# qq456cvb/CanonicalVoting

Hardware: AMD Instinct MI355X
Metric: scenes/sec (80k-pt synthetic scans) (higher is better)
Workload: dtype f32

## Files before the change

### canonicalvoting_amd/_lib.py

```python
import ctypes
import os
import threading

_HERE = os.path.dirname(os.path.abspath(__file__))
LIB_PATH = os.path.join(_HERE, "_C", "libcvhip.so")

c_float_p = ctypes.POINTER(ctypes.c_float)
c_int_p = ctypes.POINTER(ctypes.c_int)
c_i32_p = ctypes.POINTER(ctypes.c_int32)
c_i64_p = ctypes.POINTER(ctypes.c_int64)
vp = ctypes.c_void_p
ABI_VERSION = 4


class CvError(RuntimeError):
    pass


class DecodeParams(ctypes.Structure):
    _fields_ = [("thresh_high", ctypes.c_float), ("thresh_low", ctypes.c_float),
                ("valid_ratio", ctypes.c_float), ("elimination", ctypes.c_int),
                ("prob_thresh", ctypes.c_float), ("elim_hi_plus1", ctypes.c_int),
                ("max_iters", ctypes.c_int), ("err_thresh", ctypes.c_double)]


class ConvDesc(ctypes.Structure):
    _fields_ = [("in_", vp), ("n_in", ctypes.c_longlong), ("in_ld", ctypes.c_int), ("cin", ctypes.c_int),
                ("weight", vp), ("K", ctypes.c_int), ("cout", ctypes.c_int), ("nbr", vp),
                ("n_out", ctypes.c_longlong), ("scale", vp), ("shift", vp), ("residual", vp),
                ("res_ld", ctypes.c_int), ("relu", ctypes.c_int), ("out", vp), ("out_ld", ctypes.c_int),
                ("flavour", ctypes.c_int), ("ws", vp), ("ws_bytes", ctypes.c_size_t), ("row_perm", vp),
                ("j_begin", ctypes.c_int), ("j_end", ctypes.c_int), ("acc_in", vp), ("acc_ld", ctypes.c_int),
                ("perm_groups", ctypes.c_int), ("plan_ent", vp), ("plan_cnt", vp),
                ("weight_packed", vp), ("weight_x6", vp), ("in2", vp), ("in2_ld", ctypes.c_int), ("cin2", ctypes.c_int),
                ("weight2_x6", vp), ("perm_has_map", ctypes.c_int), ("weight_pieces", ctypes.c_int),
                ("acc_scale", ctypes.c_float), ("range_flag", vp), ("in_hl", ctypes.c_int), ("out_hl", ctypes.c_int),
                ("res_hl", ctypes.c_int), ("split_tickets", vp), ("acc_scale_dev", vp)]


class SceneMaps(ctypes.Structure):
    _fields_ = [("stem", ctypes.c_longlong), ("out", ctypes.c_longlong), ("down", ctypes.c_longlong * 4),
                ("k3", ctypes.c_longlong * 5), ("up", ctypes.c_longlong * 4), ("mask_perm", ctypes.c_longlong * 5),
                ("up_perm", ctypes.c_longlong * 4), ("scratch", ctypes.c_longlong), ("bitmap", ctypes.c_longlong)]


class ScenePlanLayout(ctypes.Structure):
    _fields_ = [("cap", ctypes.c_longlong), ("perm", ctypes.c_longlong), ("inv", ctypes.c_longlong),
                ("coords", ctypes.c_longlong * 5), ("vals", ctypes.c_longlong * 5), ("counts", ctypes.c_longlong),
                ("arena", ctypes.c_longlong), ("int_words", ctypes.c_longlong), ("key_words", ctypes.c_longlong),
                ("sort_ws_bytes", ctypes.c_size_t), ("levels_ws_bytes", ctypes.c_size_t)]


NET_MAP_SLOTS, NET_PERM_SLOTS = 15, 9


class NetBuf(ctypes.Structure):
    _fields_ = [("level", ctypes.c_int), ("channels", ctypes.c_int), ("rows_level", ctypes.c_int), ("hl", ctypes.c_int)]


class NetOp(ctypes.Structure):
    _fields_ = [("in_buf", ctypes.c_int), ("in_col", ctypes.c_int), ("cin", ctypes.c_int),
                ("out_buf", ctypes.c_int), ("out_col", ctypes.c_int), ("cout", ctypes.c_int),
                ("res_buf", ctypes.c_int), ("res_col", ctypes.c_int), ("map", ctypes.c_int), ("K", ctypes.c_int),
                ("perm", ctypes.c_int), ("perm_groups", ctypes.c_int), ("relu", ctypes.c_int),
                ("weight", vp), ("scale", vp), ("shift", vp), ("weight_x6", vp), ("in2_buf", ctypes.c_int),
                ("in2_col", ctypes.c_int), ("cin2", ctypes.c_int), ("weight2_x6", vp), ("weight_pieces", ctypes.c_int), ("acc_scale", ctypes.c_float)]


class SceneDesc(ctypes.Structure):
    _fields_ = [("d_coords4", vp), ("n", ctypes.c_longlong), ("d_feats", vp), ("feats_ld", ctypes.c_int), ("d_points", vp),
                ("res", ctypes.c_float), ("num_rots", ctypes.c_int), ("ops", vp), ("n_ops", ctypes.c_int), ("bufs", vp),
                ("n_bufs", ctypes.c_int), ("stem_k", ctypes.c_int), ("mask_groups", ctypes.c_int),
                ("masked_min_rows", ctypes.c_longlong), ("max_channels", ctypes.c_int),
                ("use_range_flag", ctypes.c_int),
                ("d_out_feats", vp), ("out_ld", ctypes.c_int), ("out_channels", ctypes.c_int), ("nclasses", ctypes.c_int),
                ("log_scale", ctypes.c_int), ("d_xyz_in", vp), ("d_scale_in", vp), ("d_prob_in", vp), ("d_class_in", vp),
                ("vote_algo", ctypes.c_int), ("decode", DecodeParams), ("max_candidates", ctypes.c_int),
                ("nms_threshold", ctypes.c_double), ("d_ws", vp), ("ws_bytes", ctypes.c_size_t), ("d_grids", vp),
                ("grid_capacity_floats", ctypes.c_size_t), ("h_pinned", vp), ("pinned_bytes", ctypes.c_size_t),
                ("h_cand_idx", vp), ("h_verdict", vp), ("h_boxes", vp), ("h_scores", vp), ("h_classes", vp), ("h_pick", vp),
                ("adaptive_split", ctypes.c_int), ("events", vp * 5),
                ("conv_split_target", ctypes.c_int), ("vote_part_records", ctypes.c_int)]


MAX_CATEGORIES = 16


class SceneSeparateDesc(ctypes.Structure):
    _fields_ = [("d_coords4", vp), ("n", ctypes.c_longlong), ("d_feats", vp), ("feats_ld", ctypes.c_int), ("d_points", vp),
                ("res", ctypes.c_float), ("num_rots", ctypes.c_int), ("num_models", ctypes.c_int),
                ("ops", vp), ("n_ops", vp), ("bufs", vp), ("n_bufs", vp),
                ("stem_k", ctypes.c_int), ("mask_groups", ctypes.c_int), ("masked_min_rows", ctypes.c_longlong),
                ("max_channels", ctypes.c_int), ("use_range_flag", ctypes.c_int),
                ("d_out_feats", vp), ("out_ld", ctypes.c_int), ("out_channels", ctypes.c_int), ("log_scale", ctypes.c_int),
                ("d_xyz_in", vp), ("d_scale_in", vp), ("d_prob_in", vp), ("vote_algo", ctypes.c_int), ("decode", DecodeParams),
                ("max_candidates", ctypes.c_int), ("nms_threshold", ctypes.c_double), ("d_ws", vp), ("ws_bytes", ctypes.c_size_t),
                ("h_pinned", vp), ("pinned_bytes", ctypes.c_size_t), ("h_cand_idx", vp), ("h_verdict", vp), ("h_boxes", vp),
                ("h_scores", vp), ("h_det_cat", vp), ("h_det_box", vp), ("events", vp * 5),
                ("conv_split_target", ctypes.c_int), ("vote_part_records", ctypes.c_int)]


class SceneSeparateResult(ctypes.Structure):
    _fields_ = [("n_cand", ctypes.c_int * MAX_CATEGORIES), ("n_boxes", ctypes.c_int * MAX_CATEGORIES),
                ("truncated", ctypes.c_int * MAX_CATEGORIES), ("n_det", ctypes.c_int), ("range_flag", ctypes.c_int),
                ("duplicates", ctypes.c_int), ("out_of_window", ctypes.c_int), ("dims", ctypes.c_int * 3),
                ("corner", ctypes.c_float * 3), ("level_rows", ctypes.c_longlong * 5), ("needed_ws_bytes", ctypes.c_size_t),
                ("d_grid_obj", vp), ("d_grid_rot", vp), ("d_grid_scale", vp), ("d_xyz", vp), ("d_scale", vp), ("d_prob", vp),
                ("host_us", ctypes.c_float * 4)]


class PackJob(ctypes.Structure):
    _fields_ = [("w", vp), ("wp", vp), ("K", ctypes.c_int), ("cin", ctypes.c_int), ("cout", ctypes.c_int), ("trans", ctypes.c_int),
                ("scale_log2", ctypes.c_int), ("reserved", ctypes.c_int)]


class SceneResult(ctypes.Structure):
    _fields_ = [("n_cand", ctypes.c_int), ("n_boxes", ctypes.c_int), ("n_det", ctypes.c_int), ("truncated", ctypes.c_int),
                ("range_flag", ctypes.c_int), ("duplicates", ctypes.c_int), ("out_of_window", ctypes.c_int),
                ("scenes_in_flight", ctypes.c_int), ("dims", ctypes.c_int * 3), ("corner", ctypes.c_float * 3), ("level_rows", ctypes.c_longlong * 5),
                ("needed_ws_bytes", ctypes.c_size_t), ("needed_grid_floats", ctypes.c_size_t),
                ("d_grid_obj", vp), ("d_grid_rot", vp), ("d_grid_scale", vp), ("d_xyz", vp), ("d_scale", vp),
                ("d_prob", vp), ("d_class", vp), ("host_us", ctypes.c_float * 4)]


SIGNATURES = {
    "cv_abi_version": (ctypes.c_int, []),
    "cv_last_error": (ctypes.c_char_p, []),
    "cv_hv_minmax_workspace_bytes": (ctypes.c_size_t, []),
    "cv_hv_minmax_f32": (ctypes.c_int, [vp, ctypes.c_int64, c_float_p, c_float_p, vp, ctypes.c_size_t, vp]),
    "cv_hv_minmax_async_f32": (ctypes.c_int, [vp, ctypes.c_int64, vp, vp, ctypes.c_size_t, vp]),
    "cv_hv_grid_dims_f32": (ctypes.c_int, [c_float_p, c_float_p, ctypes.c_float, c_int_p]),
    "cv_hv_forward_workspace_bytes": (ctypes.c_size_t, [ctypes.c_int64, ctypes.c_int, c_int_p, ctypes.c_int]),
    "cv_hv_forward_f32": (ctypes.c_int, [vp, vp, vp, vp, ctypes.c_int64, ctypes.c_float, ctypes.c_int,
                                         c_float_p, c_int_p, vp, vp, vp, vp, ctypes.c_size_t,
                                         ctypes.c_int, vp]),
    "cv_hv_forward_cat_workspace_bytes": (ctypes.c_size_t, [ctypes.c_int64, ctypes.c_int, c_int_p, ctypes.c_int, ctypes.c_int]),
    "cv_hv_forward_cat_f32": (ctypes.c_int, [vp, vp, vp, vp, ctypes.c_int64, ctypes.c_float, ctypes.c_int, c_float_p, c_int_p,
                                             ctypes.c_int, vp, vp, vp, vp, ctypes.c_size_t, ctypes.c_int, vp]),
    "cv_hv_set_kernel_events": (ctypes.c_int, [vp, vp]),
    "cv_hv_backward_f32": (ctypes.c_int, [vp, vp, vp, vp, vp, ctypes.c_int64, ctypes.c_float,
                                          ctypes.c_int, c_float_p, c_int_p, vp, vp, vp, vp]),
    "cv_hv_count_votes_f32": (ctypes.c_int, [vp, vp, vp, ctypes.c_int64, ctypes.c_float, ctypes.c_int,
                                             c_float_p, c_int_p, c_i64_p, vp, ctypes.c_size_t, vp]),
    "cv_decode_workspace_bytes": (ctypes.c_size_t, [c_int_p, ctypes.c_int64, ctypes.c_int]),
    "cv_decode_f32": (ctypes.c_int, [vp, vp, vp, c_int_p, c_float_p, ctypes.c_float, vp, vp, vp, vp,
                                     ctypes.c_int64, ctypes.POINTER(DecodeParams), ctypes.c_int, vp,
                                     ctypes.c_size_t, c_int_p, c_i64_p, c_i32_p, c_int_p, c_float_p,
                                     c_float_p, c_i32_p, c_int_p, vp]),
    "cv_decode_cat_workspace_bytes": (ctypes.c_size_t, [c_int_p, ctypes.c_int64, ctypes.c_int, ctypes.c_int]),
    "cv_decode_cat_f32": (ctypes.c_int, [vp, vp, vp, c_int_p, c_float_p, ctypes.c_float, vp, vp, vp, vp, ctypes.c_int64,
                                         ctypes.c_int, ctypes.POINTER(DecodeParams), ctypes.c_int, vp, ctypes.c_size_t, c_int_p,
                                         c_i64_p, c_i32_p, c_int_p, c_float_p, c_float_p, c_i32_p, c_int_p, vp]),
    "cv_detect_scene_separate_f32": (ctypes.c_int, [ctypes.POINTER(SceneSeparateDesc), ctypes.POINTER(SceneSeparateResult), vp]),
    "cv_sp_table_capacity": (ctypes.c_longlong, [ctypes.c_longlong]),
    "cv_sp_levels_workspace_bytes": (ctypes.c_size_t, [ctypes.c_longlong]),
    "cv_sp_build_levels": (ctypes.c_int, [ctypes.POINTER(vp), ctypes.POINTER(vp), ctypes.POINTER(vp),
                                          ctypes.c_longlong, ctypes.c_longlong, ctypes.c_int, vp,
                                          c_i32_p, vp, ctypes.c_size_t, vp]),
    "cv_sp_quantize_workspace_bytes": (ctypes.c_size_t, [ctypes.c_longlong]),
    "cv_sp_quantize_f32": (ctypes.c_int, [vp, ctypes.c_longlong, ctypes.c_longlong, ctypes.c_float, ctypes.c_int, c_i64_p,
                                          ctypes.c_int, vp, vp, vp, vp, c_i32_p, vp, ctypes.c_size_t, vp]),
    "cv_sp_quantize_f64": (ctypes.c_int, [vp, ctypes.c_longlong, ctypes.c_longlong, ctypes.c_double, ctypes.c_int, c_i64_p,
                                          ctypes.c_int, vp, vp, vp, vp, c_i32_p, vp, ctypes.c_size_t, vp]),
    "cv_sp_morton_keys": (ctypes.c_int, [vp, ctypes.c_longlong, vp, vp]),
    "cv_sp_sort_workspace_bytes": (ctypes.c_size_t, [ctypes.c_longlong]),
    "cv_sp_sort_rows": (ctypes.c_int, [vp, ctypes.c_longlong, vp, vp, vp, vp, ctypes.c_size_t, vp]),
    "cv_sp_pack_weights_stem_h2_f32": (ctypes.c_int, [vp, ctypes.c_int, ctypes.c_int, vp, ctypes.c_int, vp, vp]),
    "cv_sp_to_hl_f32": (ctypes.c_int, [vp, ctypes.c_longlong, ctypes.c_int, ctypes.c_int, vp, ctypes.c_int, vp, vp]),
    "cv_sp_from_hl_f32": (ctypes.c_int, [vp, ctypes.c_longlong, ctypes.c_int, ctypes.c_int, vp, ctypes.c_int, vp]),
    "cv_sp_kernel_map": (ctypes.c_int, [vp, ctypes.c_longlong, vp, vp, ctypes.c_longlong, ctypes.c_int,
                                        ctypes.c_int, vp, vp]),
    "cv_sp_up_map": (ctypes.c_int, [vp, ctypes.c_longlong, ctypes.c_longlong, vp, vp]),
    "cv_sp_conv_workspace_bytes": (ctypes.c_size_t, [ctypes.c_longlong, ctypes.c_int, ctypes.c_int]),
    "cv_sp_conv_f32": (ctypes.c_int, [ctypes.POINTER(ConvDesc), vp]),
    "cv_sp_set_split_target": (ctypes.c_int, [ctypes.c_int]),
    "cv_hv_set_part_records": (ctypes.c_int, [ctypes.c_int]),
    "cv_hv_set_part_records_thread": (ctypes.c_int, [ctypes.c_int]),
    "cv_sp_pack_weights_h2_batch_f32": (ctypes.c_int, [ctypes.POINTER(PackJob), ctypes.c_int, vp, vp]),
    "cv_sp_copy_unless_flag": (ctypes.c_int, [ctypes.POINTER(vp), ctypes.POINTER(vp), ctypes.POINTER(ctypes.c_longlong), ctypes.c_int, vp, vp]),
    "cv_sp_pack_weights_t_f32": (ctypes.c_int, [vp, ctypes.c_int, ctypes.c_int, ctypes.c_int, ctypes.c_int, ctypes.c_int, vp, vp]),
    "cv_sp_set_split_target_thread": (ctypes.c_int, [ctypes.c_int]),
    "cv_sp_set_ablation": (ctypes.c_int, [ctypes.c_int]),
    "cv_sp_set_option": (ctypes.c_int, [ctypes.c_char_p, ctypes.c_longlong, ctypes.POINTER(ctypes.c_longlong)]),
    "cv_sp_get_option": (ctypes.c_int, [ctypes.c_char_p, ctypes.POINTER(ctypes.c_longlong)]),
    "cv_sp_pack_weights_x6_f32": (ctypes.c_int, [vp, ctypes.c_int, ctypes.c_int, ctypes.c_int, vp, vp, vp]),
    "cv_sp_pack_weights_h2_f32": (ctypes.c_int, [vp, ctypes.c_int, ctypes.c_int, ctypes.c_int, vp, ctypes.c_int, vp, vp]),
    "cv_sp_pack_weights_bf16_f32": (ctypes.c_int, [vp, ctypes.c_int, ctypes.c_int, ctypes.c_int, vp, vp, vp]),
    "cv_sp_scene_maps_words": (ctypes.c_size_t, [c_i64_p, ctypes.c_longlong, ctypes.c_int, ctypes.c_int,
                                                 ctypes.c_longlong, ctypes.POINTER(SceneMaps)]),
    "cv_sp_scene_maps": (ctypes.c_int, [ctypes.POINTER(vp), ctypes.POINTER(vp), ctypes.POINTER(vp), ctypes.c_longlong,
                                        c_i64_p, vp, ctypes.c_longlong, ctypes.c_int,
                                        ctypes.c_int, ctypes.c_longlong, vp, ctypes.c_size_t, vp]),
    "cv_sp_scene_plan_words": (ctypes.c_size_t, [ctypes.c_longlong, ctypes.c_int, ctypes.c_int, ctypes.c_longlong]),
    "cv_sp_scene_plan": (ctypes.c_int, [vp, ctypes.c_longlong, vp, vp, ctypes.POINTER(vp), ctypes.POINTER(vp),
                                        ctypes.POINTER(vp), ctypes.c_longlong, vp, c_i32_p, ctypes.c_int, ctypes.c_int,
                                        ctypes.c_longlong, vp, ctypes.c_size_t, ctypes.POINTER(SceneMaps), vp,
                                        ctypes.c_size_t, vp, ctypes.c_size_t, vp]),
    "cv_sp_scene_plan_layout": (ctypes.c_int, [ctypes.c_longlong, ctypes.c_int, ctypes.c_int, ctypes.c_longlong,
                                               ctypes.POINTER(ScenePlanLayout)]),
    "cv_sp_scene_plan_slots": (ctypes.c_int, [ctypes.POINTER(ScenePlanLayout), ctypes.POINTER(SceneMaps), c_i64_p,
                                              ctypes.c_longlong, vp, ctypes.POINTER(vp), ctypes.POINTER(vp)]),
    "cv_sp_scene_conv_workspace_bytes": (ctypes.c_size_t, [c_i64_p, c_int_p, ctypes.c_int, ctypes.c_int]),
    "cv_net_arena_bytes": (ctypes.c_size_t, [ctypes.POINTER(NetBuf), ctypes.c_int, c_i64_p, ctypes.c_int]),
    "cv_net_run_f32": (ctypes.c_int, [ctypes.POINTER(NetOp), ctypes.c_int, ctypes.POINTER(NetBuf), ctypes.c_int,
                                      c_i64_p, ctypes.c_int, vp, ctypes.c_size_t, ctypes.POINTER(vp), c_int_p,
                                      ctypes.POINTER(vp), ctypes.c_int, ctypes.POINTER(vp), ctypes.c_int,
                                      vp, ctypes.c_size_t, vp, vp]),
    "cv_sp_mask_keys": (ctypes.c_int, [vp, ctypes.c_longlong, ctypes.c_int, ctypes.c_int, ctypes.c_int, vp, vp]),
    "cv_sp_mask_perms": (ctypes.c_int, [vp, ctypes.c_longlong, ctypes.c_int, ctypes.c_int, vp, vp, ctypes.c_size_t,
                                        ctypes.c_int, vp]),
    "cv_sp_transpose_map": (ctypes.c_int, [vp, ctypes.c_longlong, ctypes.c_int, ctypes.c_longlong, vp, vp]),
    "cv_sp_wgrad_workspace_bytes": (ctypes.c_size_t, [ctypes.c_longlong, ctypes.c_int, ctypes.c_int, ctypes.c_int]),
    "cv_sp_conv_wgrad_f32": (ctypes.c_int, [vp, ctypes.c_int, ctypes.c_int, vp, ctypes.c_int, ctypes.c_int, vp,
                                            ctypes.c_int, ctypes.c_longlong, vp, vp, ctypes.c_size_t, vp]),
    "cv_sp_conv_wgrad_px_f32": (ctypes.c_int, [vp, ctypes.c_int, ctypes.c_int, vp, ctypes.c_int, ctypes.c_int, vp,
                                               ctypes.c_int, ctypes.c_longlong, vp, vp, ctypes.c_size_t, ctypes.c_int,
                                               vp]),
    "cv_sp_col_sum_f32": (ctypes.c_int, [vp, ctypes.c_longlong, ctypes.c_int, ctypes.c_int, vp, vp]),
    "cv_sp_col_sum_workspace_bytes": (ctypes.c_size_t, [ctypes.c_longlong, ctypes.c_int]),
    "cv_sp_col_sum_det_f32": (ctypes.c_int, [vp, ctypes.c_longlong, ctypes.c_int, ctypes.c_int, vp, vp, ctypes.c_size_t, vp]),
    "cv_sp_bn_workspace_bytes": (ctypes.c_size_t, [ctypes.c_int]),
    "cv_sp_bn_stats_f32": (ctypes.c_int, [vp, ctypes.c_longlong, ctypes.c_int, ctypes.c_int, vp, vp, ctypes.c_float,
                                          ctypes.c_float, vp, vp, vp, vp, vp, vp, vp, ctypes.c_size_t, vp]),
    "cv_sp_bn_backward_f32": (ctypes.c_int, [vp, vp, vp, ctypes.c_longlong, ctypes.c_int, ctypes.c_int, vp, vp,
                                             ctypes.c_float, vp, vp, vp, vp, vp, vp, ctypes.c_size_t, vp]),
    "cv_sp_bn_backward_hl_f32": (ctypes.c_int, [vp, vp, vp, ctypes.c_longlong, ctypes.c_int, ctypes.c_int, vp, vp,
                                                ctypes.c_float, vp, vp, vp, vp, vp, vp, ctypes.c_size_t, vp, vp, vp, vp, vp]),
    "cv_sp_affine_f32": (ctypes.c_int, [vp, ctypes.c_longlong, ctypes.c_int, ctypes.c_int, vp, vp, vp, ctypes.c_int,
                                        ctypes.c_int, vp, ctypes.c_int, vp]),
    "cv_sp_affine_hl_f32": (ctypes.c_int, [vp, ctypes.c_longlong, ctypes.c_int, ctypes.c_int, vp, vp, vp, ctypes.c_int,
                                           ctypes.c_int, vp, ctypes.c_int, vp, ctypes.c_int, vp, vp, vp]),
    "cv_sp_bn_fold_f32": (ctypes.c_int, [vp, vp, vp, vp, vp, ctypes.c_float, ctypes.c_int, vp, vp, vp]),
    "cv_head_joint_f32": (ctypes.c_int, [vp, ctypes.c_longlong, ctypes.c_int, ctypes.c_int, ctypes.c_int,
                                         vp, vp, vp, vp, vp]),
    "cv_head_separate_f32": (ctypes.c_int, [vp, ctypes.c_longlong, ctypes.c_int, ctypes.c_int, vp, vp, vp, vp]),
    "cv_detect_scene_f32": (ctypes.c_int, [ctypes.POINTER(SceneDesc), ctypes.POINTER(SceneResult), vp]),
    "cv_iou_obb": (ctypes.c_double, [c_float_p, c_float_p]),
    "cv_nms_obb": (ctypes.c_int, [c_float_p, c_float_p, ctypes.c_int, ctypes.c_double, c_i32_p]),
}

_lib = None


def lib():
    global _lib
    if _lib is None:
        if not os.path.exists(LIB_PATH):
            raise CvError(
                "canonicalvoting_amd: HIP library %s not found. Build it with "
                "`python -m canonicalvoting_amd.csrc.build` (hipcc, gfx950). There is no CPU "
                "fallback for this op." % LIB_PATH)
        import torch
        if torch.cuda.is_available():
            torch.cuda.init()
        L = ctypes.CDLL(LIB_PATH)
        for name, (res, args) in SIGNATURES.items():
            fn = getattr(L, name)
            fn.restype = res
            fn.argtypes = args
        _lib = L
    return _lib


_scratch_lock = threading.Lock()
_scratch_bufs = {}


def scratch(dev, name, nbytes):
    import torch
    key = (dev.index if dev.index is not None else torch.cuda.current_device(),
           torch.cuda.current_stream(dev).cuda_stream, name)
    nbytes = max(int(nbytes), 256)
    with _scratch_lock:
        buf = _scratch_bufs.get(key)
    if buf is None or buf.numel() < nbytes:
        buf = torch.empty(nbytes + nbytes // 8, dtype=torch.uint8, device=dev)
        with _scratch_lock:
            _scratch_bufs[key] = buf
    return buf


def release_scratch(dev=None, stream=None):
    h = getattr(stream, "cuda_stream", stream)
    d = getattr(dev, "index", dev)
    with _scratch_lock:
        for key in [k for k in _scratch_bufs if (d is None or k[0] == d) and (h is None or k[1] == h)]:
            del _scratch_bufs[key]


def scratch_bytes():
    with _scratch_lock:
        return sum(b.numel() for b in _scratch_bufs.values())


def check(rc, what):
    if rc != 0:
        msg = lib().cv_last_error()
        raise CvError("%s failed (%d): %s" % (what, rc, msg.decode() if msg else ""))
```

### canonicalvoting_amd/csrc/net_exec.cpp

```cpp
#include <algorithm>
#include <cstdlib>
#include <mutex>
#include <unordered_map>
#include <vector>

#include "cv_common.h"

namespace {

struct Slot { char* ptr; int ld; long long rows; };

}

extern "C" {

static void scene_maps_layout(const long long* rows, long long n_orig, int stem_k, int mask_groups,
                              long long masked_min_rows, cv_scene_maps* o, size_t* total) {
    size_t off = 0;
    auto take = [&](size_t words) { const size_t at = off; off += cv_align_up(words, 64); return (long long)at; };
    const size_t K5 = (size_t)stem_k * stem_k * stem_k;
    const size_t mp_w = mask_groups > 1 ? (size_t)mask_groups * (1 + (27 + mask_groups - 1) / mask_groups) + (mask_groups + 3) / 4 : 0;
    o->stem = take((size_t)rows[0] * K5);
    o->k3[0] = take((size_t)rows[0] * 28);
    o->mask_perm[0] = (mask_groups > 1 && rows[0] >= masked_min_rows) ? take(mp_w * rows[0]) : -1;
// ... 103 lines not shown
}

namespace {
struct PlanSide { hipEvent_t ev; int32_t* h_pinned; int device; };
std::mutex g_plan_mu;
std::unordered_map<int, std::vector<PlanSide>> g_plan_free;
int plan_side_acquire(PlanSide* out) {
    int dev = 0;
    CV_HIP_CHECK(hipGetDevice(&dev));
    {
        std::lock_guard<std::mutex> lk(g_plan_mu);
        auto& pool = g_plan_free[dev];
        if (!pool.empty()) {
            *out = pool.back();
            pool.pop_back();
            return CV_OK;
        }
    }
    PlanSide p{};
    p.device = dev;
    CV_HIP_CHECK(hipEventCreateWithFlags(&p.ev, hipEventDisableTiming));
    CV_HIP_CHECK(hipHostMalloc(reinterpret_cast<void**>(&p.h_pinned), 64, hipHostMallocDefault));
    *out = p;
    return CV_OK;
}
struct PlanSideLease {
    PlanSide ps{};
    bool held = false;
    ~PlanSideLease() {
        if (!held) return;
        (void)hipEventSynchronize(ps.ev);
        std::lock_guard<std::mutex> lk(g_plan_mu);
        g_plan_free[ps.device].push_back(ps);
    }
};
}

size_t cv_sp_scene_plan_words(long long n, int stem_k, int mask_groups, long long masked_min_rows) {
    if (n <= 0 || stem_k < 1) return 0;
    const long long rows[5] = {n, n, n, n, n};
    cv_scene_maps o;
    size_t total = 0;
    scene_maps_layout(rows, n, stem_k, mask_groups, masked_min_rows, &o, &total);
    return total;
}

int cv_sp_scene_plan_layout(long long n, int stem_k, int mask_groups, long long masked_min_rows, cv_scene_plan_layout* out) {
    CV_REQUIRE(out && n > 0, CV_EINVAL, "bad scene plan layout arguments");
    auto up64 = [](long long v) { return (v + 63) / 64 * 64; };
    cv_scene_plan_layout& l = *out;
    l.cap = cv_sp_table_capacity(n);
    l.perm = 0, l.inv = up64(n);
    for (int i = 0; i < 5; ++i) l.coords[i] = l.inv + up64(n) + i * up64(4 * n);
    for (int i = 0; i < 5; ++i) l.vals[i] = l.coords[4] + up64(4 * n) + i * up64(l.cap);
    l.counts = l.vals[4] + up64(l.cap), l.arena = l.counts + 64;
    l.int_words = l.arena + (long long)cv_sp_scene_plan_words(n, stem_k, mask_groups, masked_min_rows);
    l.key_words = 5 * l.cap;
    l.sort_ws_bytes = cv_sp_sort_workspace_bytes(n), l.levels_ws_bytes = cv_sp_levels_workspace_bytes(n);
    return CV_OK;
}

int cv_sp_scene_plan_slots(const cv_scene_plan_layout* layout, const cv_scene_maps* offsets, const long long* level_rows,
                           long long min_rows, const int32_t* d_ibuf, const int32_t** maps, const int32_t** perms) {
    CV_REQUIRE(layout && offsets && level_rows && maps && perms, CV_EINVAL, "null pointer argument");
    const cv_scene_maps& off = *offsets;
    const int32_t* ap = d_ibuf + layout->arena;
    maps[0] = ap + off.stem;
    for (int i = 0; i < 4; ++i) maps[1 + i] = ap + off.down[i];
    for (int i = 0; i < 5; ++i) maps[5 + i] = ap + off.k3[i];
    for (int i = 0; i < 4; ++i) maps[10 + i] = ap + off.up[i];
    maps[14] = d_ibuf + layout->inv;
    for (int i = 0; i < 5; ++i) perms[i] = (off.mask_perm[i] >= 0 && level_rows[i] >= min_rows) ? ap + off.mask_perm[i] : nullptr;
    for (int i = 0; i < 4; ++i) perms[5 + i] = ap + off.up_perm[i];
    return CV_OK;
}

size_t cv_sp_scene_conv_workspace_bytes(const long long* level_rows, const int* masked, int mask_groups, int max_channels) {
    if (!level_rows || !masked) return 0;
    size_t bytes = 0;
    for (int i = 0; i < 5; ++i) {
        if (masked[i]) bytes = std::max(bytes, (size_t)4 * mask_groups * (size_t)level_rows[i] * max_channels + 256);
        bytes = std::max(bytes, cv_sp_conv_workspace_bytes(std::min<long long>(level_rows[i], 128 * 384 - 1), max_channels, 27));
    }
    return bytes;
}

int cv_sp_scene_plan(const int32_t* d_input, long long n, int32_t* d_perm, int32_t* d_inv, int32_t* const* d_coords,
                     unsigned long long* const* d_keys, int32_t* const* d_vals, long long cap, int32_t* d_counts,
                     int32_t* h_counts, int stem_k, int mask_groups, long long masked_min_rows, int32_t* d_arena,
                     size_t arena_words, cv_scene_maps* offsets, void* d_sort_ws, size_t sort_ws_bytes, void* d_levels_ws,
                     size_t levels_ws_bytes, void* stream) {
    return cv_sp_scene_plan_ex(d_input, n, d_perm, d_inv, d_coords, d_keys, d_vals, cap, d_counts, h_counts, stem_k, mask_groups,
                               masked_min_rows, d_arena, arena_words, offsets, d_sort_ws, sort_ws_bytes, d_levels_ws,
                               levels_ws_bytes, false, stream);
}

}

int cv_sp_scene_plan_ex(const int32_t* d_input, long long n, int32_t* d_perm, int32_t* d_inv, int32_t* const* d_coords,
                        unsigned long long* const* d_keys, int32_t* const* d_vals, long long cap, int32_t* d_counts,
                        int32_t* h_counts, int stem_k, int mask_groups, long long masked_min_rows,
                        int32_t* d_arena, size_t arena_words, cv_scene_maps* offsets, void* d_sort_ws, size_t sort_ws_bytes,
                        void* d_levels_ws, size_t levels_ws_bytes, bool single_batch, void* stream, bool bounds_prefilled) {
    CV_REQUIRE(d_input && d_perm && d_inv && d_coords && d_keys && d_vals && d_counts && h_counts && d_arena && offsets &&
                   d_sort_ws && d_levels_ws, CV_EINVAL, "null pointer argument");
    CV_REQUIRE(arena_words >= cv_sp_scene_plan_words(n, stem_k, mask_groups, masked_min_rows), CV_ENOMEM,
               "scene map arena too small (cv_sp_scene_plan_words)");
    hipStream_t st = static_cast<hipStream_t>(stream);
    int rc = cv_sp_sort_rows_ex(d_input, n, d_coords[0], d_perm, d_inv, d_sort_ws, sort_ws_bytes, single_batch, stream, bounds_prefilled);
    if (rc != CV_OK) return rc;
    long long rows[5] = {n, 1, 1, 1, 1};
    cv_scene_maps o;
    size_t total = 0;
    scene_maps_layout(rows, n, stem_k, mask_groups, masked_min_rows, &o, &total);
    static const bool bitmap_on = !(getenv("CV_MAP_BITMAP") && atoi(getenv("CV_MAP_BITMAP")) == 0);
    const long long n_zero = o.bitmap + (bitmap_on ? CV_BITMAP_WORDS : 0) - o.scratch;
    rc = cv_sp_build_levels_zero(d_coords, d_keys, d_vals, n, cap, 5, d_counts, nullptr, d_levels_ws, levels_ws_bytes,
                                 d_arena + o.scratch, n_zero, bitmap_on ? static_cast<int32_t*>(d_sort_ws) + 7 : nullptr, stream,
                                 bitmap_on ? reinterpret_cast<uint32_t*>(d_arena + o.bitmap) : nullptr);
    if (rc != CV_OK) return rc;
    PlanSideLease lease;
    rc = plan_side_acquire(&lease.ps);
    if (rc != CV_OK) return rc;
    lease.held = true;
    const PlanSide& ps = lease.ps;
    CV_HIP_CHECK(hipMemcpyAsync(ps.h_pinned, d_counts, sizeof(int32_t) * 8, hipMemcpyDeviceToHost, st));
    CV_HIP_CHECK(hipEventRecord(ps.ev, st));
    rc = scene_maps_level0(d_coords, d_keys, d_vals, cap, n, d_perm, stem_k, mask_groups, o, d_arena,
                           bitmap_on ? static_cast<const int32_t*>(d_sort_ws) : nullptr, stream, true, bitmap_on);
    if (rc != CV_OK) return rc;
    CV_HIP_CHECK(hipEventSynchronize(ps.ev));
    for (int i = 0; i < 8; ++i) h_counts[i] = ps.h_pinned[i];
    if (h_counts[5] != 0 || h_counts[6] != 0) return CV_OK;
    for (int i = 0; i < 5; ++i) rows[i] = h_counts[i];
    CV_REQUIRE(rows[0] == n, CV_EINVAL, "level 0 lost rows (%lld of %lld)", rows[0], n);
    scene_maps_layout(rows, n, stem_k, mask_groups, masked_min_rows, &o, &total);
    CV_REQUIRE(arena_words >= total, CV_ENOMEM, "scene map arena too small");
    *offsets = o;
    return scene_maps_coarse(d_coords, d_keys, d_vals, cap, rows, mask_groups, o, d_arena, stream, true);
}

extern "C" {

size_t cv_net_arena_bytes(const cv_net_buf* bufs, int n_bufs, const long long* level_rows, int n_levels) {
    if (!bufs || !level_rows || n_bufs <= 0) return 0;
    size_t total = 256;
    for (int i = 0; i < n_bufs; ++i) {
        if (bufs[i].level < 0 || bufs[i].level >= n_levels) continue;
        total += cv_align_up(sizeof(float) * (size_t)level_rows[bufs[i].level] * (size_t)bufs[i].channels, 256);
    }
    return total;
}

int cv_net_run_f32(const cv_net_op* ops, int n_ops, const cv_net_buf* bufs, int n_bufs, const long long* level_rows,
                   int n_levels, void* d_arena, size_t arena_bytes, const void* const* ext_ptr, const int* ext_ld,
                   const int32_t* const* maps, int n_maps, const int32_t* const* perms, int n_perms,
                   void* d_ws, size_t ws_bytes, int32_t* range_flag, void* stream) {
    CV_REQUIRE(ops && bufs && level_rows && d_arena && n_ops > 0 && n_bufs > 0 && n_levels > 0, CV_EINVAL,
               "bad network program arguments");
    CV_REQUIRE(arena_bytes >= cv_net_arena_bytes(bufs, n_bufs, level_rows, n_levels), CV_ENOMEM, "arena too small");
    std::vector<Slot> slot((size_t)n_bufs);
    {
        CvCarver cv(d_arena);
        int ext = 0;
        for (int i = 0; i < n_bufs; ++i) {
            const int lv = bufs[i].level;
            if (lv < 0 || lv >= n_levels) {
                CV_REQUIRE(ext_ptr && ext_ld && ext_ptr[ext], CV_EINVAL, "external buffer %d has no pointer", ext);
                slot[i] = {static_cast<char*>(const_cast<void*>(ext_ptr[ext])), ext_ld[ext], bufs[i].rows_level >= 0 &&
                           bufs[i].rows_level < n_levels ? level_rows[bufs[i].rows_level] : 0};
                ++ext;
            } else {
                slot[i] = {reinterpret_cast<char*>(cv.take<float>((size_t)level_rows[lv] * bufs[i].channels)),
                           bufs[i].channels, level_rows[lv]};
            }
        }
    }
    for (int k = 0; k < n_ops; ++k) {
        const cv_net_op& o = ops[k];
        CV_REQUIRE(o.in_buf >= 0 && o.in_buf < n_bufs && o.out_buf >= 0 && o.out_buf < n_bufs &&
                       o.res_buf < n_bufs && o.map < n_maps && o.perm < n_perms, CV_EINVAL, "op %d: bad slot", k);
        const Slot& in = slot[o.in_buf];
        const Slot& out = slot[o.out_buf];
        cv_conv_desc d = {};
        d.in_hl = bufs[o.in_buf].hl;
        d.out_hl = bufs[o.out_buf].hl;
        d.res_hl = o.res_buf >= 0 ? bufs[o.res_buf].hl : 0;
        CV_REQUIRE(o.in2_buf < 0 || bufs[o.in2_buf].hl == d.in_hl, CV_EINVAL, "op %d: both sources must share a format", k);
        d.in = reinterpret_cast<const float*>(in.ptr) + o.in_col;
        d.n_in = in.rows;
        d.in_ld = in.ld;
        d.cin = o.cin;
        d.weight = o.weight;
        d.weight_x6 = o.weight_x6;
        d.weight_pieces = o.weight_pieces;
        d.acc_scale = o.acc_scale;
        d.range_flag = (o.weight_pieces == 2 || d.out_hl) ? range_flag : nullptr;
        if (o.in2_buf >= 0) {
            CV_REQUIRE(o.in2_buf < n_bufs, CV_EINVAL, "op %d: bad second-source slot", k);
            d.in2 = reinterpret_cast<const float*>(slot[o.in2_buf].ptr) + o.in2_col;
            d.in2_ld = slot[o.in2_buf].ld;
            d.cin2 = o.cin2;
            d.weight2_x6 = o.weight2_x6;
        }
        d.K = o.K;
        d.cout = o.cout;
        d.nbr = o.map >= 0 ? maps[o.map] : nullptr;
        d.n_out = out.rows;
        d.scale = o.scale;
        d.shift = o.shift;
        if (o.res_buf >= 0) {
            d.residual = reinterpret_cast<const float*>(slot[o.res_buf].ptr) + o.res_col;
            d.res_ld = slot[o.res_buf].ld;
        }
        d.relu = o.relu;
        d.out = reinterpret_cast<float*>(out.ptr) + o.out_col;
        d.out_ld = out.ld;
        d.ws = d_ws;
        d.ws_bytes = ws_bytes;
        const int32_t* perm = o.perm >= 0 ? perms[o.perm] : nullptr;
        if (perm) {
            d.row_perm = perm;
            d.perm_groups = o.perm_groups;
            d.perm_has_map = o.perm_groups > 1;
        }
        const int rc = cv_sp_conv_f32(&d, stream);
        if (rc != CV_OK) return rc;
    }
    return CV_OK;
}

}
```

### canonicalvoting_amd/csrc/scene_exec.cpp

```cpp
#include <algorithm>
#include <atomic>
#include <chrono>
#include <cstdlib>
#include <cstring>
#include <vector>

#include "cv_common.h"

namespace {

struct Carver {
    char* base; size_t off = 0, cap;
    Carver(void* p, size_t c) : base(static_cast<char*>(p)), cap(c) {}
    template <typename T> T* take(size_t count) {
        off = cv_align_up(off, 256);
        T* r = (base && off + count * sizeof(T) <= cap) ? reinterpret_cast<T*>(base + off) : nullptr;
        off += count * sizeof(T);
        return r;
    }
};

std::atomic<int> g_scenes_inside{0};
struct SceneCount {
    int before;
    bool set_target, set_records;
    int prev_target = 0, prev_records = 0;
    SceneCount(bool adaptive, int split_target, int part_records)
        : before(g_scenes_inside.fetch_add(1, std::memory_order_relaxed)), set_target(adaptive || split_target > 0),
          set_records(part_records > 0) {
        if (set_target) prev_target = cv_sp_set_split_target_thread(split_target > 0 ? split_target : before + 1 >= 4 ? 256 : 768);
        if (set_records) prev_records = cv_hv_set_part_records_thread(part_records);
    }
    ~SceneCount() {
        if (set_target) cv_sp_set_split_target_thread(prev_target);
        if (set_records) cv_hv_set_part_records_thread(prev_records);
        g_scenes_inside.fetch_sub(1, std::memory_order_relaxed);
    }
};

struct StageClock {
    void* const* events; hipStream_t st; float* host_us;
    std::chrono::steady_clock::time_point t_prev = std::chrono::steady_clock::now();
    hipError_t mark(int i) const { return events[i] ? hipEventRecord(static_cast<hipEvent_t>(events[i]), st) : hipSuccess; }
    void lap(int i) {
        const auto t = std::chrono::steady_clock::now();
        host_us[i] += std::chrono::duration<float, std::micro>(t - t_prev).count();
        t_prev = t;
    }
};

struct SceneFront {
    const int32_t* d_coords4; long long n; const float* d_points; float res;
    int stem_k, mask_groups; long long masked_min_rows; int max_channels;
    float* h_minmax;
    cv_scene_plan_layout lay;
    void* mm_ws; int32_t* ibuf; unsigned long long* kbuf; char* sort_ws; char* lev_ws;
    cv_scene_maps off;
    long long rows[5];
    float mn[3]; int dims[3]; size_t cells;
    const int32_t* maps[CV_NET_MAP_SLOTS]; const int32_t* perms[CV_NET_PERM_SLOTS];
    size_t conv_ws_b;

    template <class D> explicit SceneFront(const D* d)
        : d_coords4(d->d_coords4), n(d->n), d_points(d->d_points), res(d->res), stem_k(d->stem_k), mask_groups(d->mask_groups),
          masked_min_rows(d->masked_min_rows), max_channels(d->max_channels), h_minmax(static_cast<float*>(d->h_pinned)) {}

    bool carve(Carver& cv) {
        mm_ws = cv.take<char>(cv_hv_minmax_workspace_bytes());
        cv_sp_scene_plan_layout(n, stem_k, mask_groups, masked_min_rows, &lay);
        ibuf = cv.take<int32_t>((size_t)lay.int_words);
        kbuf = cv.take<unsigned long long>((size_t)lay.key_words);
        sort_ws = cv.take<char>(lay.sort_ws_bytes);
        lev_ws = cv.take<char>(lay.levels_ws_bytes);
        return mm_ws && ibuf && kbuf && sort_ws && lev_ws;
    }

    template <class R> int run(int32_t* d_zero_word, R* r, StageClock& clock, void* stream) {
        int rc = cv_hv_minmax_async_ex(d_points, n, h_minmax, mm_ws, cv_hv_minmax_workspace_bytes(), d_zero_word,
                                       reinterpret_cast<int32_t*>(sort_ws), stream);
        if (rc != CV_OK) return rc;
        int32_t *c_coords[5], *c_vals[5];
        unsigned long long* c_keys[5];
        for (int i = 0; i < 5; ++i) {
            c_coords[i] = ibuf + lay.coords[i];
            c_keys[i] = kbuf + (size_t)lay.cap * i;
            c_vals[i] = ibuf + lay.vals[i];
        }
        int32_t counts_h[8] = {0};
        rc = cv_sp_scene_plan_ex(d_coords4, n, ibuf + lay.perm, ibuf + lay.inv, c_coords, c_keys, c_vals, lay.cap, ibuf + lay.counts,
                                 counts_h, stem_k, mask_groups, masked_min_rows, ibuf + lay.arena, (size_t)(lay.int_words - lay.arena),
                                 &off, sort_ws, lay.sort_ws_bytes, lev_ws, lay.levels_ws_bytes,
                                  true, stream,  true);
        if (rc != CV_OK) return rc;
        r->duplicates = counts_h[5];
        r->out_of_window = counts_h[6];
        CV_REQUIRE(counts_h[5] == 0 && counts_h[6] == 0, CV_EINVAL,
                   "duplicate coordinates (%d) or coordinates outside the 16-bit key window (%d)", counts_h[5], counts_h[6]);
        clock.lap(0);
        for (int i = 0; i < 5; ++i) { rows[i] = counts_h[i]; r->level_rows[i] = counts_h[i]; }
        float mx[3];
        for (int k = 0; k < 3; ++k) { mn[k] = h_minmax[k]; mx[k] = h_minmax[3 + k]; r->corner[k] = mn[k]; }
        rc = cv_hv_grid_dims_f32(mn, mx, res, dims);
        if (rc != CV_OK) return rc;
        for (int k = 0; k < 3; ++k) r->dims[k] = dims[k];
        cells = (size_t)dims[0] * dims[1] * dims[2];
        int masked[5];
        for (int i = 0; i < 5; ++i) masked[i] = off.mask_perm[i] >= 0;
        conv_ws_b = cv_sp_scene_conv_workspace_bytes(rows, masked, mask_groups, max_channels);
        return cv_sp_scene_plan_slots(&lay, &off, rows, masked_min_rows, ibuf, maps, perms);
    }
};

template <class R> int fixed_part_too_small(R* r, size_t fixed_end) {
    r->needed_ws_bytes = fixed_end * 2 + ((size_t)256 << 20);
    cv_set_error("scene workspace too small (needs at least %zu bytes)", r->needed_ws_bytes);
    return CV_ENOMEM;
}

}

extern "C" {

int cv_detect_scene_f32(const cv_scene_desc* d, cv_scene_result* r, void* stream) {
    CV_REQUIRE(d && r, CV_EINVAL, "null scene descriptor / result");
    CV_REQUIRE(d->d_coords4 && d->d_feats && d->d_points && d->n > 0 && d->ops && d->bufs && d->n_ops > 0 && d->n_bufs > 0,
               CV_EINVAL, "bad scene descriptor");
    CV_REQUIRE(d->d_out_feats && d->out_ld >= d->out_channels && d->out_channels > 0, CV_EINVAL, "bad network output buffer");
    CV_REQUIRE(d->h_pinned && d->pinned_bytes >= 256 && d->d_ws, CV_EINVAL, "pinned scratch (>= 256 bytes) and a device workspace are required");
    CV_REQUIRE(d->h_boxes && d->h_scores && d->h_classes && d->h_cand_idx && d->h_verdict && d->h_pick && d->max_candidates > 0,
               CV_EINVAL, "null result arrays");
    hipStream_t st = static_cast<hipStream_t>(stream);
    const long long n = d->n;
    std::memset(r, 0, sizeof(*r));
    CV_REQUIRE(d->conv_split_target >= 0 && d->vote_part_records >= 0, CV_EINVAL, "negative launch sizing");
    SceneCount in_flight(d->adaptive_split != 0, d->conv_split_target, d->vote_part_records);
    r->scenes_in_flight = in_flight.before + 1;
    Carver cv(d->d_ws, d->ws_bytes);
    StageClock clock{d->events, st, r->host_us};
    CV_HIP_CHECK(clock.mark(0));

    SceneFront f(d);
    int32_t* h_flag = reinterpret_cast<int32_t*>(static_cast<char*>(d->h_pinned) + 64);
    const bool plan_fits = f.carve(cv);
    float* xyz = cv.take<float>((size_t)n * 3);
    float* scale = cv.take<float>((size_t)n * 3);
    float* prob = cv.take<float>((size_t)n);
    int32_t* cls = cv.take<int32_t>((size_t)n);
    int32_t* d_flag = cv.take<int32_t>(64);
    if (!plan_fits || !xyz || !scale || !prob || !cls || !d_flag) return fixed_part_too_small(r, cv.off);
    int rc = f.run(d_flag, r, clock, stream);
    if (rc != CV_OK) return rc;
    const size_t cells = f.cells;

    const size_t arena_b = cv_net_arena_bytes(d->bufs, d->n_bufs, f.rows, 5);
    const size_t vote_ws_b = cv_hv_forward_workspace_bytes(n, d->num_rots, f.dims, d->vote_algo);
    const size_t dec_ws_b = cv_decode_workspace_bytes(f.dims, n, d->max_candidates);
    char* arena = cv.take<char>(arena_b);
    char* conv_ws = cv.take<char>(f.conv_ws_b);
    char* vote_ws = cv.take<char>(std::max<size_t>(vote_ws_b, 256));
    char* dec_ws = cv.take<char>(dec_ws_b);
    float* grids = d->d_grids ? d->d_grids : cv.take<float>(6 * cells);
    r->needed_ws_bytes = cv.off + 4096;
    r->needed_grid_floats = 6 * cells;
    CV_REQUIRE(arena && conv_ws && vote_ws && dec_ws && grids, CV_ENOMEM, "scene workspace too small (needs %zu bytes)", r->needed_ws_bytes);
    CV_REQUIRE(!d->d_grids || d->grid_capacity_floats >= 6 * cells, CV_ENOMEM, "grid buffer too small (needs %zu floats)", 6 * cells);
    float* g_obj = grids;
    float* g_rot = grids + cells;
    float* g_scale = grids + 3 * cells;
    r->d_grid_obj = g_obj; r->d_grid_rot = g_rot; r->d_grid_scale = g_scale;

    const void* ext_ptr[2] = {d->d_feats, d->d_out_feats};
    const int ext_ld[2] = {d->feats_ld, d->out_ld};
    rc = cv_net_run_f32(d->ops, d->n_ops, d->bufs, d->n_bufs, f.rows, 5, arena, arena_b, ext_ptr, ext_ld, f.maps, CV_NET_MAP_SLOTS,
                        f.perms, CV_NET_PERM_SLOTS, conv_ws, f.conv_ws_b, d->use_range_flag ? d_flag : nullptr, stream);
    if (rc != CV_OK) return rc;
    clock.lap(1);
    CV_HIP_CHECK(clock.mark(1));
    rc = cv_head_joint_f32(d->d_out_feats, n, d->out_ld, d->nclasses, d->log_scale, xyz, scale, prob, cls, stream);
    if (rc != CV_OK) return rc;
    if (d->use_range_flag) CV_HIP_CHECK(hipMemcpyAsync(h_flag, d_flag, sizeof(int32_t), hipMemcpyDeviceToHost, st));
    r->d_xyz = xyz; r->d_scale = scale; r->d_prob = prob; r->d_class = cls;
    CV_HIP_CHECK(clock.mark(2));

    const float* v_xyz = d->d_xyz_in ? d->d_xyz_in : xyz;
    const float* v_scale = d->d_scale_in ? d->d_scale_in : scale;
    const float* v_prob = d->d_prob_in ? d->d_prob_in : prob;
    const int32_t* v_cls = d->d_class_in ? d->d_class_in : cls;
    rc = cv_hv_forward_f32(d->d_points, v_xyz, v_scale, v_prob, n, d->res, d->num_rots, f.mn, f.dims, g_obj, g_rot, g_scale, vote_ws,
                           std::max<size_t>(vote_ws_b, 256), d->vote_algo, stream);
    if (rc != CV_OK) return rc;
    CV_HIP_CHECK(clock.mark(3));
    clock.lap(2);
    cv_decode_params prm = d->decode;
    prm.max_iters = d->max_candidates;
    int n_cand = 0, n_boxes = 0, truncated = 0;
    rc = cv_decode_f32_ev(g_obj, g_rot, g_scale, f.dims, f.mn, d->res, d->d_points, v_xyz, v_prob, v_cls, n, &prm, 0, dec_ws, dec_ws_b, &n_cand,
                          d->h_cand_idx, d->h_verdict, &n_boxes, d->h_boxes, d->h_scores, d->h_classes, &truncated, stream, d->events[4]);
    if (rc != CV_OK) return rc;
    r->n_cand = n_cand;
    r->n_boxes = n_boxes;
    r->truncated = truncated;
    r->range_flag = d->use_range_flag ? *h_flag : 0;

    int n_det = 0;
    std::vector<float> bc, sc;
    std::vector<int32_t> idx, pick;
    for (int c = 0; c < d->nclasses; ++c) {
        bc.clear(); sc.clear(); idx.clear();
        for (int i = 0; i < n_boxes; ++i)
            if (d->h_classes[i] == c) {
                bc.insert(bc.end(), d->h_boxes + (size_t)i * 24, d->h_boxes + (size_t)i * 24 + 24);
                sc.push_back(d->h_scores[i]);
                idx.push_back(i);
            }
        if (idx.empty()) continue;
        pick.assign(idx.size(), 0);
        const int k = cv_nms_obb(bc.data(), sc.data(), (int)idx.size(), d->nms_threshold, pick.data());
        if (k < 0) return k;
        for (int j = 0; j < k; ++j) d->h_pick[n_det++] = idx[(size_t)pick[j]];
    }
    r->n_det = n_det;
    clock.lap(3);
    return CV_OK;
}

int cv_detect_scene_separate_f32(const cv_scene_separate_desc* d, cv_scene_separate_result* r, void* stream) {
    CV_REQUIRE(d && r, CV_EINVAL, "null scene descriptor / result");
    std::memset(r, 0, sizeof(*r));
    const int K = d->num_models;
    CV_REQUIRE(K >= 1 && K <= CV_MAX_CATEGORIES, CV_EINVAL, "num_models out of range (%d, 1..%d)", K, CV_MAX_CATEGORIES);
    CV_REQUIRE(d->d_coords4 && d->d_feats && d->d_points && d->n > 0 && d->ops && d->n_ops && d->bufs && d->n_bufs && d->d_out_feats,
               CV_EINVAL, "bad scene descriptor");
    for (int k = 0; k < K; ++k)
        CV_REQUIRE(d->ops[k] && d->bufs[k] && d->n_ops[k] > 0 && d->n_bufs[k] > 0 && d->d_out_feats[k], CV_EINVAL,
                   "bad program or output buffer of model %d", k);
    CV_REQUIRE(d->out_ld >= d->out_channels && d->out_channels >= 8, CV_EINVAL, "bad network output buffer");
    CV_REQUIRE(d->h_pinned && d->pinned_bytes >= 64 + 64 * (size_t)K && d->d_ws, CV_EINVAL,
               "pinned scratch (>= 64 + 64 K bytes) and a device workspace are required");
    CV_REQUIRE(d->h_boxes && d->h_scores && d->h_cand_idx && d->h_verdict && d->h_det_cat && d->h_det_box && d->max_candidates > 0,
               CV_EINVAL, "null result arrays");
    CV_REQUIRE(!!d->d_xyz_in == !!d->d_scale_in && !!d->d_xyz_in == !!d->d_prob_in, CV_EINVAL, "predictions: all three or none");
    CV_REQUIRE(d->conv_split_target >= 0 && d->vote_part_records >= 0, CV_EINVAL, "negative launch sizing");
    hipStream_t st = static_cast<hipStream_t>(stream);
    const long long n = d->n;
    SceneCount in_flight(false, d->conv_split_target, d->vote_part_records);
    Carver cv(d->d_ws, d->ws_bytes);
    StageClock clock{d->events, st, r->host_us};
    CV_HIP_CHECK(clock.mark(0));

    SceneFront f(d);
    int32_t* h_flags = reinterpret_cast<int32_t*>(static_cast<char*>(d->h_pinned) + 64);
    const bool plan_fits = f.carve(cv);
    float* xyz = cv.take<float>((size_t)K * n * 3);
    float* scale = cv.take<float>((size_t)K * n * 3);
    float* prob = cv.take<float>((size_t)K * n);
    int32_t* d_flags = cv.take<int32_t>(16 * (size_t)K);
    if (!plan_fits || !xyz || !scale || !prob || !d_flags) return fixed_part_too_small(r, cv.off);
    if (d->use_range_flag) CV_HIP_CHECK(hipMemsetAsync(d_flags, 0, sizeof(int32_t) * 16 * K, st));
    int rc = f.run(nullptr, r, clock, stream);
    if (rc != CV_OK) return rc;
    const size_t cells = f.cells;

    size_t arena_b = 0;
    for (int k = 0; k < K; ++k) arena_b = std::max(arena_b, cv_net_arena_bytes(d->bufs[k], d->n_bufs[k], f.rows, 5));
    const size_t vote_ws_b = cv_hv_forward_cat_workspace_bytes(n, d->num_rots, f.dims, d->vote_algo, K);
    const size_t dec_ws_b = cv_decode_cat_workspace_bytes(f.dims, n, d->max_candidates, K);
    char* arena = cv.take<char>(arena_b);
    char* conv_ws = cv.take<char>(f.conv_ws_b);
    char* vote_ws = cv.take<char>(std::max<size_t>(vote_ws_b, 256));
    char* dec_ws = cv.take<char>(dec_ws_b);
    float* grids = cv.take<float>(6 * cells * (size_t)K);
    r->needed_ws_bytes = cv.off + 4096;
    CV_REQUIRE(arena && conv_ws && vote_ws && dec_ws && grids, CV_ENOMEM, "scene workspace too small (needs %zu bytes)", r->needed_ws_bytes);
    float* g_obj = grids;
    float* g_rot = grids + cells * K;
    float* g_scale = grids + 3 * cells * K;
    r->d_grid_obj = g_obj; r->d_grid_rot = g_rot; r->d_grid_scale = g_scale;

    for (int k = 0; k < K; ++k) {
        const void* ext_ptr[2] = {d->d_feats, d->d_out_feats[k]};
        const int ext_ld[2] = {d->feats_ld, d->out_ld};
        rc = cv_net_run_f32(d->ops[k], d->n_ops[k], d->bufs[k], d->n_bufs[k], f.rows, 5, arena, arena_b, ext_ptr, ext_ld, f.maps,
                            CV_NET_MAP_SLOTS, f.perms, CV_NET_PERM_SLOTS, conv_ws, f.conv_ws_b,
                            d->use_range_flag ? d_flags + 16 * k : nullptr, stream);
        if (rc != CV_OK) return rc;
    }
    clock.lap(1);
    CV_HIP_CHECK(clock.mark(1));
    for (int k = 0; k < K; ++k) {
        rc = cv_head_separate_f32(d->d_out_feats[k], n, d->out_ld, d->log_scale, xyz + (size_t)k * n * 3, scale + (size_t)k * n * 3,
                                  prob + (size_t)k * n, stream);
        if (rc != CV_OK) return rc;
    }
    if (d->use_range_flag) CV_HIP_CHECK(hipMemcpyAsync(h_flags, d_flags, sizeof(int32_t) * 16 * K, hipMemcpyDeviceToHost, st));
    r->d_xyz = xyz; r->d_scale = scale; r->d_prob = prob;
    CV_HIP_CHECK(clock.mark(2));

    const float* v_xyz = d->d_xyz_in ? d->d_xyz_in : xyz;
    const float* v_scale = d->d_xyz_in ? d->d_scale_in : scale;
    const float* v_prob = d->d_xyz_in ? d->d_prob_in : prob;
    rc = cv_hv_forward_cat_f32(d->d_points, v_xyz, v_scale, v_prob, n, d->res, d->num_rots, f.mn, f.dims, K, g_obj, g_rot, g_scale, vote_ws,
                               std::max<size_t>(vote_ws_b, 256), d->vote_algo, stream);
    if (rc != CV_OK) return rc;
    CV_HIP_CHECK(clock.mark(3));
    clock.lap(2);
    cv_decode_params prm = d->decode;
    prm.max_iters = d->max_candidates;
    const int M = d->max_candidates;
    std::vector<int32_t> classes((size_t)K * M);
    rc = cv_decode_cat_f32_ev(g_obj, g_rot, g_scale, f.dims, f.mn, d->res, d->d_points, v_xyz, v_prob, nullptr, n, K, &prm, 0, dec_ws,
                              dec_ws_b, r->n_cand, d->h_cand_idx, d->h_verdict, r->n_boxes, d->h_boxes, d->h_scores, classes.data(),
                              r->truncated, stream, d->events[4]);
    if (rc != CV_OK) return rc;
    if (d->use_range_flag)
        for (int k = 0; k < K; ++k) r->range_flag |= h_flags[16 * k] ? (1 << k) : 0;

    int n_det = 0;
    std::vector<int32_t> pick((size_t)M);
    for (int k = 0; k < K; ++k) {
        const int nb = r->n_boxes[k];
        if (nb == 0) continue;
        const int kept = cv_nms_obb(d->h_boxes + (size_t)k * M * 24, d->h_scores + (size_t)k * M, nb, d->nms_threshold, pick.data());
        if (kept < 0) return kept;
        for (int j = 0; j < kept; ++j) { d->h_det_cat[n_det] = k; d->h_det_box[n_det] = pick[(size_t)j]; ++n_det; }
    }
    r->n_det = n_det;
    clock.lap(3);
    return CV_OK;
}

}
```

### canonicalvoting_amd/csrc/sparse_conv.hip

```cpp
#include "cv_common.h"

#include <atomic>
#include <cstring>
#include <type_traits>
#include <utility>

#include "sparse_conv_common.h"

using namespace cvsc;

namespace {

template <int NB, bool VEC>
__global__ __launch_bounds__(THREADS) void conv_rows(ConvArgs a) {
    __shared__ float A_s[KC][A_LD];
    __shared__ float B_s[KC][NB * 32];
    __shared__ int nbr_s[TM];
    __shared__ int rows_s[TM];
    __shared__ __attribute__((aligned(16))) float ep_s[4][32][EP_LD];
    const int tid = threadIdx.x, lane = tid & 63, wave = tid >> 6;
    const int n0 = blockIdx.y * (NB * 32);

    if (tid < TM) {
        const long long tile_id = a.row_perm ? (long long)gridDim.x - 1 - blockIdx.x : blockIdx.x;
// ... 1254 lines not shown

__global__ __launch_bounds__(256) void col_sum_partial(const float* __restrict__ x, long long n, int c, int ld,
                                                       float* __restrict__ ws) {
    __shared__ float s[8][32];
    const int col = blockIdx.x * 32 + (threadIdx.x & 31), ry = threadIdx.x >> 5;
    const long long r_lo = n * blockIdx.y / gridDim.y, r_hi = n * (blockIdx.y + 1) / gridDim.y;
    float acc = 0.f;
    if (col < c)
        for (long long r = r_lo + ry; r < r_hi; r += 8) acc += x[r * ld + col];
    s[ry][threadIdx.x & 31] = acc;
    __syncthreads();
    if (ry == 0 && col < c) {
        float t = 0.f;
        for (int k = 0; k < 8; ++k) t += s[k][threadIdx.x & 31];
        ws[(long long)blockIdx.y * c + col] = t;
    }
}
__global__ __launch_bounds__(256) void col_sum_chunks(const float* __restrict__ ws, int chunks, int c,
                                                      float* __restrict__ out) {
    const int col = blockIdx.x * 256 + threadIdx.x;
    if (col >= c) return;
    float s0 = 0.f, s1 = 0.f, s2 = 0.f, s3 = 0.f;
    int k = 0;
    for (; k + 3 < chunks; k += 4) {
        s0 += ws[(long long)k * c + col];
        s1 += ws[(long long)(k + 1) * c + col];
        s2 += ws[(long long)(k + 2) * c + col];
        s3 += ws[(long long)(k + 3) * c + col];
    }
    for (; k < chunks; ++k) s0 += ws[(long long)k * c + col];
    out[col] = (s0 + s1) + (s2 + s3);
}

__global__ __launch_bounds__(256) void conv_finish(ConvArgs a) {
    __shared__ float4 red[4][64];
    const int q = threadIdx.x >> 6, l = threadIdx.x & 63;
    const long long total4 = a.n_out * (long long)a.cout / 4;
    const long long total = a.n_out * (long long)a.cout;
    for (long long base = blockIdx.x * 64ll; base < total4; base += (long long)gridDim.x * 64) {
        const long long e4 = base + l;
        float4 s = make_float4(0.f, 0.f, 0.f, 0.f);
        if (e4 < total4) {
            const float4* p = reinterpret_cast<const float4*>(a.partial) + e4;
#pragma unroll 4
            for (int k = q; k < a.splits; k += 4) {
                const float4 v = partial_load4(p + (long long)k * (total / 4));
                s.x += v.x; s.y += v.y; s.z += v.z; s.w += v.w;
            }
        }
        red[q][l] = s;
        __syncthreads();
        if (q == 0 && e4 < total4) {
            float v[4] = {red[0][l].x + red[1][l].x + red[2][l].x + red[3][l].x,
                          red[0][l].y + red[1][l].y + red[2][l].y + red[3][l].y,
                          red[0][l].z + red[1][l].z + red[2][l].z + red[3][l].z,
                          red[0][l].w + red[1][l].w + red[2][l].w + red[3][l].w};
            const long long e = e4 * 4;
            const long long row = e / a.cout;
            const int col = (int)(e - row * a.cout);
            if (a.wide) {
                float4 x = make_float4(v[0], v[1], v[2], v[3]);
                if (a.acc_in) {
                    const float4 p = *reinterpret_cast<const float4*>(a.acc_in + row * a.acc_ld + col);
                    x.x += p.x; x.y += p.y; x.z += p.z; x.w += p.w;
                }
                const float4 sc = a.scale ? *reinterpret_cast<const float4*>(a.scale + col) : make_float4(1.f, 1.f, 1.f, 1.f);
                const float4 sh = a.shift ? *reinterpret_cast<const float4*>(a.shift + col) : make_float4(0.f, 0.f, 0.f, 0.f);
                x.x = x.x * sc.x + sh.x; x.y = x.y * sc.y + sh.y; x.z = x.z * sc.z + sh.z; x.w = x.w * sc.w + sh.w;
                if (a.res) {
                    const float4 p = a.res_hl ? hl_load4(a.res + row * a.res_ld, col)
                                              : *reinterpret_cast<const float4*>(a.res + row * a.res_ld + col);
                    x.x += p.x; x.y += p.y; x.z += p.z; x.w += p.w;
                }
                if (a.relu) { x.x = fmaxf(x.x, 0.f); x.y = fmaxf(x.y, 0.f); x.z = fmaxf(x.z, 0.f); x.w = fmaxf(x.w, 0.f); }
                if (a.out_hl) {
                    if (a.range_flag && hl_out_of_range(x)) *a.range_flag = 1;
                    hl_store4(a.out + row * a.out_ld, col, x);
                } else {
                    *reinterpret_cast<float4*>(a.out + row * a.out_ld + col) = x;
                }
            } else
#pragma unroll
            for (int i = 0; i < 4; ++i) {
                float x = v[i];
                if (a.acc_in) x += a.acc_in[row * a.acc_ld + col + i];
                x = x * (a.scale ? a.scale[col + i] : 1.f) + (a.shift ? a.shift[col + i] : 0.f);
                if (a.res) x += a.res[row * a.res_ld + col + i];
                if (a.relu) x = fmaxf(x, 0.f);
                a.out[row * a.out_ld + col + i] = x;
            }
        }
        __syncthreads();
    }
}

constexpr int FINISH_SMALL_MAX = 16;
__global__ __launch_bounds__(256) void conv_finish_small(ConvArgs a) {
    const long long total4 = a.n_out * (long long)a.cout / 4;
    const int cq = a.cout >> 2;
    for (long long e4 = blockIdx.x * 256ll + threadIdx.x; e4 < total4; e4 += (long long)gridDim.x * 256) {
        const float4* p = reinterpret_cast<const float4*>(a.partial) + e4;
        const long long row = e4 / cq;
        float4 pv[FINISH_SMALL_MAX];
#pragma unroll
        for (int k = 0; k < FINISH_SMALL_MAX; ++k)
            pv[k] = (k < a.splits && (!a.gvalid || a.gvalid[(long long)k * a.n_out + row]))
                        ? partial_load4(p + (long long)k * total4) : make_float4(0.f, 0.f, 0.f, 0.f);
        const int col = (int)(e4 - row * cq) * 4;
        float4 sq[4];
#pragma unroll
        for (int q = 0; q < 4; ++q) sq[q] = make_float4(0.f, 0.f, 0.f, 0.f);
#pragma unroll
        for (int k = 0; k < FINISH_SMALL_MAX; ++k)
            if (k < a.splits) { sq[k & 3].x += pv[k].x; sq[k & 3].y += pv[k].y; sq[k & 3].z += pv[k].z; sq[k & 3].w += pv[k].w; }
        float4 x = make_float4(sq[0].x + sq[1].x + sq[2].x + sq[3].x, sq[0].y + sq[1].y + sq[2].y + sq[3].y,
                               sq[0].z + sq[1].z + sq[2].z + sq[3].z, sq[0].w + sq[1].w + sq[2].w + sq[3].w);
        if (a.acc_in) {
            const float4 q = *reinterpret_cast<const float4*>(a.acc_in + row * a.acc_ld + col);
            x.x += q.x; x.y += q.y; x.z += q.z; x.w += q.w;
        }
        const float4 sc = a.scale ? *reinterpret_cast<const float4*>(a.scale + col) : make_float4(1.f, 1.f, 1.f, 1.f);
        const float4 sh = a.shift ? *reinterpret_cast<const float4*>(a.shift + col) : make_float4(0.f, 0.f, 0.f, 0.f);
        x.x = x.x * sc.x + sh.x; x.y = x.y * sc.y + sh.y; x.z = x.z * sc.z + sh.z; x.w = x.w * sc.w + sh.w;
        if (a.res) {
            const float4 q = a.res_hl ? hl_load4(a.res + row * a.res_ld, col)
                                      : *reinterpret_cast<const float4*>(a.res + row * a.res_ld + col);
            x.x += q.x; x.y += q.y; x.z += q.z; x.w += q.w;
        }
        if (a.relu) { x.x = fmaxf(x.x, 0.f); x.y = fmaxf(x.y, 0.f); x.z = fmaxf(x.z, 0.f); x.w = fmaxf(x.w, 0.f); }
        if (a.out_hl) {
            if (a.range_flag && hl_out_of_range(x)) *a.range_flag = 1;
            hl_store4(a.out + row * a.out_ld, col, x);
        } else {
            *reinterpret_cast<float4*>(a.out + row * a.out_ld + col) = x;
        }
    }
}

__global__ __launch_bounds__(256) void conv_finish_scalar(ConvArgs a) {
    const long long total = a.n_out * (long long)a.cout;
    for (long long t = blockIdx.x * 256ll + threadIdx.x; t < total; t += (long long)gridDim.x * 256) {
        const long long row = t / a.cout;
        const int col = (int)(t - row * a.cout);
        float v = 0.f;
        for (int sidx = 0; sidx < a.splits; ++sidx) v += a.partial[sidx * total + t];
        if (a.acc_in) v += a.acc_in[row * a.acc_ld + col];
        v = v * (a.scale ? a.scale[col] : 1.f) + (a.shift ? a.shift[col] : 0.f);
        if (a.res) v += a.res[row * a.res_ld + col];
        if (a.relu) v = fmaxf(v, 0.f);
        a.out[row * a.out_ld + col] = v;
    }
}

}
namespace cvsc {
std::atomic<int> g_ablation{0};
int launch_finish(const ConvArgs& a, hipStream_t st) {
    if (g_ablation.load(std::memory_order_relaxed) & 1) return CV_OK;
    const long long total = a.n_out * (long long)a.cout;
    if (a.wide && a.splits <= FINISH_SMALL_MAX)
        conv_finish_small<<<(unsigned)std::min<long long>((total / 4 + 255) / 256, 16384), 256, 0, st>>>(a);
    else if (a.cout % 4 == 0)
        conv_finish<<<(unsigned)std::min<long long>((total / 4 + 63) / 64, 8192), 256, 0, st>>>(a);
    else
        conv_finish_scalar<<<(unsigned)std::min<long long>((total + 255) / 256, 4096), 256, 0, st>>>(a);
    CV_LAUNCH_CHECK();
    return CV_OK;
}
}
namespace {

__global__ __launch_bounds__(256) void mask_keys(const int* __restrict__ nbr, long long n, int K, int j_begin,
                                                 int j_end, long long* __restrict__ keys) {
    const long long i = blockIdx.x * 256ll + threadIdx.x;
    if (i >= n) return;
    unsigned long long m = 0;
    for (int j = j_begin; j < j_end; ++j)
        if (nbr[i * K + j] >= 0) m |= 1ull << (j - j_begin);
    keys[i] = (long long)m;
}

constexpr int MP_BINS = 1024;
constexpr int MP_THREADS = 1024;

__device__ __forceinline__ int group_mask(const int* __restrict__ nbr, long long row, long long n, int K, int jb, int je) {
    int m = 0;
    for (int j = jb; j < je; ++j)
        if (nbr[row * K + j] >= 0) m |= 1 << (j - jb);
    if (je - jb <= 7) m |= __popc(m) << 7;
    (void)n;
    return m;
}

__device__ __forceinline__ int group_mask_of_word(int word, int jb, int je) {
    int m = (int)(((unsigned)word >> jb) & ((1u << (je - jb)) - 1u));
    if (je - jb <= 7) m |= __popc(m) << 7;
    return m;
}

__global__ __launch_bounds__(MP_THREADS) void mp_hist(const int* __restrict__ nbr, long long n, int K, int groups,
                                                      int* __restrict__ hist ) {
    __shared__ int lh[MP_BINS];
    const int g = blockIdx.y;
    const int jb = K * g / groups, je = K * (g + 1) / groups;
    for (int i = threadIdx.x; i < MP_BINS; i += MP_THREADS) lh[i] = 0;
    __syncthreads();
    const long long row = blockIdx.x * (long long)MP_THREADS + threadIdx.x;
    if (row < n) atomicAdd(&lh[group_mask(nbr, row, n, K, jb, je)], 1);
    __syncthreads();
    for (int i = threadIdx.x; i < MP_BINS; i += MP_THREADS)
        if (lh[i]) atomicAdd(&hist[g * MP_BINS + i], lh[i]);
}

__global__ __launch_bounds__(MP_BINS) void mp_scan(int* __restrict__ hist) {
    __shared__ int s[MP_BINS];
    int* h = hist + blockIdx.x * MP_BINS;
    const int v = h[threadIdx.x];
    s[threadIdx.x] = v;
    __syncthreads();
    for (int off = 1; off < MP_BINS; off <<= 1) {
        const int t = threadIdx.x >= off ? s[threadIdx.x - off] : 0;
        __syncthreads();
        s[threadIdx.x] += t;
        __syncthreads();
    }
    h[threadIdx.x] = s[threadIdx.x] - v;
}

__global__ __launch_bounds__(MP_THREADS) void mp_scatter(const int* __restrict__ nbr, long long n, int K, int groups,
                                                         int* __restrict__ cursor, int* __restrict__ perm,
                                                         int* __restrict__ nbrp, int W) {
    unsigned char* gv = nbrp ? reinterpret_cast<unsigned char*>(nbrp + (long long)groups * n * W) : nullptr;
    __shared__ int lh[MP_BINS];
    const int g = blockIdx.y;
    const int jb = K * g / groups, je = K * (g + 1) / groups;
    for (int i = threadIdx.x; i < MP_BINS; i += MP_THREADS) lh[i] = 0;
    __syncthreads();
    const long long row = blockIdx.x * (long long)MP_THREADS + threadIdx.x;
    int key = 0, rank = 0;
    if (row < n) {
        key = group_mask(nbr, row, n, K, jb, je);
        rank = atomicAdd(&lh[key], 1);
    }
    __syncthreads();
    for (int i = threadIdx.x; i < MP_BINS; i += MP_THREADS)
        if (lh[i]) lh[i] = atomicAdd(&cursor[g * MP_BINS + i], lh[i]);
    __syncthreads();
    if (row < n) {
        const long long pos = (long long)g * n + lh[key] + rank;
        perm[pos] = (int)row;
        if (nbrp) {
            for (int j = jb; j < je; ++j) nbrp[pos * W + (j - jb)] = nbr[row * K + j];
            gv[(long long)g * n + row] = key != 0;
        }
    }
}

struct PermJobsDev {
    CvPermJob j[CV_MAX_PERM_JOBS];
    int group_begin[CV_MAX_PERM_JOBS + 1];
    int n;
};

__device__ __forceinline__ int perm_job_of(const PermJobsDev& jobs, int gy) {
    int ji = 0;
    while (ji + 1 < jobs.n && gy >= jobs.group_begin[ji + 1]) ++ji;
    return ji;
}

__global__ __launch_bounds__(MP_THREADS) void mp_hist_batch(const PermJobsDev jobs, int* __restrict__ hist) {
    __shared__ int lh[MP_BINS];
    const int ji = perm_job_of(jobs, blockIdx.y);
    const CvPermJob& jb = jobs.j[ji];
    const long long row = blockIdx.x * (long long)MP_THREADS + threadIdx.x;
    if (blockIdx.x * (long long)MP_THREADS >= jb.n) return;
    const int g = blockIdx.y - jobs.group_begin[ji];
    const int jlo = jb.K * g / jb.groups, jhi = jb.K * (g + 1) / jb.groups;
    for (int i = threadIdx.x; i < MP_BINS; i += MP_THREADS) lh[i] = 0;
    __syncthreads();
    if (row < jb.n)
        atomicAdd(&lh[jb.mask_words ? group_mask_of_word(jb.mask_words[row], jlo, jhi) : group_mask(jb.nbr, row, jb.n, jb.K, jlo, jhi)], 1);
    __syncthreads();
    for (int i = threadIdx.x; i < MP_BINS; i += MP_THREADS)
        if (lh[i]) atomicAdd(&hist[blockIdx.y * MP_BINS + i], lh[i]);
}

__global__ __launch_bounds__(MP_THREADS) void mp_scatter_batch(const PermJobsDev jobs, const int* __restrict__ hist,
                                                               int* __restrict__ cursor) {
    static_assert(MP_THREADS == MP_BINS, "one bin per thread in the scan");
    __shared__ int lh[MP_BINS];
    __shared__ int pre[MP_BINS];
    __shared__ int wtot[MP_THREADS / 64];
    const int ji = perm_job_of(jobs, blockIdx.y);
    const CvPermJob& jb = jobs.j[ji];
    if (blockIdx.x * (long long)MP_THREADS >= jb.n) return;
    const int g = blockIdx.y - jobs.group_begin[ji];
    const int K = jb.K, jlo = K * g / jb.groups, jhi = K * (g + 1) / jb.groups, W = (K + jb.groups - 1) / jb.groups;
    int* nbrp = jb.with_map ? jb.perm + (long long)jb.groups * jb.n : nullptr;
    for (int i = threadIdx.x; i < MP_BINS; i += MP_THREADS) lh[i] = 0;
    {
        const int lane = threadIdx.x & 63, wave = threadIdx.x >> 6;
        const int v = hist[blockIdx.y * MP_BINS + threadIdx.x];
        int incl = v;
#pragma unroll
        for (int off = 1; off < 64; off <<= 1) {
            const int t = __shfl_up(incl, off);
            if (lane >= off) incl += t;
        }
        if (lane == 63) wtot[wave] = incl;
        __syncthreads();
        int base = 0;
#pragma unroll
// ... 227 lines not shown
            const long long o = r * ld + k;
            take(*reinterpret_cast<const float4*>(x + o), MODE == 1 ? *reinterpret_cast<const float4*>(dy + o) : z4,
                 (MODE == 1 && (y || ybits)) ? relu_open4(y, ybits, r, k, ld, c) : z4, y != nullptr || ybits != nullptr);
        }
    }
#pragma unroll
    for (int i = 0; i < 8; ++i) red[threadIdx.x][i] = a[i];
    __syncthreads();
    if (threadIdx.x < cq) {
        double t[8] = {0, 0, 0, 0, 0, 0, 0, 0};
        for (int q = 0; q < rl; ++q)
#pragma unroll
            for (int i = 0; i < 8; ++i) t[i] += red[q * cq + threadIdx.x][i];
#pragma unroll
        for (int i = 0; i < 4; ++i) {
            partial[((long long)blockIdx.x * c + threadIdx.x * 4 + i) * 2 + 0] = t[i];
            partial[((long long)blockIdx.x * c + threadIdx.x * 4 + i) * 2 + 1] = t[4 + i];
        }
    }
}

template <int MODE>
__global__ __launch_bounds__(256) void bn_col_finish(const double* __restrict__ partial, int chunks, long long n, int c,
                                                     float* out0, float* out1, float* running_mean, float* running_var,
                                                     float momentum, const float* gamma, const float* beta, float eps,
                                                     float* scale, float* shift) {
    const int sub = threadIdx.x & 15;
    const int k = blockIdx.x * 16 + (threadIdx.x >> 4);
    double t0 = 0.0, t1 = 0.0;
    if (k < c)
        for (int q = sub; q < chunks; q += 16) {
            t0 += partial[((long long)q * c + k) * 2];
            t1 += partial[((long long)q * c + k) * 2 + 1];
        }
#pragma unroll
    for (int off = 8; off >= 1; off >>= 1) {
        t0 += __shfl_xor(t0, off);
        t1 += __shfl_xor(t1, off);
    }
    if (k >= c || sub != 0) return;
    if (MODE == 0) {
        const double mu = t0 / (double)n;
        double v = t1 / (double)n - mu * mu;
        if (v < 0.0) v = 0.0;
        out0[k] = (float)mu;
        out1[k] = (float)v;
        if (running_mean) {
            const double unb = n > 1 ? v * (double)n / (double)(n - 1) : v;
            running_mean[k] = (1.f - momentum) * running_mean[k] + momentum * (float)mu;
            running_var[k] = (1.f - momentum) * running_var[k] + momentum * (float)unb;
        }
        const float sc = gamma[k] / sqrtf((float)v + eps);
        scale[k] = sc;
        shift[k] = beta[k] - (float)mu * sc;
    } else {
        out0[k] = (float)t0;
        out1[k] = (float)t1;
    }
}

constexpr int BN_SLOT_BLOCKS = 4096;
__global__ __launch_bounds__(256) void bn_backward_apply(const float* __restrict__ x, const float* __restrict__ dy,
                                                         const float* __restrict__ y, long long n, int c, int ld,
                                                         const float* __restrict__ mean, const float* __restrict__ var,
                                                         float eps, const float* __restrict__ gamma,
                                                         const float* __restrict__ sum_dy,
                                                         const float* __restrict__ sum_dy_xhat, float* __restrict__ dx,
                                                         float* __restrict__ dres) {
    const float inv_n = 1.0f / (float)n;
    for (long long t = blockIdx.x * 256ll + threadIdx.x; t < n * c; t += (long long)gridDim.x * 256) {
        const long long r = t / c;
        const int k = (int)(t - r * c);
        const float istd = 1.0f / sqrtf(var[k] + eps);
        const float xh = (x[r * ld + k] - mean[k]) * istd;
        float g = dy[r * ld + k];
        if (y && !(y[r * ld + k] > 0.f)) g = 0.f;
        dx[r * ld + k] = gamma[k] * istd * (g - sum_dy[k] * inv_n - xh * sum_dy_xhat[k] * inv_n);
        if (dres) dres[r * ld + k] = g;
    }
}

__global__ __launch_bounds__(256) void bn_backward_apply4(const float* __restrict__ x, const float* __restrict__ dy,
                                                          const float* __restrict__ y, long long n, int c, int ld,
                                                          const float* __restrict__ mean, const float* __restrict__ var,
                                                          float eps, const float* __restrict__ gamma,
                                                          const float* __restrict__ sum_dy,
                                                          const float* __restrict__ sum_dy_xhat, float* __restrict__ dx,
                                                          float* __restrict__ dres, float* __restrict__ dx_hl = nullptr,
                                                          unsigned* __restrict__ slot = nullptr,
                                                          int* __restrict__ range_flag = nullptr,
                                                          const unsigned* __restrict__ ybits = nullptr) {
    const float inv_n = 1.0f / (float)n;
    const int cq = c >> 2;
    __shared__ unsigned wred[4];
    float hs = 1.f, dmax = 0.f;
    if (dx_hl) {
        unsigned mb = 0u;
        for (int i = threadIdx.x; i < BN_SLOT_BLOCKS; i += 256) mb = max(mb, slot[BN_SLOT_BLOCKS + i]);
#pragma unroll
        for (int off = 32; off > 0; off >>= 1) mb = max(mb, (unsigned)__shfl_xor((int)mb, off));
        if ((threadIdx.x & 63) == 0) wred[threadIdx.x >> 6] = mb;
        __syncthreads();
        mb = max(max(wred[0], wred[1]), max(wred[2], wred[3]));
        __syncthreads();
        const unsigned E = (mb >> 23) & 255u;
        hs = (E >= 10u && E <= 250u) ? __uint_as_float((263u - E) << 23) : 1.f;
        if (blockIdx.x == 0 && threadIdx.x == 0) reinterpret_cast<float*>(slot)[2 * BN_SLOT_BLOCKS] = 1.f / hs;
    }
    for (long long t = blockIdx.x * 256ll + threadIdx.x; t < n * cq; t += (long long)gridDim.x * 256) {
        const long long r = t / cq;
        const int k = (int)(t - r * cq) * 4;
        const long long o = r * ld + k;
        const float4 xv = *reinterpret_cast<const float4*>(x + o);
        float4 g = *reinterpret_cast<const float4*>(dy + o);
        if (y || ybits) {
            const float4 yv = relu_open4(y, ybits, r, k, ld, c);
            if (!(yv.x > 0.f)) g.x = 0.f;
            if (!(yv.y > 0.f)) g.y = 0.f;
            if (!(yv.z > 0.f)) g.z = 0.f;
            if (!(yv.w > 0.f)) g.w = 0.f;
        }
        const float xs[4] = {xv.x, xv.y, xv.z, xv.w}, gs[4] = {g.x, g.y, g.z, g.w};
        float d[4];
#pragma unroll
        for (int i = 0; i < 4; ++i) {
            const float istd = 1.0f / sqrtf(var[k + i] + eps);
            const float xh = (xs[i] - mean[k + i]) * istd;
            d[i] = gamma[k + i] * istd * (gs[i] - sum_dy[k + i] * inv_n - xh * sum_dy_xhat[k + i] * inv_n);
        }
        *reinterpret_cast<float4*>(dx + o) = make_float4(d[0], d[1], d[2], d[3]);
        if (dres) *reinterpret_cast<float4*>(dres + o) = g;
        if (dx_hl) {
            dmax = fmaxf(fmaxf(dmax, fmaxf(fabsf(d[0]), fabsf(d[1]))), fmaxf(fabsf(d[2]), fabsf(d[3])));
            const float4 v = make_float4(d[0] * hs, d[1] * hs, d[2] * hs, d[3] * hs);
            if (range_flag && hl_out_of_range(v)) *range_flag = 1;
            hl_store4(dx_hl + r * ld, k, v);
        }
    }
    if (dx_hl) {
#pragma unroll
        for (int off = 32; off > 0; off >>= 1) dmax = fmaxf(dmax, __shfl_xor(dmax, off));
        if ((threadIdx.x & 63) == 0) wred[threadIdx.x >> 6] = __float_as_uint(dmax);
        __syncthreads();
        if (threadIdx.x == 0) slot[blockIdx.x] = max(max(wred[0], wred[1]), max(wred[2], wred[3]));
    }
}

__global__ __launch_bounds__(256) void head_joint(const float* __restrict__ f, long long n, int ld,
                                                  int ncls, int log_scale, float* __restrict__ xyz,
                                                  float* __restrict__ scale, float* __restrict__ prob,
                                                  int* __restrict__ cls) {
    const long long i = blockIdx.x * 256ll + threadIdx.x;
    if (i >= n) return;
    const float* row = f + i * ld;
    const float* logit = row + 6 * ncls;
    float mx = logit[0];
    int am = 0;
    for (int k = 1; k <= ncls; ++k)
        if (logit[k] > mx) { mx = logit[k]; am = k; }
    float mo = logit[0];
    int ao = 0;
    for (int k = 1; k < ncls; ++k)
        if (logit[k] > mo) { mo = logit[k]; ao = k; }
    float den = 0.f;
    for (int k = 0; k <= ncls; ++k) den += expf(logit[k] - mx);
    const int h = am == ncls ? 0 : am;
    for (int d = 0; d < 3; ++d) {
        xyz[i * 3 + d] = row[h * 3 + d];
        const float s = row[3 * ncls + h * 3 + d];
        scale[i * 3 + d] = log_scale ? expf(s) : s;
    }
    prob[i] = expf(mo - mx) / den;
    cls[i] = ao;
}

__global__ __launch_bounds__(256) void head_separate(const float* __restrict__ f, long long n, int ld,
                                                     int log_scale, float* __restrict__ xyz,
                                                     float* __restrict__ scale, float* __restrict__ prob) {
    const long long i = blockIdx.x * 256ll + threadIdx.x;
    if (i >= n) return;
    const float* row = f + i * ld;
    for (int d = 0; d < 3; ++d) {
        xyz[i * 3 + d] = row[d];
        scale[i * 3 + d] = log_scale ? expf(row[3 + d]) : row[3 + d];
    }
    const float mx = fmaxf(row[6], row[7]);
    const float e0 = expf(row[6] - mx), e1 = expf(row[7] - mx);
    prob[i] = e1 / (e0 + e1);
}

std::atomic<long long> g_opt_zskip{getenv("CV_ZSKIP") ? atoll(getenv("CV_ZSKIP")) : 0};
std::atomic<long long> g_opt_hd_mask{getenv("CV_HD") ? atoll(getenv("CV_HD")) : 4};
std::atomic<long long> g_opt_hd_min_rows{getenv("CV_HD_MIN_ROWS") ? atoll(getenv("CV_HD_MIN_ROWS")) : 16384};
std::atomic<long long> g_opt_hd_shape{getenv("CV_HD_SHAPE") ? atoll(getenv("CV_HD_SHAPE")) : 2};

template <int NB>
int launch_rows(const ConvArgs& a, bool vec, hipStream_t st) {
    dim3 grid((unsigned)((a.n_out + TM - 1) / TM), (unsigned)((a.cout + NB * 32 - 1) / (NB * 32)),
              (unsigned)a.splits);
    int per_wg = 0;
    if (vec) {
        const int nj_wp = a.j_end - a.j_begin, nch_wp = a.cin / KC;
        for (int z = 0; z < a.splits; ++z) {
            long long lo, hi;
            if (a.perm_per_split) {
                lo = (long long)nj_wp * z / a.splits * nch_wp;
                hi = (long long)nj_wp * (z + 1) / a.splits * nch_wp;
            } else {
                lo = (long long)nj_wp * nch_wp * z / a.splits;
                hi = (long long)nj_wp * nch_wp * (z + 1) / a.splits;
            }
            if (hi > lo) per_wg = std::max(per_wg, (int)((hi - 1) / nch_wp - lo / nch_wp + 1));
        }
    }
    static const bool xcd_on = getenv("CV_XCD_TILES") && atoi(getenv("CV_XCD_TILES")) != 0;
    ConvArgs ax = a;
    dim3 gridx = grid;
    if (xcd_on && grid.x >= 64) {
        ax.xcd_tiles = 1;
        gridx.x = (grid.x + 7) / 8 * 8;
    }
    if (a.in_hl) {
        CV_REQUIRE(per_wg * (a.cin / KC) + (a.in2 ? a.cin2 / KC : 0) <= HL_MAX_UNITS, CV_EINVAL,
                   "hl-format convolution: more than %d units per workgroup (Cin too wide)", HL_MAX_UNITS);
        CV_REQUIRE(vec && a.wp6 && a.pieces == 2 && a.wide && per_wg <= WP_NPRE && NB <= 4, CV_EINVAL,
                   "hl-format input needs the fp16-pair weights, Cin %% 32 == 0, 16-byte aligned operands and at most %d "
                   "kernel offsets per workgroup", WP_NPRE);
        const int hd_mask = (int)g_opt_hd_mask.load(std::memory_order_relaxed);
        const long long hd_min_rows = g_opt_hd_min_rows.load(std::memory_order_relaxed);
        const int hd_shape = (int)g_opt_hd_shape.load(std::memory_order_relaxed);
        if constexpr (NB <= 3) {
            if (((hd_mask >> (NB - 1)) & 1) && a.n_out >= hd_min_rows && !ax.xcd_tiles) {
                ConvArgs ah = a;
                ah.tickets = nullptr;
                const int nw = hd_shape == 1 ? 4 : 8;
                dim3 g((unsigned)((a.n_out + nw * 32 - 1) / (nw * 32)), grid.y, grid.z);
                if (hd_shape == 1) conv_hd<NB, 4, 2><<<g, 256, 0, st>>>(ah);
                else if (hd_shape == 2) conv_hd<NB, 8, 2><<<g, 512, 0, st>>>(ah);
                else conv_hd<NB, 8, 3><<<g, 512, 0, st>>>(ah);
                CV_LAUNCH_CHECK();
                if (a.splits > 1) return launch_finish(a, st);
                return CV_OK;
            }
        }
        if (!(ax.splits > 1 && !ax.perm_per_split && !ax.xcd_tiles && (long long)gridx.x * gridx.y <= CV_SPLIT_TICKETS))
            ax.tickets = nullptr;
        conv_hl<NB><<<gridx, THREADS, 0, st>>>(ax);
        CV_LAUNCH_CHECK();
        if (a.splits > 1 && !ax.tickets) return launch_finish(a, st);
        return CV_OK;
    }
    if (vec && a.wp6 && per_wg <= WP_NPRE) {
        if (a.pieces == 2) conv_rows_wp<NB, 2><<<gridx, THREADS, 0, st>>>(ax);
        else if (a.pieces == 1) conv_rows_wp<NB, 1><<<gridx, THREADS, 0, st>>>(ax);
        else conv_rows_wp<NB, 3><<<gridx, THREADS, 0, st>>>(ax);
        CV_LAUNCH_CHECK();
        if (a.splits > 1) return launch_finish(a, st);
        return CV_OK;
    }
    if (vec && a.wp6 && per_wg <= WP_NPRE_BIG) {
        if (a.pieces == 2) conv_rows_wp<NB, 2, WP_NPRE_BIG><<<gridx, THREADS, 0, st>>>(ax);
        else if (a.pieces == 1) conv_rows_wp<NB, 1, WP_NPRE_BIG><<<gridx, THREADS, 0, st>>>(ax);
        else conv_rows_wp<NB, 3, WP_NPRE_BIG><<<gridx, THREADS, 0, st>>>(ax);
        CV_LAUNCH_CHECK();
        if (a.splits > 1) return launch_finish(a, st);
        return CV_OK;
    }
    CV_REQUIRE(a.pieces != 1 || !(vec && a.wp6), CV_EINVAL, "the bf16 compute mode takes at most %d kernel offsets per workgroup", WP_NPRE_BIG);
    if (vec) conv_rows<NB, true><<<grid, THREADS, 0, st>>>(a);
    else conv_rows<NB, false><<<grid, THREADS, 0, st>>>(a);
    CV_LAUNCH_CHECK();
    if (a.splits > 1) return launch_finish(a, st);
    return CV_OK;
}

}
namespace cvsc {
int nb_full(int cout) { return cout <= 32 ? 1 : cout <= 64 ? 2 : cout <= 96 ? 3 : 4; }
}
namespace {
int nb_for(int cout) {
    static const int nb_max = getenv("CV_NB_MAX") ? atoi(getenv("CV_NB_MAX")) : 0;
    if (nb_max > 0) return std::min(nb_max, nb_full(cout));
    if (cout <= 32) return 1;
    if (cout <= 64) return 2;
    if (cout <= 96) return 3;
    static const int nb_wide = getenv("CV_NB_WIDE") ? atoi(getenv("CV_NB_WIDE")) : 2;
    return std::max(1, std::min(nb_wide, 2));
}

std::atomic<long long> g_split_target{-1};
thread_local long long t_split_target = 0;
long long process_split_target() {
    long long v = g_split_target.load(std::memory_order_relaxed);
    if (v <= 0) {
        v = getenv("CV_SPLIT_TARGET") ? std::max(1ll, atoll(getenv("CV_SPLIT_TARGET"))) : 768;
        g_split_target.store(v, std::memory_order_relaxed);
    }
    return v;
}
long long split_target() { return t_split_target > 0 ? t_split_target : process_split_target(); }

int pick_splits(long long n_out, int cout, int K, int cin, bool vec) {
    const int nb = nb_for(cout);
    const long long tiles = ((n_out + TM - 1) / TM) * ((cout + nb * 32 - 1) / (nb * 32));
    const long long units = vec ? (long long)K * (cin / KC) : ((long long)K * cin + KC - 1) / KC;
    if (tiles >= 384 || units <= 1) return 1;
    const long long target = split_target();
    long long s = (target + tiles - 1) / tiles;
    s = std::min(s, units);
    static const long long traffic_mb = getenv("CV_SPLIT_TRAFFIC_MB") ? atoll(getenv("CV_SPLIT_TRAFFIC_MB")) : 24;
    const long long by_traffic = (traffic_mb << 20) / std::max<long long>(1, n_out * cout * 4);
    s = std::min(s, std::max<long long>(by_traffic, 2));
    s = std::min<long long>(s, 64);
    return (int)std::max<long long>(s, 1);
}

}

int cv_sp_set_option(const char* name, long long value, long long* previous) {
    CV_REQUIRE(name, CV_EINVAL, "null option name");
    std::atomic<long long>* o = !strcmp(name, "hd_mask") ? &g_opt_hd_mask : !strcmp(name, "hd_min_rows") ? &g_opt_hd_min_rows :
                                !strcmp(name, "hd_shape") ? &g_opt_hd_shape : !strcmp(name, "zskip") ? &g_opt_zskip : nullptr;
    CV_REQUIRE(o, CV_EINVAL, "unknown option '%s' (hd_mask, hd_min_rows, hd_shape, zskip)", name);
    const long long before = o->exchange(value, std::memory_order_relaxed);
    if (previous) *previous = before;
    return CV_OK;
}

int cv_sp_get_option(const char* name, long long* value) {
    CV_REQUIRE(name && value, CV_EINVAL, "null option name / value");
    const std::atomic<long long>* o = !strcmp(name, "hd_mask") ? &g_opt_hd_mask : !strcmp(name, "hd_min_rows") ? &g_opt_hd_min_rows :
                                      !strcmp(name, "hd_shape") ? &g_opt_hd_shape : !strcmp(name, "zskip") ? &g_opt_zskip : nullptr;
    CV_REQUIRE(o, CV_EINVAL, "unknown option '%s'", name);
    *value = o->load(std::memory_order_relaxed);
    return CV_OK;
}

int cv_sp_set_ablation(int bits) { return cvsc::g_ablation.exchange(bits, std::memory_order_relaxed); }

int cv_sp_set_split_target_thread(int workgroups) {
    const int before = (int)t_split_target;
    t_split_target = workgroups > 0 ? workgroups : 0;
    return before;
}

int cv_sp_set_split_target(int workgroups) {
    const int before = (int)process_split_target();
    g_split_target.store(workgroups > 0 ? workgroups : -1, std::memory_order_relaxed);
    return before;
}

int cv_sp_mask_perms_batch(const CvPermJob* jobs, int n_jobs, void* d_ws, size_t ws_bytes, void* stream, bool pre_zeroed) {
    CV_REQUIRE(jobs && d_ws && n_jobs > 0 && n_jobs <= CV_MAX_PERM_JOBS, CV_EINVAL, "bad mask perm batch");
    PermJobsDev d;
    d.n = n_jobs;
    int groups = 0;
    long long max_n = 0;
    for (int i = 0; i < n_jobs; ++i) {
        const CvPermJob& j = jobs[i];
        CV_REQUIRE(j.nbr && j.perm && j.n > 0 && j.K > 0 && j.groups >= 1 && j.groups <= j.K, CV_EINVAL,
                   "bad mask perm job %d", i);
        CV_REQUIRE((j.K + j.groups - 1) / j.groups <= 10, CV_EINVAL, "at most 10 kernel offsets per group");
        CV_REQUIRE(!j.mask_words || j.K <= 32, CV_EINVAL, "validity words hold at most 32 kernel offsets");
        d.j[i] = j;
        d.group_begin[i] = groups;
        groups += j.groups;
        max_n = std::max(max_n, j.n);
    }
    d.group_begin[n_jobs] = groups;
    CV_REQUIRE(ws_bytes >= sizeof(int) * (size_t)groups * MP_BINS * 2, CV_ENOMEM, "workspace too small");
    hipStream_t st = static_cast<hipStream_t>(stream);
    int* hist = static_cast<int*>(d_ws);
    int* cursor = hist + (size_t)groups * MP_BINS;
    if (!pre_zeroed) CV_HIP_CHECK(hipMemsetAsync(hist, 0, sizeof(int) * (size_t)groups * MP_BINS * 2, st));
    dim3 grid((unsigned)((max_n + MP_THREADS - 1) / MP_THREADS), (unsigned)groups);
    mp_hist_batch<<<grid, MP_THREADS, 0, st>>>(d, hist);
    CV_LAUNCH_CHECK();
    mp_scatter_batch<<<grid, MP_THREADS, 0, st>>>(d, hist, cursor);
    CV_LAUNCH_CHECK();
    return CV_OK;
}

extern "C" {

size_t cv_sp_conv_workspace_bytes(long long n_out, int cout, int K) {
    if (n_out <= 0 || cout <= 0 || K <= 0) return 0;
    const size_t one = sizeof(float) * (size_t)n_out * (size_t)cout;
    return 256 + std::min<size_t>(64 * one, std::max<size_t>((size_t)48 << 20, 3 * one));
}

int cv_sp_conv_f32(const cv_conv_desc* d, void* stream) {
    CV_REQUIRE(d, CV_EINVAL, "null descriptor");
    CV_REQUIRE(d->in && d->weight && d->out, CV_EINVAL, "null pointer argument");
    CV_REQUIRE(d->n_in > 0 && d->n_out > 0 && d->cin > 0 && d->cout > 0 && d->K > 0, CV_EINVAL, "bad conv sizes");
    CV_REQUIRE(d->nbr || (d->K == 1 && d->n_in == d->n_out), CV_EINVAL, "a kernel map is required unless K == 1");
    CV_REQUIRE(d->in_ld >= d->cin && d->out_ld >= d->cout && (!d->residual || d->res_ld >= d->cout) &&
                   (!d->acc_in || d->acc_ld >= d->cout), CV_EINVAL, "bad leading dimension");
    CV_REQUIRE(d->out != d->in, CV_EINVAL, "conv cannot run in place");
    const int jb = d->j_begin, je = d->j_end > 0 ? d->j_end : d->K;
    CV_REQUIRE(jb >= 0 && jb < je && je <= d->K, CV_EINVAL, "bad kernel offset range");
    hipStream_t st = static_cast<hipStream_t>(stream);
    ConvArgs a{d->in, d->n_in, d->in_ld, d->cin, d->weight, d->K, d->cout, d->nbr, d->n_out, d->scale,
               d->shift, d->residual, d->res_ld, d->relu, d->out, d->out_ld, 1, nullptr, d->row_perm, 0, jb, je,
               d->acc_in, d->acc_ld, d->plan_ent, d->plan_cnt,
               reinterpret_cast<const float4*>(d->weight_packed), 0, nullptr, 0, 0,
               static_cast<const unsigned short*>(d->weight_x6), d->in2, d->in2_ld, d->cin2,
               static_cast<const unsigned short*>(d->weight2_x6), d->weight_pieces == 2 ? 2 : d->weight_pieces == 1 ? 1 : 3,
               d->acc_scale != 0.f ? d->acc_scale : 1.f, d->range_flag, d->in_hl, d->out_hl, d->res_hl, 0, d->split_tickets};
    if (d->in_hl || d->out_hl || d->res_hl) {
        CV_REQUIRE(!d->in_hl || (d->weight_pieces == 2 && d->cin % 32 == 0 && d->in_ld % 32 == 0 &&
                                 (reinterpret_cast<uintptr_t>(d->in) & 127) == 0 &&
                                 (!d->in2 || (d->cin2 % 32 == 0 && d->in2_ld % 32 == 0 &&
                                              (reinterpret_cast<uintptr_t>(d->in2) & 127) == 0))),
                   CV_EINVAL, "hl-format input: fp16-pair weights, channels and leading dimensions %% 32 == 0, 128-byte aligned rows");
        CV_REQUIRE(!d->out_hl || (d->cout % 32 == 0 && d->out_ld % 32 == 0 && (reinterpret_cast<uintptr_t>(d->out) & 127) == 0),
                   CV_EINVAL, "hl-format output: Cout and leading dimension %% 32 == 0, 128-byte aligned rows");
        CV_REQUIRE(!d->res_hl || !d->residual || (d->res_ld % 32 == 0 && (reinterpret_cast<uintptr_t>(d->residual) & 127) == 0),
                   CV_EINVAL, "hl-format residual: leading dimension %% 32 == 0, 128-byte aligned rows");
        CV_REQUIRE(d->flavour == 0, CV_EINVAL, "the hl format runs with flavour 0 only");
        CV_REQUIRE(!d->in_hl || ((unsigned long long)d->n_in * (unsigned long long)d->in_ld * 4ull + (unsigned long long)d->cin * 4ull < (1ull << 32) &&
                                 (!d->in2 || (unsigned long long)d->n_out * (unsigned long long)d->in2_ld * 4ull + (unsigned long long)d->cin2 * 4ull < (1ull << 32))),
                   CV_EINVAL, "hl-format input larger than 4 GiB (rows x leading dimension x 4): split the batch");
    }
    CV_REQUIRE(d->weight_pieces >= 0 && d->weight_pieces <= 3, CV_EINVAL,
               "weight_pieces is 0/3 (bf16 triples), 2 (fp16 pairs) or 1 (single bf16 product)");
    CV_REQUIRE(d->weight_pieces != 1 || (d->weight_x6 && d->cin % KC == 0), CV_EINVAL,
               "weight_pieces = 1 needs weight_x6 from cv_sp_pack_weights_bf16_f32 and Cin %% 32 == 0");
    const bool stem_h2 = d->weight_pieces == 2 && d->weight_x6 && d->cout == 32 && (d->cin == 3 || d->cin == 6) && d->K <= 128;
    CV_REQUIRE(d->weight_pieces != 2 || stem_h2 || (d->weight_x6 && d->cin % KC == 0), CV_EINVAL,
               "weight_pieces = 2 needs weight_x6 from cv_sp_pack_weights_h2_f32 and Cin %% 32 == 0 (or the stem shape with "
               "cv_sp_pack_weights_stem_h2_f32)");

    if (!d->in_hl) a.tickets = nullptr;
    CV_REQUIRE(!d->plan_ent && !d->plan_cnt && !d->weight_packed && (d->flavour == 0 || d->flavour == 1), CV_EINVAL,
               "flavours 3 / 4 (the experimental wave / tile kernels of rounds 1-3) are gone: flavour is 0 or 1, plan_ent / plan_cnt / "
               "weight_packed must be NULL");
    a.wide = d->cout % 4 == 0 && d->out_ld % 4 == 0 && (!d->residual || d->res_ld % 4 == 0) &&
             (!d->acc_in || d->acc_ld % 4 == 0) &&
             ((reinterpret_cast<uintptr_t>(d->out) | reinterpret_cast<uintptr_t>(d->residual) |
               reinterpret_cast<uintptr_t>(d->acc_in) | reinterpret_cast<uintptr_t>(d->scale) |
               reinterpret_cast<uintptr_t>(d->shift) | reinterpret_cast<uintptr_t>(d->ws)) & 15) == 0;
    CV_REQUIRE(a.wide || (!d->out_hl && !d->res_hl), CV_EINVAL,
               "hl-format output / residual: Cout, leading dimensions %% 4 == 0 and 16-byte aligned out, residual, acc_in, "
               "scale, shift and ws");
    const bool vec = (d->cin % KC == 0) && (d->in_ld % 4 == 0) && (d->cout % 4 == 0) &&
                     ((reinterpret_cast<uintptr_t>(d->in) & 15) == 0) &&
                     ((reinterpret_cast<uintptr_t>(d->weight) & 15) == 0);
    CV_REQUIRE(!d->weight_x6 || vec || stem_h2, CV_EINVAL,
               "weight_x6 needs the vector path: Cin %% 32 == 0, Cout %% 4 == 0, in_ld %% 4 == 0, 16-byte aligned in / weight");
    if (d->in2) {
        CV_REQUIRE(vec && d->weight_x6 && d->weight2_x6 && d->cin2 > 0 && d->cin2 % KC == 0 && d->in2_ld >= d->cin2 &&
                       d->in2_ld % 4 == 0 && (reinterpret_cast<uintptr_t>(d->in2) & 15) == 0,
                   CV_EINVAL, "a second source needs the bf16x6 vector path (weight_x6, weight2_x6, Cin2 %% 32 == 0, "
                              "16-byte aligned rows)");
    }
    if (!vec && d->cout == 32 && (d->cin == 3 || d->cin == 6) && d->nbr && !d->row_perm && d->perm_groups <= 1 &&
        d->flavour == 0) {
        if (d->weight_x6 && d->weight_pieces == 2 && d->K <= 128 && a.wide && !d->acc_in && d->j_begin == 0 &&
            (d->j_end == 0 || d->j_end == d->K)) {
            const unsigned gm = (unsigned)((d->n_out + TM - 1) / TM);
            if (d->cin == 3) conv_stem_mfma<3><<<gm, THREADS, 0, st>>>(a);
            else conv_stem_mfma<6><<<gm, THREADS, 0, st>>>(a);
            CV_LAUNCH_CHECK();
            return CV_OK;
        }
    }
    a.acc_scale_dev = d->acc_scale_dev;
    if (d->perm_groups > 1) {
        const size_t need = sizeof(float) * (size_t)d->perm_groups * (size_t)d->n_out * (size_t)d->cout;
        CV_REQUIRE(d->row_perm && vec && d->ws && d->ws_bytes >= need, CV_EINVAL,
                   "perm_groups needs row_perm[groups][n_out], Cin %% 32 == 0 and a workspace of %zu bytes", need);
        a.splits = d->perm_groups;
        a.perm_per_split = 1;
        a.partial = static_cast<float*>(d->ws);
        if (d->perm_has_map && jb == 0 && je == d->K && d->nbr) {
            a.nbr_perm = d->row_perm + (long long)d->perm_groups * d->n_out;
            a.nbr_perm_w = (d->K + d->perm_groups - 1) / d->perm_groups;
            if (g_opt_zskip.load(std::memory_order_relaxed) && !d->in2 && a.wide && d->perm_groups <= FINISH_SMALL_MAX && d->in_hl)
                a.gvalid = reinterpret_cast<const unsigned char*>(a.nbr_perm + (long long)d->perm_groups * d->n_out * a.nbr_perm_w);
        }
    } else if (d->flavour == 0) {
        int sp = pick_splits(d->n_out, d->cout, je - jb, d->cin, vec);
        if (d->in_hl || (vec && a.wp6)) {
            const int nj = je - jb;
            const int per_wg = sp <= 1 ? nj : (nj + sp - 1) / sp + 1;
            if (per_wg > WP_NPRE) sp = std::max(sp, (nj + WP_NPRE - 2) / (WP_NPRE - 1));
        }
        const size_t need = sizeof(float) * (size_t)sp * (size_t)d->n_out * (size_t)d->cout;
        CV_REQUIRE(!d->in_hl || sp <= 1 || (d->ws && d->ws_bytes >= need), CV_ENOMEM,
                   "hl-format convolution needs a workspace of %zu bytes (cv_sp_conv_workspace_bytes)", need);
        if (sp > 1 && d->ws && d->ws_bytes >= need) {
            a.splits = sp;
            a.partial = static_cast<float*>(d->ws);
        }
    }
    switch (nb_for(d->cout)) {
        case 1: return launch_rows<1>(a, vec, st);
        case 2: return launch_rows<2>(a, vec, st);
        case 3: return launch_rows<3>(a, vec, st);
        default: return launch_rows<4>(a, vec, st);
    }
}

int cv_sp_mask_keys(const int32_t* d_nbr, long long n, int K, int j_begin, int j_end, long long* d_keys,
                    void* stream) {
    CV_REQUIRE(d_nbr && d_keys && n > 0 && K > 0 && j_begin >= 0 && j_begin < j_end && j_end <= K &&
                   j_end - j_begin <= 63, CV_EINVAL, "bad mask key arguments");
    hipStream_t st = static_cast<hipStream_t>(stream);
    mask_keys<<<(unsigned)((n + 255) / 256), 256, 0, st>>>(d_nbr, n, K, j_begin, j_end, d_keys);
    CV_LAUNCH_CHECK();
    return CV_OK;
}

int cv_sp_mask_perms(const int32_t* d_nbr, long long n, int K, int groups, int32_t* d_perm, void* d_ws,
                     size_t ws_bytes, int with_map, void* stream) {
    CV_REQUIRE(d_nbr && d_perm && d_ws && n > 0 && K > 0 && groups >= 1 && groups <= K, CV_EINVAL,
               "bad mask perm arguments");
    CV_REQUIRE((K + groups - 1) / groups <= 10, CV_EINVAL, "at most 10 kernel offsets per group");
    CV_REQUIRE(ws_bytes >= sizeof(int) * (size_t)groups * MP_BINS, CV_ENOMEM, "workspace too small");
    hipStream_t st = static_cast<hipStream_t>(stream);
    int* hist = static_cast<int*>(d_ws);
    CV_HIP_CHECK(hipMemsetAsync(hist, 0, sizeof(int) * (size_t)groups * MP_BINS, st));
    dim3 grid((unsigned)((n + MP_THREADS - 1) / MP_THREADS), (unsigned)groups);
    mp_hist<<<grid, MP_THREADS, 0, st>>>(d_nbr, n, K, groups, hist);
    CV_LAUNCH_CHECK();
    mp_scan<<<groups, MP_BINS, 0, st>>>(hist);
    CV_LAUNCH_CHECK();
    mp_scatter<<<grid, MP_THREADS, 0, st>>>(d_nbr, n, K, groups, hist, d_perm,
                                            with_map ? d_perm + (long long)groups * n : nullptr, (K + groups - 1) / groups);
    CV_LAUNCH_CHECK();
    return CV_OK;
}

int cv_sp_pack_weights_x6_f32(const float* d_w, int K, int cin, int cout, const float* d_col_scale, void* d_wp6,
                              void* stream) {
    CV_REQUIRE(d_w && d_wp6 && K > 0 && cin > 0 && cout > 0, CV_EINVAL, "bad pack_weights_x6 arguments");
    CV_REQUIRE(cin % 32 == 0, CV_EINVAL, "pack_weights_x6 needs Cin %% 32 == 0 (got %d)", cin);
    CV_REQUIRE((reinterpret_cast<uintptr_t>(d_wp6) & 15) == 0, CV_EINVAL, "d_wp6 must be 16-byte aligned");
    hipStream_t st = static_cast<hipStream_t>(stream);
    const long long total = (long long)K * cin * cout / 2;
    pack_weights_x6<<<(unsigned)std::min<long long>((total + 255) / 256, 8192), 256, 0, st>>>(
        d_w, K, cin, cout, d_col_scale, static_cast<unsigned short*>(d_wp6));
    CV_LAUNCH_CHECK();
    return CV_OK;
}
// ... 429 lines not shown
```

### canonicalvoting_amd/csrc/sparse_conv_common.h

```cpp
#pragma once
#include "cv_common.h"

#include <type_traits>
#include <utility>

namespace cvsc {

typedef float f32x16 __attribute__((ext_vector_type(16)));

constexpr int KC = 32;
constexpr int TM = 128;
constexpr int A_LD = TM + 2;
constexpr int THREADS = 256;

struct ConvArgs {
    const float* in; long long n_in; int in_ld; int cin;
    const float* w; int K; int cout;
    const int* nbr; long long n_out;
    const float* scale; const float* shift;
    const float* res; int res_ld;
    int relu;
    float* out; int out_ld;
    int splits;
    float* partial;
    const int* row_perm;
    int perm_per_split;
    int j_begin, j_end;
    const float* acc_in;
    int acc_ld;
    const int* plan_ent;
    const int* plan_cnt;
    const float4* wp;
    int wide;
    const int* nbr_perm;
    int nbr_perm_w;
    int reserved0;
    const unsigned short* wp6;
    const float* in2;
    int in2_ld, cin2;
    const unsigned short* wp6_2;
    int pieces;
    float acc_scale;
    int* range_flag;
    int in_hl, out_hl, res_hl;
    int xcd_tiles;
    int* tickets;
    const float* acc_scale_dev;
    const unsigned char* gvalid;
};

__device__ __forceinline__ void hl_split2(float x0, float x1, unsigned& h, unsigned& l);
__device__ __forceinline__ float4 hl_load4(const float* row, int col) {
    const unsigned char* p = reinterpret_cast<const unsigned char*>(row) + (col >> 5) * 128 + (col & 31) * 2;
    const uint2 h = *reinterpret_cast<const uint2*>(p), l = *reinterpret_cast<const uint2*>(p + 64);
    typedef _Float16 h2 __attribute__((ext_vector_type(2)));
    const h2 h0 = __builtin_bit_cast(h2, h.x), h1 = __builtin_bit_cast(h2, h.y), l0 = __builtin_bit_cast(h2, l.x),
             l1 = __builtin_bit_cast(h2, l.y);
    return make_float4((float)h0[0] + (float)l0[0], (float)h0[1] + (float)l0[1], (float)h1[0] + (float)l1[0],
                       (float)h1[1] + (float)l1[1]);
}
__device__ __forceinline__ void hl_store4(float* row, int col, float4 v) {
    unsigned h0, l0, h1, l1;
    hl_split2(v.x, v.y, h0, l0);
    hl_split2(v.z, v.w, h1, l1);
    unsigned char* p = reinterpret_cast<unsigned char*>(row) + (col >> 5) * 128 + (col & 31) * 2;
    *reinterpret_cast<uint2*>(p) = make_uint2(h0, h1);
    *reinterpret_cast<uint2*>(p + 64) = make_uint2(l0, l1);
}
__device__ __forceinline__ bool hl_out_of_range(float4 v) {
    return fmaxf(fmaxf(fabsf(v.x), fabsf(v.y)), fmaxf(fabsf(v.z), fabsf(v.w))) > 65000.f;
}

typedef float f32x4v __attribute__((ext_vector_type(4)));
__device__ __forceinline__ void partial_store4(float* p, float4 v) {
    f32x4v t; t[0] = v.x; t[1] = v.y; t[2] = v.z; t[3] = v.w;
    __builtin_nontemporal_store(t, reinterpret_cast<f32x4v*>(p));
}
__device__ __forceinline__ void partial_store4_wt(float* p, float4 v) {
    f32x4v t; t[0] = v.x; t[1] = v.y; t[2] = v.z; t[3] = v.w;
    asm volatile("global_store_dwordx4 %0, %1, off sc1\n\ts_nop 1" :: "v"(p), "v"(t) : "memory");
}
__device__ __forceinline__ float4 partial_load4(const float4* p) {
    const f32x4v t = __builtin_nontemporal_load(reinterpret_cast<const f32x4v*>(p));
    return make_float4(t[0], t[1], t[2], t[3]);
}

__device__ __forceinline__ void epilogue_store(const ConvArgs& a, const f32x16& acc, const int* rows,
                                               int col, int lane) {
    if (col >= a.cout) return;
    if (a.splits > 1) {
        float* p = a.partial + (long long)blockIdx.z * a.n_out * a.cout;
#pragma unroll
        for (int r = 0; r < 16; ++r) {
            const int row = rows[(r & 3) + 8 * (r >> 2) + 4 * (lane >> 5)];
            if (row >= 0) p[(long long)row * a.cout + col] = acc[r];
        }
        return;
    }
    const float sc = a.scale ? a.scale[col] : 1.f;
    const float sh = a.shift ? a.shift[col] : 0.f;
#pragma unroll
    for (int r = 0; r < 16; ++r) {
        const int row = rows[(r & 3) + 8 * (r >> 2) + 4 * (lane >> 5)];
        if (row < 0) continue;
        float v = acc[r];
        if (a.acc_in) v += a.acc_in[(long long)row * a.acc_ld + col];
        v = v * sc + sh;
        if (a.res) v += a.res[(long long)row * a.res_ld + col];
        if (a.relu) v = fmaxf(v, 0.f);
        a.out[(long long)row * a.out_ld + col] = v;
    }
}

__device__ __forceinline__ void epilogue_apply4(const ConvArgs& a, long long row, int col, float4 v) {
    if (a.acc_in) {
        const float4 p = *reinterpret_cast<const float4*>(a.acc_in + row * a.acc_ld + col);
        v.x += p.x; v.y += p.y; v.z += p.z; v.w += p.w;
    }
    const float4 sc = a.scale ? *reinterpret_cast<const float4*>(a.scale + col) : make_float4(1.f, 1.f, 1.f, 1.f);
    const float4 sh = a.shift ? *reinterpret_cast<const float4*>(a.shift + col) : make_float4(0.f, 0.f, 0.f, 0.f);
    v.x = v.x * sc.x + sh.x; v.y = v.y * sc.y + sh.y; v.z = v.z * sc.z + sh.z; v.w = v.w * sc.w + sh.w;
    if (a.res) {
        const float4 p = a.res_hl ? hl_load4(a.res + row * a.res_ld, col)
                                  : *reinterpret_cast<const float4*>(a.res + row * a.res_ld + col);
        v.x += p.x; v.y += p.y; v.z += p.z; v.w += p.w;
    }
    if (a.relu) { v.x = fmaxf(v.x, 0.f); v.y = fmaxf(v.y, 0.f); v.z = fmaxf(v.z, 0.f); v.w = fmaxf(v.w, 0.f); }
    if (a.out_hl) {
        if (a.range_flag && hl_out_of_range(v)) *a.range_flag = 1;
        hl_store4(a.out + row * a.out_ld, col, v);
    } else {
        *reinterpret_cast<float4*>(a.out + row * a.out_ld + col) = v;
    }
}

constexpr int EP_LD = 36;
__device__ __forceinline__ void epilogue_store_wide(const ConvArgs& a, const f32x16& acc, const int* rows, int colbase,
                                                    int lane, float (*T)[EP_LD]) {
    const int h = lane >> 5, c = lane & 31;
#pragma unroll
    for (int r = 0; r < 16; ++r) T[(r & 3) + 8 * (r >> 2) + 4 * h][c] = acc[r];
    __builtin_amdgcn_fence(__ATOMIC_RELEASE, "wavefront");
    __builtin_amdgcn_wave_barrier();
    __builtin_amdgcn_fence(__ATOMIC_ACQUIRE, "wavefront");
    const int col = colbase + (lane & 7) * 4;
    if (col < a.cout) {
#pragma unroll
        for (int it = 0; it < 4; ++it) {
            const int rl = (lane >> 3) + 8 * it;
            const int row = rows[rl];
            if (row < 0) continue;
            float4 v = *reinterpret_cast<const float4*>(&T[rl][(lane & 7) * 4]);
            if (a.splits > 1) {
                float* pp = a.partial + ((long long)blockIdx.z * a.n_out + row) * a.cout + col;
                if (a.tickets) partial_store4_wt(pp, v);
                else partial_store4(pp, v);
                continue;
            }
            epilogue_apply4(a, row, col, v);
        }
    }
    __builtin_amdgcn_wave_barrier();
}

typedef short bf16x8 __attribute__((ext_vector_type(8)));

typedef __bf16 bf16x2v __attribute__((ext_vector_type(2)));
typedef float f32x2v __attribute__((ext_vector_type(2)));
__device__ __forceinline__ unsigned cvt_pk_bf16(float lo, float hi) {
    const f32x2v v = {lo, hi};
    return __builtin_bit_cast(unsigned, __builtin_convertvector(v, bf16x2v));
}
__device__ __forceinline__ void split3(float x0, float x1, unsigned& h, unsigned& m, unsigned& l) {
    h = cvt_pk_bf16(x0, x1);
    const float r0 = x0 - __uint_as_float(h << 16), r1 = x1 - __uint_as_float(h & 0xffff0000u);
    m = cvt_pk_bf16(r0, r1);
    const float s0 = r0 - __uint_as_float(m << 16), s1 = r1 - __uint_as_float(m & 0xffff0000u);
    l = cvt_pk_bf16(s0, s1);
}

typedef _Float16 f16x2 __attribute__((ext_vector_type(2)));
typedef _Float16 f16x8 __attribute__((ext_vector_type(8)));
__device__ __forceinline__ void split2h(float x0, float x1, unsigned& h, unsigned& l) {
    const f16x2 hv = {(_Float16)x0, (_Float16)x1};
    h = __builtin_bit_cast(unsigned, hv);
    float r0, r1;
    asm("v_fma_mix_f32 %0, %1, -1.0, %2 op_sel_hi:[1,0,0]" : "=v"(r0) : "v"(h), "v"(x0));
    asm("v_fma_mix_f32 %0, %1, -1.0, %2 op_sel:[1,0,0] op_sel_hi:[1,0,0]" : "=v"(r1) : "v"(h), "v"(x1));
    const f16x2 lv = {(_Float16)r0, (_Float16)r1};
    l = __builtin_bit_cast(unsigned, lv);
}

__device__ __forceinline__ void hl_split2(float x0, float x1, unsigned& h, unsigned& l) { split2h(x0, x1, h, l); }


template <int... I, class F>
__device__ __forceinline__ void static_for_impl(std::integer_sequence<int, I...>, F&& f) {
    (f(std::integral_constant<int, I>{}), ...);
}
template <int N, class F>
__device__ __forceinline__ void static_for(F&& f) { static_for_impl(std::make_integer_sequence<int, N>{}, f); }

static __device__ __attribute__((aligned(128))) unsigned char g_zero_chunk[128];
// ... 50 lines not shown
```

### canonicalvoting_amd/me/__init__.py

```python
import ctypes
import math
import os
import threading

import numpy as np
import torch
import torch.nn as nn

from .. import _lib
from . import utils

__version__ = "0.5.3-cvhip"


def _ptr(t):
    return ctypes.c_void_p(t.data_ptr() if t is not None else 0)


def _stream(dev):
    return ctypes.c_void_p(torch._C._cuda_getCurrentRawStream(dev.index if dev.index is not None else torch.cuda.current_device()))


class _NoSwitch:
    def __enter__(self):
# ... 214 lines not shown
            keys = [kbuf[i * cap:(i + 1) * cap] for i in range(NL)]
            vals = [ibuf[o:o + cap] for o in lay.vals]
            cm_s = CoordinateManager._from_levels(coords_buf, keys, vals, ibuf[o_counts:o_counts + 8], c, cap)
            arena = ibuf[o_arena:]
            view = lambda o, r, k: arena[o:o + r * k].view(r, k)
            stem_map = view(off.stem, c[0], stem_k ** 3)
            out_map = ibuf[o_inv:o_inv + n].view(n, 1)
            for i in range(4):
                cm_s._maps[("k", 2, 1 << i, 2)] = view(off.down[i], c[i + 1], 8)
                cm_s._maps[("up", 16 >> i)] = view(off.up[i], c[3 - i], 8)
                cm_s._maps[("upperm", 16 >> i)] = arena[off.up_perm[i]:off.up_perm[i] + c[3 - i]]
            for i in range(5):
                cm_s._maps[("k", 3, 1 << i, 1)] = view(off.k3[i], c[i], 27)
                if off.mask_perm[i] >= 0:
                    mp = view(off.mask_perm[i], G, c[i])
                    mp._cv_has_map = True
                    mp._cv_from_plan = True
                    cm_s._maps[("mp", 3, 1 << i, G)] = mp
                    cm_s._maps[("k", 3, 1 << i, 1)]._cv_mask_perms = mp
            plan.views = (cm_s, stem_map, out_map)
        return plan.views

    def num_rows(self, ts):
        if ts == 1:
            return self._input.shape[0]
        if ts not in self._level:
            self.ensure_levels()
        return self.counts[self._level[ts]]

    def kernel_map(self, k, ts_in, stride=1):
        if ts_in * stride not in self._level:
            self.ensure_levels()
        self._verify()
        key = ("k", k, ts_in, stride)
        m = self._maps.get(key)
        if m is None:
            L = _lib.lib()
            li = self._level[ts_in]
            out = self.coords[ts_in * stride]
            m = torch.empty((out.shape[0], k ** 3), dtype=torch.int32, device=self.device)
            with torch.cuda.device(self.device):
                _lib.check(L.cv_sp_kernel_map(_ptr(out), out.shape[0], _ptr(self._keys[li]),
                                              _ptr(self._vals[li]), self.cap, k, ts_in, _ptr(m),
                                              _stream(self.device)), "cv_sp_kernel_map")
            self._maps[key] = m
        return m

    def up_map(self, ts_coarse):
        key = ("up", ts_coarse)
        m = self._maps.get(key)
        if m is None:
            L = _lib.lib()
            down = self.kernel_map(2, ts_coarse // 2, 2)
            n_fine = self.num_rows(ts_coarse // 2)
            m = torch.empty((n_fine, 8), dtype=torch.int32, device=self.device)
            with torch.cuda.device(self.device):
                _lib.check(L.cv_sp_up_map(_ptr(down), down.shape[0], n_fine, _ptr(m), _stream(self.device)),
                           "cv_sp_up_map")
            self._maps[key] = m
        return m


class SparseTensor:

    def __init__(self, features, coordinates=None, device=None, coordinate_manager=None, tensor_stride=1,
                 **_):
        if device is None:
            device = features.device if coordinates is None else (
                features.device if features.is_cuda else torch.device("cuda"))
        device = torch.device(device)
        if device.type != "cuda":
            raise RuntimeError("canonicalvoting_amd SparseTensor runs on the GPU only (no CPU engine); "
                               "pass device='cuda'")
        self.F = features.to(device=device, dtype=torch.float32)
        self.F_hl = None
        if coordinate_manager is None:
            if coordinates is None:
                raise ValueError("coordinates or coordinate_manager required")
            c = coordinates
            if c.is_floating_point():
                c = torch.floor(c)
            coordinate_manager = CoordinateManager(c.to(device=device, dtype=torch.int32).contiguous(),
                                                   num_levels=1, check=False, lazy=True)
        self.coordinate_manager = coordinate_manager
        self.tensor_stride = tensor_stride if isinstance(tensor_stride, int) else int(tensor_stride[0])
        if self.F.shape[0] != coordinate_manager.num_rows(self.tensor_stride):
            raise RuntimeError("features have %d rows, coordinate set has %d" % (
                self.F.shape[0], coordinate_manager.num_rows(self.tensor_stride)))

    @property
    def C(self):
        cm = self.coordinate_manager
        if self.tensor_stride not in cm.coords:
            cm.ensure_levels()
        return cm.coords[self.tensor_stride]

    @property
    def coordinates(self):
        return self.C

    @property
    def features(self):
        return self.F

    @property
    def device(self):
        return self.F.device

    @property
    def shape(self):
        return self.F.shape

    def __len__(self):
        return self.F.shape[0]

    @property
    def decomposed_coordinates_and_features(self):
        C, Fm = self.C, self.F
        nb = int(C[:, 0].max().item()) + 1
        cs, fs = [], []
        for b in range(nb):
            m = C[:, 0] == b
            cs.append(C[m][:, 1:])
            fs.append(Fm[m])
        return cs, fs

    def _like(self, F, tensor_stride=None, F_hl=None):
        t = SparseTensor(F, coordinate_manager=self.coordinate_manager,
                         tensor_stride=self.tensor_stride if tensor_stride is None else tensor_stride)
        t.F_hl = F_hl
        return t


def _workspace(dev, nbytes):
    return _lib.scratch(dev, "conv_ws", nbytes)


_range_flags = {}
_range_lock = threading.Lock()


def range_flag(dev):
    key = (dev, torch.cuda.current_stream(dev).cuda_stream)
    with _range_lock:
        f = _range_flags.get(key)
        if f is None:
            f = _range_flags[key] = torch.zeros(1, dtype=torch.int32).pin_memory()
    return f


def conv_forward(x_feats, weight, nbr, n_out, scale=None, shift=None, residual=None, relu=False,
                 out=None, flavour=0, row_perm=None, j_begin=0, j_end=0, acc_in=None, perm_groups=0,
                 cache_weights=True, pieces=None, in_hl=False, out_hl=False, res_hl=False, stem_mfma=False,
                 split_tickets=None, weight_t=False, acc_scale_dev=None):
    if pieces is None:
        pieces = 1 if COMPUTE_DTYPE == "bf16" else 3
    L = _lib.lib()
    dev = x_feats.device
    w = weight if weight.dim() == 3 else weight[None]
    if weight_t:
        K, cout, cin = w.shape
        x6_ok = CONV_X6 and flavour in (0, 1) and cin % 32 == 0 and cout % 4 == 0 and pieces in (1, 2, 3)
        if not x6_ok:
            w = w.permute(0, 2, 1)
            weight_t = False
    else:
        K, cin, cout = w.shape
    assert x_feats.shape[1] == cin and x_feats.stride(1) == 1
    w = w.contiguous()
    if out is None:
        out = torch.empty((n_out, cout), dtype=torch.float32, device=dev)
    if (AUTO_MASK_GROUPS > 1 and row_perm is None and perm_groups == 0 and flavour == 0 and nbr is not None
            and K == 27 and n_out >= AUTO_MASK_MIN_ROWS and cin % 32 == 0 and j_begin == 0 and j_end == 0
            and acc_in is None):
        row_perm = map_mask_perms(nbr, AUTO_MASK_GROUPS)
        perm_groups = row_perm.shape[0]
    wp6 = None
    acc_scale, flag = 0.0, None
    if CONV_X6 and flavour in (0, 1) and cin % 32 == 0 and cout % 4 == 0:
        if pieces == 2 and weight_t:
            pk = _bwd_ctx.get("packed")
            pre = pk.get((w.data_ptr(), 1)) if pk else None
            if pre is not None and pre[0].numel() == 2 * w.numel():
                wp6, k = pre
                TRAIN_COUNTERS["prepacked"] += 1
            else:
                hints = _bwd_ctx.get("pair_scales")
                k = hints.get(weight.data_ptr()) if hints is not None else None
                if k is None:
                    k = h2_scale_log2((w, None))
                wp6 = torch.empty(2 * w.numel(), dtype=torch.int16, device=dev)
                with _on(dev):
                    _lib.check(L.cv_sp_pack_weights_t_f32(_ptr(w), K, cout, cin, 2, int(k), _ptr(wp6), _stream(dev)),
                               "cv_sp_pack_weights_t_f32")
            acc_scale, flag = 2.0 ** -k, range_flag(dev)
        elif pieces == 2:
            key = id(weight)
            ver = (weight.data_ptr(), weight._version, tuple(weight.shape))
            hit = _packed_h2.get(key) if cache_weights else None
            pk = _bwd_ctx.get("packed") if not cache_weights else None
            pre = pk.get((w.data_ptr(), 0)) if pk else None
            if pre is not None and pre[0].numel() == 2 * w.numel():
                hit = (ver, pre[0], pre[1])
                TRAIN_COUNTERS["prepacked"] += 1
            elif hit is None or hit[0] != ver:
                hints = getattr(_train_state, "pair_scales", None)
                k = hints.get(weight.data_ptr()) if hints is not None else None
                if k is None:
                    k = h2_scale_log2((w, None))
                hit = (ver, packed_weights_h2(w, None, k), k)
                if cache_weights:
                    if len(_packed_h2) > 512:
                        _packed_h2.clear()
                    _packed_h2[key] = hit
            wp6, acc_scale, flag = hit[1], 2.0 ** -hit[2], range_flag(dev)
        elif weight_t:
            wp6 = torch.empty((3 if pieces == 3 else 1) * w.numel(), dtype=torch.int16, device=dev)
            with _on(dev):
                _lib.check(L.cv_sp_pack_weights_t_f32(_ptr(w), K, cout, cin, pieces, 0, _ptr(wp6), _stream(dev)),
                           "cv_sp_pack_weights_t_f32")
        elif pieces == 1:
            wp6 = packed_weights_bf16(w)
        else:
            wp6 = packed_weights_x6(weight, w, cache_weights)
    if stem_mfma and pieces == 2 and cin in (3, 6) and cout == 32 and K <= 128 and nbr is not None and flavour == 0:
        hints = getattr(_train_state, "pair_scales", None) if scale is None else None
        k = hints.get(weight.data_ptr()) if hints is not None else None
        if k is None:
            k = h2_scale_log2((w, scale))
        wp6, acc_scale, flag, scale = packed_weights_stem_h2(w, scale, k), 2.0 ** -k, range_flag(dev), None
    ws = None
    if perm_groups > 1:
        ws = _workspace(dev, 4 * perm_groups * n_out * cout + 256)
    elif flavour == 0 and n_out < 128 * 384:
        ws = _workspace(dev, int(L.cv_sp_conv_workspace_bytes(n_out, cout, K)))
    p = lambda t: t.data_ptr() if t is not None else None
    d = _lib.ConvDesc(p(x_feats), x_feats.shape[0], x_feats.stride(0), cin, p(w), K, cout, p(nbr), n_out,
                      p(scale), p(shift), p(residual), residual.stride(0) if residual is not None else 0,
                      1 if relu else 0, p(out), out.stride(0), flavour, p(ws),
                      ws.numel() if ws is not None else 0, p(row_perm), j_begin, j_end, p(acc_in),
                      acc_in.stride(0) if acc_in is not None else 0, perm_groups,
                      None, None, None, p(wp6), None, 0, 0, None,
                      1 if (perm_groups > 1 and getattr(row_perm, "_cv_has_map", False)) else 0,
                      2 if flag is not None else (1 if (pieces == 1 and wp6 is not None) else 0), acc_scale, p(flag),
                      1 if in_hl else 0, 1 if out_hl else 0, 1 if res_hl else 0, p(split_tickets), p(acc_scale_dev))
    with _on(dev):
        _lib.check(L.cv_sp_conv_f32(ctypes.byref(d), _stream(dev)), "cv_sp_conv_f32")
    return out


_policy_tls = threading.local()


def masked_min_rows():
    v = getattr(_policy_tls, "masked_min_rows", None)
    return CoordinateManager.MASKED_MIN_ROWS if v is None else v


def set_masked_min_rows_thread(rows):
    before = getattr(_policy_tls, "masked_min_rows", None)
    _policy_tls.masked_min_rows = None if rows is None else int(rows)
    return before


def set_split_target(workgroups):
    return int(_lib.lib().cv_sp_set_split_target(int(workgroups)))


def set_option(name, value):
    import ctypes
    prev = ctypes.c_longlong(0)
    _lib.check(_lib.lib().cv_sp_set_option(name.encode(), int(value), ctypes.byref(prev)), "cv_sp_set_option")
    return int(prev.value)


def option(name):
    v = ctypes.c_longlong(0)
    _lib.check(_lib.lib().cv_sp_get_option(name.encode(), ctypes.byref(v)), "cv_sp_get_option")
    return int(v.value)


def to_hl(x):
    y = torch.empty((x.shape[0], x.shape[1]), dtype=torch.float32, device=x.device)
    with _on(x.device):
        _lib.check(_lib.lib().cv_sp_to_hl_f32(x.data_ptr(), x.shape[0], x.shape[1], x.stride(0), y.data_ptr(), y.stride(0),
                                              range_flag(x.device).data_ptr(), _stream(x.device)), "cv_sp_to_hl_f32")
    return y


def from_hl(x):
    y = torch.empty((x.shape[0], x.shape[1]), dtype=torch.float32, device=x.device)
    with _on(x.device):
        _lib.check(_lib.lib().cv_sp_from_hl_f32(x.data_ptr(), x.shape[0], x.shape[1], x.stride(0), y.data_ptr(),
                                                y.stride(0), _stream(x.device)), "cv_sp_from_hl_f32")
    return y


AUTO_MASK_GROUPS = int(os.environ.get("CV_MASK_GROUPS", "4"))
AUTO_MASK_MIN_ROWS = int(os.environ.get("CV_AUTO_MASK_MIN_ROWS", "16384"))


def map_mask_perms(nbr, groups):
    hit = getattr(nbr, "_cv_mask_perms", None)
    if hit is not None and getattr(hit, "_cv_from_plan", False):
        return hit
    if hit is None or hit.shape[0] != groups:
        hit = nbr._cv_mask_perms = _perms_with_map(nbr, groups)
    return hit


def _perms_with_map(nbr, groups):
    L = _lib.lib()
    n, K = nbr.shape
    W = (K + groups - 1) // groups
    flat = torch.empty(groups * n * (1 + W) + (groups * n + 3) // 4, dtype=torch.int32, device=nbr.device)
    ws = torch.empty(groups * 4096, dtype=torch.uint8, device=nbr.device)
    with _on(nbr.device):
        _lib.check(L.cv_sp_mask_perms(_ptr(nbr), n, K, groups, _ptr(flat), _ptr(ws), ws.numel(), 1,
                                      _stream(nbr.device)), "cv_sp_mask_perms")
    m = flat[:groups * n].view(groups, n)
    m._cv_has_map = True
    m._cv_flat = flat
    return m


_packed = {}
_packed_x6 = {}
_packed_h2 = {}
CONV_X6 = os.environ.get("CV_CONV_X6", "1") != "0"


COMPUTE_DTYPE = "bf16" if os.environ.get("CV_COMPUTE_DTYPE", "fp32") == "bf16" else "fp32"


def set_compute_dtype(dtype):
    global COMPUTE_DTYPE
    assert dtype in ("fp32", "bf16"), dtype
    prev, COMPUTE_DTYPE = COMPUTE_DTYPE, dtype
    return prev


def packed_weights_bf16(w3, col_scale=None):
    L = _lib.lib()
    K, cin, cout = w3.shape
    wp = torch.empty(w3.numel(), dtype=torch.int16, device=w3.device)
    with _on(w3.device):
        _lib.check(L.cv_sp_pack_weights_bf16_f32(_ptr(w3), K, cin, cout, _ptr(col_scale), _ptr(wp),
                                                 _stream(w3.device)), "cv_sp_pack_weights_bf16_f32")
    return wp


def invalidate_weight_caches():
    _packed.clear()
    _packed_x6.clear()
    _packed_h2.clear()


def packed_weights_x6_scaled(w3, col_scale):
    L = _lib.lib()
    K, cin, cout = w3.shape
    wp = torch.empty(3 * w3.numel(), dtype=torch.int16, device=w3.device)
    with _on(w3.device):
        _lib.check(L.cv_sp_pack_weights_x6_f32(_ptr(w3), K, cin, cout, _ptr(col_scale), _ptr(wp), _stream(w3.device)),
                   "cv_sp_pack_weights_x6_f32")
    return wp


def h2_scale_log2(*scaled_weights):
    import math
    amax = 0.0
    for w3, col_scale in scaled_weights:
        a = w3.abs().amax(dim=(0, 1)) if col_scale is not None else w3.abs().max()
        amax = max(amax, float((a * col_scale.abs()).max()) if col_scale is not None else float(a))
    if not math.isfinite(amax) or amax <= 0.0:
        return 0
    return max(-60, min(60, 13 - math.ceil(math.log2(amax))))


def packed_weights_h2(w3, col_scale, scale_log2):
    L = _lib.lib()
    K, cin, cout = w3.shape
    wp = torch.empty(2 * w3.numel(), dtype=torch.int16, device=w3.device)
    with _on(w3.device):
        _lib.check(L.cv_sp_pack_weights_h2_f32(_ptr(w3), K, cin, cout, _ptr(col_scale), int(scale_log2), _ptr(wp),
                                               _stream(w3.device)), "cv_sp_pack_weights_h2_f32")
    return wp


def packed_weights_stem_h2(w3, col_scale, scale_log2):
    L = _lib.lib()
    K, cin, cout = w3.shape
    assert cout == 32
    wp = torch.empty(8 * cin * 1024, dtype=torch.int16, device=w3.device)
    with _on(w3.device):
        _lib.check(L.cv_sp_pack_weights_stem_h2_f32(_ptr(w3), K, cin, _ptr(col_scale), int(scale_log2), _ptr(wp),
                                                    _stream(w3.device)), "cv_sp_pack_weights_stem_h2_f32")
    return wp

# ... 657 lines not shown
```

### include/cv_hip.h

```cpp
#ifndef CV_HIP_H
#define CV_HIP_H

#include <stddef.h>
#include <stdint.h>

#ifdef __cplusplus
extern "C" {
#endif

#define CV_OK 0
#define CV_EINVAL (-22)
#define CV_ENOMEM (-12)
#define CV_EHIP (-5)
#define CV_ERANGE (-34)

#define CV_ABI_VERSION 4
int cv_abi_version(void);
const char* cv_last_error(void);


size_t cv_hv_minmax_workspace_bytes(void);
int cv_hv_minmax_f32(const float* d_points, int64_t n, float* h_min3, float* h_max3,
                     void* d_ws, size_t ws_bytes, void* stream);
int cv_hv_minmax_async_f32(const float* d_points, int64_t n, float* h_minmax6, void* d_ws, size_t ws_bytes,
                           void* stream);

int cv_hv_grid_dims_f32(const float h_min3[3], const float h_max3[3], float res, int dims_out[3]);

size_t cv_hv_forward_workspace_bytes(int64_t n, int num_rots, const int dims[3], int algo);

int cv_hv_forward_f32(const float* d_points, const float* d_xyz, const float* d_scale,
                      const float* d_obj, int64_t n, float res, int num_rots,
                      const float h_corner3[3], const int dims[3], float* d_grid_obj,
                      float* d_grid_rot, float* d_grid_scale, void* d_ws, size_t ws_bytes,
                      int algo, void* stream);

#define CV_MAX_CATEGORIES 16
size_t cv_hv_forward_cat_workspace_bytes(int64_t n, int num_rots, const int dims[3], int algo, int num_cats);
int cv_hv_forward_cat_f32(const float* d_points, const float* d_xyz, const float* d_scale, const float* d_obj, int64_t n,
                          float res, int num_rots, const float h_corner3[3], const int dims[3], int num_cats, float* d_grid_obj,
                          float* d_grid_rot, float* d_grid_scale, void* d_ws, size_t ws_bytes, int algo, void* stream);

int cv_hv_set_part_records(int records);
int cv_hv_set_part_records_thread(int records);
int cv_hv_set_kernel_events(void* ev_start, void* ev_stop);

int cv_hv_backward_f32(const float* d_grad_obj, const float* d_points, const float* d_xyz,
                       const float* d_scale, const float* d_obj, int64_t n, float res,
                       int num_rots, const float h_corner3[3], const int dims[3], float* d_dxyz,
                       float* d_dscale, float* d_dobj, void* stream);

int cv_hv_count_votes_f32(const float* d_points, const float* d_xyz, const float* d_scale, int64_t n,
                          float res, int num_rots, const float h_corner3[3], const int dims[3],
                          int64_t* h_count, void* d_ws, size_t ws_bytes, void* stream);

typedef struct cv_decode_params {
    float thresh_high;
    float thresh_low;
    float valid_ratio;
    int elimination;
    float prob_thresh;
    int elim_hi_plus1;
    int max_iters;
    double err_thresh;
} cv_decode_params;

size_t cv_decode_workspace_bytes(const int dims[3], int64_t n, int max_iters);

int cv_decode_f32(float* d_grid_obj, const float* d_grid_rot, const float* d_grid_scale,
                  const int dims[3], const float h_corner3[3], float res, const float* d_points,
                  const float* d_xyz, const float* d_prob, const int32_t* d_class, int64_t n,
                  const cv_decode_params* params, int mutate_grid, void* d_ws, size_t ws_bytes,
                  int* h_n_cand, int64_t* h_cand_idx, int32_t* h_verdict, int* h_n_boxes,
                  float* h_boxes, float* h_scores, int32_t* h_classes, int* h_truncated, void* stream);

size_t cv_decode_cat_workspace_bytes(const int dims[3], int64_t n, int max_iters, int num_cats);
int cv_decode_cat_f32(float* d_grid_obj, const float* d_grid_rot, const float* d_grid_scale, const int dims[3],
                      const float h_corner3[3], float res, const float* d_points, const float* d_xyz, const float* d_prob,
                      const int32_t* d_class, int64_t n, int num_cats, const cv_decode_params* params, int mutate_grid, void* d_ws,
                      size_t ws_bytes, int* h_n_cand, int64_t* h_cand_idx, int32_t* h_verdict, int* h_n_boxes, float* h_boxes,
                      float* h_scores, int32_t* h_classes, int* h_truncated, void* stream);

double cv_iou_obb(const float* h_box1, const float* h_box2);
int cv_nms_obb(const float* h_boxes, const float* h_scores, int n, double thr, int32_t* h_pick);


long long cv_sp_table_capacity(long long n);
size_t cv_sp_levels_workspace_bytes(long long n);

int cv_sp_build_levels(int32_t* const* d_coords, unsigned long long* const* d_keys,
                       int32_t* const* d_vals, long long n, long long cap, int num_levels,
                       int32_t* d_counts, int32_t* h_counts, void* d_ws, size_t ws_bytes, void* stream);

#define CV_QUANTIZE_MAX_CLOUDS 256
size_t cv_sp_quantize_workspace_bytes(long long m);
int cv_sp_quantize_f32(const float* d_points, long long m, long long ld, float quantization_size, int floor_only,
                       const long long* h_offsets, int n_clouds, int32_t* d_coords4, int32_t* d_index, int32_t* d_inverse,
                       int32_t* d_counts, int32_t* h_counts, void* d_ws, size_t ws_bytes, void* stream);
int cv_sp_quantize_f64(const double* d_points, long long m, long long ld, double quantization_size, int floor_only,
                       const long long* h_offsets, int n_clouds, int32_t* d_coords4, int32_t* d_index, int32_t* d_inverse,
                       int32_t* d_counts, int32_t* h_counts, void* d_ws, size_t ws_bytes, void* stream);

size_t cv_sp_sort_workspace_bytes(long long n);
int cv_sp_sort_rows(const int32_t* d_coords, long long n, int32_t* d_sorted, int32_t* d_perm, int32_t* d_inv,
                    void* d_ws, size_t ws_bytes, void* stream);

int cv_sp_morton_keys(const int32_t* d_coords, long long n, long long* d_keys, void* stream);

int cv_sp_kernel_map(const int32_t* d_out_coords, long long n_out, const unsigned long long* d_keys,
                     const int32_t* d_vals, long long cap, int k, int ts, int32_t* d_nbr, void* stream);

int cv_sp_up_map(const int32_t* d_nbr_down, long long n_coarse, long long n_fine, int32_t* d_up,
                 void* stream);

typedef struct cv_conv_desc {
    const float* in;
    long long n_in;
    int in_ld, cin;
    const float* weight;
    int K, cout;
    const int32_t* nbr;
    long long n_out;
    const float* scale;
    const float* shift;
    const float* residual;
    int res_ld;
    int relu;
    float* out;
    int out_ld;
    int flavour;
    void* ws;
    size_t ws_bytes;
    const int32_t* row_perm;
    int j_begin, j_end;
    const float* acc_in;
    int acc_ld;
    int perm_groups;
    const int32_t* plan_ent;
    const int32_t* plan_cnt;
    const float* weight_packed;
    const void* weight_x6;
    const float* in2;
    int in2_ld, cin2;
    const void* weight2_x6;
    int perm_has_map;
    int weight_pieces;
    float acc_scale;
    int32_t* range_flag;
    int in_hl, out_hl, res_hl;
    int32_t* split_tickets;
    const float* acc_scale_dev;
} cv_conv_desc;
#define CV_SPLIT_TICKETS 4096

int cv_sp_to_hl_f32(const float* d_x, long long n, int c, int x_ld, float* d_y, int y_ld, int32_t* range_flag, void* stream);
int cv_sp_from_hl_f32(const float* d_x, long long n, int c, int x_ld, float* d_y, int y_ld, void* stream);

int cv_sp_pack_weights_x6_f32(const float* d_w, int K, int cin, int cout, const float* d_col_scale, void* d_wp6,
                              void* stream);
int cv_sp_pack_weights_h2_f32(const float* d_w, int K, int cin, int cout, const float* d_col_scale, int scale_log2,
                              void* d_wp, void* stream);
typedef struct cv_pack_job {
    const float* w;
    void* wp;
    int K, cin, cout;
    int trans;
    int scale_log2;
    int reserved;
} cv_pack_job;
int cv_sp_pack_weights_h2_batch_f32(const cv_pack_job* h_jobs, int n_jobs, void* d_jobs, void* stream);
int cv_sp_pack_weights_bf16_f32(const float* d_w, int K, int cin, int cout, const float* d_col_scale, void* d_wp,
                                void* stream);
int cv_sp_pack_weights_t_f32(const float* d_w, int K, int rows, int cols, int pieces, int scale_log2, void* d_wp, void* stream);
int cv_sp_pack_weights_stem_h2_f32(const float* d_w, int K, int cin, const float* d_col_scale, int scale_log2, void* d_wp,
                                   void* stream);

size_t cv_sp_conv_workspace_bytes(long long n_out, int cout, int K);
int cv_sp_conv_f32(const cv_conv_desc* desc, void* stream);

int cv_sp_set_split_target(int workgroups);
int cv_sp_set_split_target_thread(int workgroups);
int cv_sp_set_ablation(int bits);
int cv_sp_set_option(const char* name, long long value, long long* previous);
int cv_sp_get_option(const char* name, long long* value);

typedef struct cv_scene_maps {
    long long stem, out, down[4], k3[5], up[4], mask_perm[5], up_perm[4], scratch;
    long long bitmap;
} cv_scene_maps;
size_t cv_sp_scene_maps_words(const long long* level_rows, long long n_orig, int stem_k, int mask_groups,
                              long long masked_min_rows, cv_scene_maps* offsets);
int cv_sp_scene_maps(int32_t* const* d_coords, const unsigned long long* const* d_keys, const int32_t* const* d_vals,
                     long long cap, const long long* level_rows, const int32_t* d_perm, long long n_orig, int stem_k,
                     int mask_groups, long long masked_min_rows, int32_t* d_arena, size_t arena_words, void* stream);

size_t cv_sp_scene_plan_words(long long n, int stem_k, int mask_groups, long long masked_min_rows);
int cv_sp_scene_plan(const int32_t* d_input, long long n, int32_t* d_perm, int32_t* d_inv, int32_t* const* d_coords,
                     unsigned long long* const* d_keys, int32_t* const* d_vals, long long cap, int32_t* d_counts,
                     int32_t* h_counts, int stem_k, int mask_groups, long long masked_min_rows, int32_t* d_arena,
                     size_t arena_words, cv_scene_maps* offsets, void* d_sort_ws, size_t sort_ws_bytes, void* d_levels_ws,
                     size_t levels_ws_bytes, void* stream);

typedef struct cv_scene_plan_layout {
    long long cap;
    long long perm, inv, coords[5], vals[5], counts, arena;
    long long int_words, key_words;
    size_t sort_ws_bytes, levels_ws_bytes;
} cv_scene_plan_layout;
int cv_sp_scene_plan_layout(long long n, int stem_k, int mask_groups, long long masked_min_rows, cv_scene_plan_layout* out);
#define CV_NET_MAP_SLOTS 15
#define CV_NET_PERM_SLOTS 9
int cv_sp_scene_plan_slots(const cv_scene_plan_layout* layout, const cv_scene_maps* offsets, const long long* level_rows,
                           long long min_rows, const int32_t* d_ibuf, const int32_t** maps, const int32_t** perms);
size_t cv_sp_scene_conv_workspace_bytes(const long long* level_rows, const int* masked, int mask_groups, int max_channels);

typedef struct cv_net_buf {
    int level, channels, rows_level;
    int hl;
} cv_net_buf;
typedef struct cv_net_op {
    int in_buf, in_col, cin;
    int out_buf, out_col, cout;
    int res_buf, res_col;
    int map, K;
    int perm, perm_groups;
    int relu;
    const float* weight;
    const float* scale;
    const float* shift;
    const void* weight_x6;
    int in2_buf, in2_col, cin2;
    const void* weight2_x6;
    int weight_pieces;
    float acc_scale;
} cv_net_op;
size_t cv_net_arena_bytes(const cv_net_buf* bufs, int n_bufs, const long long* level_rows, int n_levels);
int cv_net_run_f32(const cv_net_op* ops, int n_ops, const cv_net_buf* bufs, int n_bufs, const long long* level_rows,
                   int n_levels, void* d_arena, size_t arena_bytes, const void* const* ext_ptr, const int* ext_ld,
                   const int32_t* const* maps, int n_maps, const int32_t* const* perms, int n_perms,
                   void* d_ws, size_t ws_bytes, int32_t* range_flag, void* stream);

int cv_sp_mask_keys(const int32_t* d_nbr, long long n, int K, int j_begin, int j_end, long long* d_keys,
                    void* stream);

int cv_sp_mask_perms(const int32_t* d_nbr, long long n, int K, int groups, int32_t* d_perm, void* d_ws,
                     size_t ws_bytes, int with_map, void* stream);

int cv_sp_transpose_map(const int32_t* d_nbr, long long n_out, int K, long long n_in, int32_t* d_nbr_t, void* stream);
size_t cv_sp_wgrad_workspace_bytes(long long n_out, int cin, int cout, int K);
int cv_sp_conv_wgrad_f32(const float* d_x, int x_ld, int cin, const float* d_dy, int dy_ld, int cout,
                         const int32_t* d_nbr, int K, long long n_out, float* d_dw, void* d_ws, size_t ws_bytes,
                         void* stream);
int cv_sp_conv_wgrad_px_f32(const float* d_x, int x_ld, int cin, const float* d_dy, int dy_ld, int cout,
                            const int32_t* d_nbr, int K, long long n_out, float* d_dw, void* d_ws, size_t ws_bytes,
                            int pieces, void* stream);
int cv_sp_col_sum_f32(const float* d_x, long long n, int c, int ld, float* d_out, void* stream);
size_t cv_sp_col_sum_workspace_bytes(long long n, int c);
int cv_sp_col_sum_det_f32(const float* d_x, long long n, int c, int ld, float* d_out, void* d_ws, size_t ws_bytes,
                          void* stream);

size_t cv_sp_bn_workspace_bytes(int c);
int cv_sp_bn_stats_f32(const float* d_x, long long n, int c, int ld, const float* d_gamma, const float* d_beta,
                       float eps, float momentum, float* d_running_mean, float* d_running_var, float* d_mean,
                       float* d_var, float* d_scale, float* d_shift, void* d_ws, size_t ws_bytes, void* stream);
int cv_sp_bn_backward_f32(const float* d_x, const float* d_dy, const float* d_y, long long n, int c, int ld,
                          const float* d_mean, const float* d_var, float eps, const float* d_gamma, float* d_dgamma,
                          float* d_dbeta, float* d_dx, float* d_dres, void* d_ws, size_t ws_bytes, void* stream);

#define CV_BN_SLOT_WORDS 8200
int cv_sp_bn_backward_hl_f32(const float* d_x, const float* d_dy, const float* d_y, long long n, int c, int ld,
                             const float* d_mean, const float* d_var, float eps, const float* d_gamma, float* d_dgamma,
                             float* d_dbeta, float* d_dx, float* d_dres, void* d_ws, size_t ws_bytes, float* d_dx_hl,
                             uint32_t* d_slot, int32_t* range_flag, const uint32_t* d_relu_bits, void* stream);

int cv_sp_copy_unless_flag(const void* const* h_src, void* const* h_dst, const long long* h_bytes, int n, const int32_t* flag,
                           void* stream);

int cv_sp_affine_f32(const float* d_x, long long n, int c, int x_ld, const float* d_scale,
                     const float* d_shift, const float* d_residual, int res_ld, int relu, float* d_y, int y_ld,
                     void* stream);
int cv_sp_affine_hl_f32(const float* d_x, long long n, int c, int x_ld, const float* d_scale, const float* d_shift,
                        const float* d_residual, int res_ld, int relu, float* d_y, int y_ld, float* d_y_hl, int y_hl_ld,
                        uint32_t* d_relu_bits, int32_t* range_flag, void* stream);

int cv_sp_bn_fold_f32(const float* d_gamma, const float* d_beta, const float* d_mean, const float* d_var,
                      const float* d_bias, float eps, int c, float* d_scale, float* d_shift, void* stream);

int cv_head_joint_f32(const float* d_feats, long long n, int ld, int nclasses, int log_scale, float* d_xyz,
                      float* d_scale, float* d_prob, int32_t* d_class, void* stream);

int cv_head_separate_f32(const float* d_feats, long long n, int ld, int log_scale, float* d_xyz, float* d_scale,
                         float* d_prob, void* stream);

typedef struct cv_scene_desc {
    const int32_t* d_coords4;
    long long n;
    const float* d_feats;
    int feats_ld;
    const float* d_points;
    float res;
    int num_rots;
    const cv_net_op* ops; int n_ops;
    const cv_net_buf* bufs; int n_bufs;
    int stem_k, mask_groups;
    long long masked_min_rows;
    int max_channels;
    int use_range_flag;
    float* d_out_feats;
    int out_ld, out_channels;
    int nclasses, log_scale;
    const float* d_xyz_in; const float* d_scale_in; const float* d_prob_in; const int32_t* d_class_in;
    int vote_algo;
    cv_decode_params decode;
    int max_candidates;
    double nms_threshold;
    void* d_ws; size_t ws_bytes;
    float* d_grids; size_t grid_capacity_floats;
    void* h_pinned; size_t pinned_bytes;
    int64_t* h_cand_idx; int32_t* h_verdict;
    float* h_boxes; float* h_scores; int32_t* h_classes;
    int32_t* h_pick;
    int adaptive_split;
    void* events[5];
    int conv_split_target;
    int vote_part_records;
} cv_scene_desc;
typedef struct cv_scene_result {
    int n_cand, n_boxes, n_det, truncated, range_flag, duplicates, out_of_window;
    int scenes_in_flight;
    int dims[3];
    float corner[3];
    long long level_rows[5];
    size_t needed_ws_bytes, needed_grid_floats;
    float* d_grid_obj; float* d_grid_rot; float* d_grid_scale;
    float* d_xyz; float* d_scale; float* d_prob; int32_t* d_class;
    float host_us[4];
} cv_scene_result;
int cv_detect_scene_f32(const cv_scene_desc* desc, cv_scene_result* result, void* stream);

typedef struct cv_scene_separate_desc {
    const int32_t* d_coords4; long long n;
    const float* d_feats; int feats_ld;
    const float* d_points; float res; int num_rots;
    int num_models;
    const cv_net_op* const* ops; const int* n_ops;
    const cv_net_buf* const* bufs; const int* n_bufs;
    int stem_k, mask_groups;
    long long masked_min_rows;
    int max_channels;
    int use_range_flag;
    float* const* d_out_feats;
    int out_ld, out_channels;
    int log_scale;
    const float* d_xyz_in; const float* d_scale_in; const float* d_prob_in;
    int vote_algo;
    cv_decode_params decode;
    int max_candidates;
    double nms_threshold;
    void* d_ws; size_t ws_bytes;
    void* h_pinned; size_t pinned_bytes;
    int64_t* h_cand_idx; int32_t* h_verdict;
    float* h_boxes; float* h_scores;
    int32_t* h_det_cat; int32_t* h_det_box;
    void* events[5];
    int conv_split_target, vote_part_records;
} cv_scene_separate_desc;
typedef struct cv_scene_separate_result {
    int n_cand[CV_MAX_CATEGORIES], n_boxes[CV_MAX_CATEGORIES], truncated[CV_MAX_CATEGORIES];
    int n_det, range_flag, duplicates, out_of_window;
    int dims[3];
    float corner[3];
    long long level_rows[5];
    size_t needed_ws_bytes;
    float* d_grid_obj; float* d_grid_rot; float* d_grid_scale;
    float* d_xyz; float* d_scale; float* d_prob;
    float host_us[4];
} cv_scene_separate_result;
int cv_detect_scene_separate_f32(const cv_scene_separate_desc* desc, cv_scene_separate_result* result, void* stream);

#ifdef __cplusplus
}
#endif
#endif
```

Before: 626.7.

## Fuse final 1x1 conv and voting head into the last conv's finish kernel

Detects the pattern of a K>1 conv followed by a 1x1 output conv and folds the 1x1 conv, its BN/ReLU and the joint/separate voting head into a new finish-tail kernel. The kernel loads the packed 1x1 weights into shared memory and consumes the previous layer's split-K partials directly. This avoids writing the intermediate feature map, a separate conv launch and a head launch. It adds a large new kernel with extra shared memory use and split-count limits, and falls back to the unfused path when the alignment, size or split conditions are not met.

```diff
diff --git a/canonicalvoting_amd/_lib.py b/canonicalvoting_amd/_lib.py
--- a/canonicalvoting_amd/_lib.py
+++ b/canonicalvoting_amd/_lib.py
@@ -10,7 +10,7 @@
 c_i32_p = ctypes.POINTER(ctypes.c_int32)
 c_i64_p = ctypes.POINTER(ctypes.c_int64)
 vp = ctypes.c_void_p
-ABI_VERSION = 4
+ABI_VERSION = 5
 
 
 class CvError(RuntimeError):
@@ -22,6 +22,19 @@
                 ("valid_ratio", ctypes.c_float), ("elimination", ctypes.c_int),
                 ("prob_thresh", ctypes.c_float), ("elim_hi_plus1", ctypes.c_int),
                 ("max_iters", ctypes.c_int), ("err_thresh", ctypes.c_double)]
+
+
+class ConvTail(ctypes.Structure):
+    _fields_ = [("weight", vp), ("weight_x6", vp), ("weight_pieces", ctypes.c_int), ("acc_scale", ctypes.c_float),
+                ("cout", ctypes.c_int), ("relu", ctypes.c_int), ("scale", vp), ("shift", vp), ("map", vp),
+                ("n_out", ctypes.c_longlong), ("out", vp), ("out_ld", ctypes.c_int), ("range_flag", vp),
+                ("head_kind", ctypes.c_int), ("nclasses", ctypes.c_int), ("log_scale", ctypes.c_int),
+                ("d_xyz", vp), ("d_scale", vp), ("d_prob", vp), ("d_class", vp)]
+
+
+class NetHead(ctypes.Structure):
+    _fields_ = [("kind", ctypes.c_int), ("nclasses", ctypes.c_int), ("log_scale", ctypes.c_int),
+                ("d_xyz", vp), ("d_scale", vp), ("d_prob", vp), ("d_class", vp)]
 
 
 class ConvDesc(ctypes.Structure):
@@ -35,7 +48,8 @@
                 ("weight_packed", vp), ("weight_x6", vp), ("in2", vp), ("in2_ld", ctypes.c_int), ("cin2", ctypes.c_int),
                 ("weight2_x6", vp), ("perm_has_map", ctypes.c_int), ("weight_pieces", ctypes.c_int),
                 ("acc_scale", ctypes.c_float), ("range_flag", vp), ("in_hl", ctypes.c_int), ("out_hl", ctypes.c_int),
-                ("res_hl", ctypes.c_int), ("split_tickets", vp), ("acc_scale_dev", vp)]
+                ("res_hl", ctypes.c_int), ("split_tickets", vp), ("acc_scale_dev", vp),
+                ("tail", ctypes.POINTER(ConvTail))]
 
 
 class SceneMaps(ctypes.Structure):
@@ -206,6 +220,10 @@
                                       c_i64_p, ctypes.c_int, vp, ctypes.c_size_t, ctypes.POINTER(vp), c_int_p,
                                       ctypes.POINTER(vp), ctypes.c_int, ctypes.POINTER(vp), ctypes.c_int,
                                       vp, ctypes.c_size_t, vp, vp]),
+    "cv_net_run_head_f32": (ctypes.c_int, [ctypes.POINTER(NetOp), ctypes.c_int, ctypes.POINTER(NetBuf), ctypes.c_int,
+                                           c_i64_p, ctypes.c_int, vp, ctypes.c_size_t, ctypes.POINTER(vp), c_int_p,
+                                           ctypes.POINTER(vp), ctypes.c_int, ctypes.POINTER(vp), ctypes.c_int,
+                                           vp, ctypes.c_size_t, vp, ctypes.POINTER(NetHead), vp]),
     "cv_sp_mask_keys": (ctypes.c_int, [vp, ctypes.c_longlong, ctypes.c_int, ctypes.c_int, ctypes.c_int, vp, vp]),
     "cv_sp_mask_perms": (ctypes.c_int, [vp, ctypes.c_longlong, ctypes.c_int, ctypes.c_int, vp, vp, ctypes.c_size_t,
                                         ctypes.c_int, vp]),
diff --git a/canonicalvoting_amd/csrc/net_exec.cpp b/canonicalvoting_amd/csrc/net_exec.cpp
--- a/canonicalvoting_amd/csrc/net_exec.cpp
+++ b/canonicalvoting_amd/csrc/net_exec.cpp
@@ -279,10 +279,23 @@
     return total;
 }
 
-int cv_net_run_f32(const cv_net_op* ops, int n_ops, const cv_net_buf* bufs, int n_bufs, const long long* level_rows,
+static bool tail_pattern(const cv_net_op* ops, int n_ops, const cv_net_buf* bufs, int n_levels, int k) {
+    if (k + 1 >= n_ops) return false;
+    const cv_net_op &p = ops[k], &c = ops[k + 1];
+    const bool ext_out = bufs[c.out_buf].level < 0 || bufs[c.out_buf].level >= n_levels;
+    if (!(c.K == 1 && c.in_buf == p.out_buf && c.in_col == 0 && p.out_col == 0 && c.cin == p.cout && bufs[p.out_buf].channels == p.cout &&
+          c.in2_buf < 0 && c.res_buf < 0 && c.weight_pieces == 2 && c.weight_x6 && c.perm < 0 && ext_out && !bufs[c.out_buf].hl &&
+          c.out_col == 0 && bufs[p.out_buf].hl && p.K > 1))
+        return false;
+    for (int j = k + 2; j < n_ops; ++j)
+        if (ops[j].in_buf == p.out_buf || ops[j].in2_buf == p.out_buf || ops[j].res_buf == p.out_buf) return false;
+    return true;
+}
+
+static int net_run(const cv_net_op* ops, int n_ops, const cv_net_buf* bufs, int n_bufs, const long long* level_rows,
                    int n_levels, void* d_arena, size_t arena_bytes, const void* const* ext_ptr, const int* ext_ld,
                    const int32_t* const* maps, int n_maps, const int32_t* const* perms, int n_perms,
-                   void* d_ws, size_t ws_bytes, int32_t* range_flag, void* stream) {
+                   void* d_ws, size_t ws_bytes, int32_t* range_flag, const cv_net_head* head, void* stream) {
     CV_REQUIRE(ops && bufs && level_rows && d_arena && n_ops > 0 && n_bufs > 0 && n_levels > 0, CV_EINVAL,
                "bad network program arguments");
     CV_REQUIRE(arena_bytes >= cv_net_arena_bytes(bufs, n_bufs, level_rows, n_levels), CV_ENOMEM, "arena too small");
@@ -303,13 +316,13 @@
             }
         }
     }
-    for (int k = 0; k < n_ops; ++k) {
+    auto describe = [&](int k, cv_conv_desc& d) -> int {
         const cv_net_op& o = ops[k];
+        d = {};
         CV_REQUIRE(o.in_buf >= 0 && o.in_buf < n_bufs && o.out_buf >= 0 && o.out_buf < n_bufs &&
                        o.res_buf < n_bufs && o.map < n_maps && o.perm < n_perms, CV_EINVAL, "op %d: bad slot", k);
         const Slot& in = slot[o.in_buf];
         const Slot& out = slot[o.out_buf];
-        cv_conv_desc d = {};
         d.in_hl = bufs[o.in_buf].hl;
         d.out_hl = bufs[o.out_buf].hl;
         d.res_hl = o.res_buf >= 0 ? bufs[o.res_buf].hl : 0;
@@ -351,10 +364,62 @@
             d.perm_groups = o.perm_groups;
             d.perm_has_map = o.perm_groups > 1;
         }
-        const int rc = cv_sp_conv_f32(&d, stream);
+        return CV_OK;
+    };
+    long long fuse = 1;
+    (void)cv_sp_get_option("tail_fuse", &fuse);
+    bool head_done = false;
+    for (int k = 0; k < n_ops; ++k) {
+        cv_conv_desc d;
+        int rc = describe(k, d);
         if (rc != CV_OK) return rc;
+        cv_conv_tail t = {};
+        if (fuse && tail_pattern(ops, n_ops, bufs, n_levels, k)) {
+            cv_conv_desc c;
+            rc = describe(k + 1, c);
+            if (rc != CV_OK) return rc;
+            t.weight = c.weight; t.weight_x6 = c.weight_x6; t.weight_pieces = c.weight_pieces; t.acc_scale = c.acc_scale;
+            t.cout = c.cout; t.relu = c.relu; t.scale = c.scale; t.shift = c.shift;
+            t.map = c.nbr; t.n_out = c.n_out; t.out = c.out; t.out_ld = c.out_ld; t.range_flag = c.range_flag;
+            if (head && k + 2 == n_ops) {
+                t.head_kind = head->kind; t.nclasses = head->nclasses; t.log_scale = head->log_scale;
+                t.d_xyz = head->d_xyz; t.d_scale = head->d_scale; t.d_prob = head->d_prob; t.d_class = head->d_class;
+                head_done = true;
+            }
+            d.tail = &t;
+            ++k;
+        }
+        rc = cv_sp_conv_f32(&d, stream);
+        if (rc != CV_OK) return rc;
+    }
+    if (head && !head_done) {
+        const Slot& y = slot[ops[n_ops - 1].out_buf];
+        const float* f = reinterpret_cast<const float*>(y.ptr) + ops[n_ops - 1].out_col;
+        if (head->kind == 1)
+            return cv_head_joint_f32(f, y.rows, y.ld, head->nclasses, head->log_scale, head->d_xyz, head->d_scale, head->d_prob,
+                                     head->d_class, stream);
+        return cv_head_separate_f32(f, y.rows, y.ld, head->log_scale, head->d_xyz, head->d_scale, head->d_prob, stream);
     }
     return CV_OK;
 }
 
-}
+int cv_net_run_f32(const cv_net_op* ops, int n_ops, const cv_net_buf* bufs, int n_bufs, const long long* level_rows,
+                   int n_levels, void* d_arena, size_t arena_bytes, const void* const* ext_ptr, const int* ext_ld,
+                   const int32_t* const* maps, int n_maps, const int32_t* const* perms, int n_perms,
+                   void* d_ws, size_t ws_bytes, int32_t* range_flag, void* stream) {
+    return net_run(ops, n_ops, bufs, n_bufs, level_rows, n_levels, d_arena, arena_bytes, ext_ptr, ext_ld, maps, n_maps, perms, n_perms,
+                   d_ws, ws_bytes, range_flag, nullptr, stream);
+}
+
+int cv_net_run_head_f32(const cv_net_op* ops, int n_ops, const cv_net_buf* bufs, int n_bufs, const long long* level_rows,
+                        int n_levels, void* d_arena, size_t arena_bytes, const void* const* ext_ptr, const int* ext_ld,
+                        const int32_t* const* maps, int n_maps, const int32_t* const* perms, int n_perms,
+                        void* d_ws, size_t ws_bytes, int32_t* range_flag, const cv_net_head* head, void* stream) {
+    CV_REQUIRE(head && (head->kind == 1 || head->kind == 2) && head->d_xyz && head->d_scale && head->d_prob &&
+                   (head->kind != 1 || (head->d_class && head->nclasses > 0)), CV_EINVAL, "bad head descriptor");
+    return net_run(ops, n_ops, bufs, n_bufs, level_rows, n_levels, d_arena, arena_bytes, ext_ptr, ext_ld, maps, n_maps, perms, n_perms,
+                   d_ws, ws_bytes, range_flag, head, stream);
+}
+
+
+}
diff --git a/canonicalvoting_amd/csrc/scene_exec.cpp b/canonicalvoting_amd/csrc/scene_exec.cpp
--- a/canonicalvoting_amd/csrc/scene_exec.cpp
+++ b/canonicalvoting_amd/csrc/scene_exec.cpp
@@ -171,13 +171,12 @@
 
     const void* ext_ptr[2] = {d->d_feats, d->d_out_feats};
     const int ext_ld[2] = {d->feats_ld, d->out_ld};
-    rc = cv_net_run_f32(d->ops, d->n_ops, d->bufs, d->n_bufs, f.rows, 5, arena, arena_b, ext_ptr, ext_ld, f.maps, CV_NET_MAP_SLOTS,
-                        f.perms, CV_NET_PERM_SLOTS, conv_ws, f.conv_ws_b, d->use_range_flag ? d_flag : nullptr, stream);
+    const cv_net_head head = {1, d->nclasses, d->log_scale, xyz, scale, prob, cls};
+    rc = cv_net_run_head_f32(d->ops, d->n_ops, d->bufs, d->n_bufs, f.rows, 5, arena, arena_b, ext_ptr, ext_ld, f.maps, CV_NET_MAP_SLOTS,
+                             f.perms, CV_NET_PERM_SLOTS, conv_ws, f.conv_ws_b, d->use_range_flag ? d_flag : nullptr, &head, stream);
     if (rc != CV_OK) return rc;
     clock.lap(1);
     CV_HIP_CHECK(clock.mark(1));
-    rc = cv_head_joint_f32(d->d_out_feats, n, d->out_ld, d->nclasses, d->log_scale, xyz, scale, prob, cls, stream);
-    if (rc != CV_OK) return rc;
     if (d->use_range_flag) CV_HIP_CHECK(hipMemcpyAsync(h_flag, d_flag, sizeof(int32_t), hipMemcpyDeviceToHost, st));
     r->d_xyz = xyz; r->d_scale = scale; r->d_prob = prob; r->d_class = cls;
     CV_HIP_CHECK(clock.mark(2));
@@ -280,18 +279,14 @@
     for (int k = 0; k < K; ++k) {
         const void* ext_ptr[2] = {d->d_feats, d->d_out_feats[k]};
         const int ext_ld[2] = {d->feats_ld, d->out_ld};
-        rc = cv_net_run_f32(d->ops[k], d->n_ops[k], d->bufs[k], d->n_bufs[k], f.rows, 5, arena, arena_b, ext_ptr, ext_ld, f.maps,
-                            CV_NET_MAP_SLOTS, f.perms, CV_NET_PERM_SLOTS, conv_ws, f.conv_ws_b,
-                            d->use_range_flag ? d_flags + 16 * k : nullptr, stream);
+        const cv_net_head head = {2, 0, d->log_scale, xyz + (size_t)k * n * 3, scale + (size_t)k * n * 3, prob + (size_t)k * n, nullptr};
+        rc = cv_net_run_head_f32(d->ops[k], d->n_ops[k], d->bufs[k], d->n_bufs[k], f.rows, 5, arena, arena_b, ext_ptr, ext_ld, f.maps,
+                                 CV_NET_MAP_SLOTS, f.perms, CV_NET_PERM_SLOTS, conv_ws, f.conv_ws_b,
+                                 d->use_range_flag ? d_flags + 16 * k : nullptr, &head, stream);
         if (rc != CV_OK) return rc;
     }
     clock.lap(1);
     CV_HIP_CHECK(clock.mark(1));
-    for (int k = 0; k < K; ++k) {
-        rc = cv_head_separate_f32(d->d_out_feats[k], n, d->out_ld, d->log_scale, xyz + (size_t)k * n * 3, scale + (size_t)k * n * 3,
-                                  prob + (size_t)k * n, stream);
-        if (rc != CV_OK) return rc;
-    }
     if (d->use_range_flag) CV_HIP_CHECK(hipMemcpyAsync(h_flags, d_flags, sizeof(int32_t) * 16 * K, hipMemcpyDeviceToHost, st));
     r->d_xyz = xyz; r->d_scale = scale; r->d_prob = prob;
     CV_HIP_CHECK(clock.mark(2));
diff --git a/canonicalvoting_amd/csrc/sparse_conv.hip b/canonicalvoting_amd/csrc/sparse_conv.hip
--- a/canonicalvoting_amd/csrc/sparse_conv.hip
+++ b/canonicalvoting_amd/csrc/sparse_conv.hip
@@ -1430,12 +1430,262 @@
     }
 }
 
+__device__ __forceinline__ void head_joint_row(const float* row, long long i, int ncls, int log_scale, float* __restrict__ xyz,
+                                               float* __restrict__ scale, float* __restrict__ prob, int* __restrict__ cls) {
+    const float* logit = row + 6 * ncls;
+    float mx = logit[0];
+    int am = 0;
+    for (int k = 1; k <= ncls; ++k)
+        if (logit[k] > mx) { mx = logit[k]; am = k; }
+    float mo = logit[0];
+    int ao = 0;
+    for (int k = 1; k < ncls; ++k)
+        if (logit[k] > mo) { mo = logit[k]; ao = k; }
+    float den = 0.f;
+    for (int k = 0; k <= ncls; ++k) den += expf(logit[k] - mx);
+    const int h = am == ncls ? 0 : am;
+    for (int d = 0; d < 3; ++d) {
+        xyz[i * 3 + d] = row[h * 3 + d];
+        const float s = row[3 * ncls + h * 3 + d];
+        scale[i * 3 + d] = log_scale ? expf(s) : s;
+    }
+    prob[i] = expf(mo - mx) / den;
+    cls[i] = ao;
+}
+__device__ __forceinline__ void head_separate_row(const float* row, long long i, int log_scale, float* __restrict__ xyz,
+                                                  float* __restrict__ scale, float* __restrict__ prob) {
+    for (int d = 0; d < 3; ++d) {
+        xyz[i * 3 + d] = row[d];
+        scale[i * 3 + d] = log_scale ? expf(row[3 + d]) : row[3 + d];
+    }
+    const float mx = fmaxf(row[6], row[7]);
+    const float e0 = expf(row[6] - mx), e1 = expf(row[7] - mx);
+    prob[i] = e1 / (e0 + e1);
+}
+
+constexpr int TAIL_MAX_NCH = 4;
+template <int NB, int HEAD, bool SPLIT>
+__global__ __launch_bounds__(THREADS) void conv_finish_tail(ConvArgs a, TailArgs t) {
+    constexpr int NW = THREADS / 64;
+    constexpr int YLD = NB * 32 + 4;
+    constexpr int B_CHUNK = 2 * NB * 32 * 64;
+    constexpr int B_BYTES = TAIL_MAX_NCH * B_CHUNK, Y_BYTES = NW * 32 * YLD * 4;
+    __shared__ __attribute__((aligned(16))) unsigned char by_s[B_BYTES > Y_BYTES ? B_BYTES : Y_BYTES];
+    __shared__ __attribute__((aligned(16))) unsigned char a_s[NW][32 * 128];
+    __shared__ int rows_s[TM];
+    const int tid = threadIdx.x, lane = tid & 63, wave = tid >> 6;
+    const int half = lane >> 5, l31 = lane & 31;
+    const int nch = a.cout / KC;
+    {
+        const int per_chunk = 2 * NB * 32 * 4;
+        const unsigned slab_words = 2u * (unsigned)t.cout * 32u;
+        for (int f = tid; f < nch * per_chunk; f += THREADS) {
+            const int c = f / per_chunk, rem = f - c * per_chunk;
+            const int p = rem / (NB * 32 * 4), rem2 = rem - p * (NB * 32 * 4);
+            const int col = rem2 >> 2, ch = rem2 & 3;
+            uint4 v = make_uint4(0u, 0u, 0u, 0u);
+            if (col < t.cout) v = *reinterpret_cast<const uint4*>(t.wp + (size_t)c * slab_words + (p * t.cout + col) * 32 + ch * 8);
+            *reinterpret_cast<uint4*>(by_s + c * B_CHUNK + (p * NB * 32 + col) * 64 + ((ch ^ ((col >> 2) & 3)) << 4)) = v;
+        }
+    }
+    const long long row0 = blockIdx.x * (long long)TM;
+    if (tid < TM) {
+        const long long i = row0 + tid;
+        int r = i < t.n_out ? (t.map ? t.map[i] : (int)i) : -1;
+        if (r >= a.n_out) r = -1;
+        rows_s[tid] = r;
+    }
+    __syncthreads();
+
+    f32x16 acc[NB], xs[SPLIT ? NB : 1];
+#pragma unroll
+    for (int nb = 0; nb < NB; ++nb)
+#pragma unroll
+        for (int r = 0; r < 16; ++r) acc[nb][r] = 0.f;
+    int z = 0;
+    auto close_split = [&]() {
+#pragma unroll
+        for (int nb = 0; nb < NB; ++nb)
+#pragma unroll
+            for (int r = 0; r < 16; ++r) {
+                float p = acc[nb][r] * t.acc_scale;
+                asm volatile("" : "+v"(p));
+                const float s = 0.f + p;
+                xs[SPLIT ? nb : 0][r] = z == 0 ? s : xs[SPLIT ? nb : 0][r] + s;
+                acc[nb][r] = 0.f;
+            }
+    };
+    unsigned char* const At = a_s[wave];
+    const int cq = a.cout >> 2;
+    const long long total4 = a.n_out * (long long)cq;
+    const float4* const part = reinterpret_cast<const float4*>(a.partial);
+    const int bswz = (l31 >> 2) & 3;
+    for (int c = 0; c < nch; ++c) {
+        if constexpr (SPLIT) {
+            if (c == (int)((long long)nch * (z + 1) / t.splits)) { close_split(); ++z; }
+        }
+#pragma unroll
+        for (int it = 0; it < 4; it += 2) {
+            int rl[2], col[2];
+            long long row[2];
+            float4 sq[2][4];
+#pragma unroll
+            for (int u = 0; u < 2; ++u) {
+                const int e = (it + u) * 64 + lane;
+                rl[u] = e >> 3;
+                col[u] = c * 32 + (e & 7) * 4;
+                row[u] = rows_s[wave * 32 + rl[u]];
+#pragma unroll
+                for (int q = 0; q < 4; ++q) sq[u][q] = make_float4(0.f, 0.f, 0.f, 0.f);
+            }
+            for (int k0 = 0; k0 < a.splits; k0 += 4) {
+                float4 pv[2][4];
+#pragma unroll
+                for (int u = 0; u < 2; ++u)
+#pragma unroll
+                    for (int q = 0; q < 4; ++q) {
+                        const int k = k0 + q;
+                        pv[u][q] = (row[u] >= 0 && k < a.splits && (!a.gvalid || a.gvalid[(long long)k * a.n_out + row[u]]))
+                                       ? partial_load4(part + (long long)k * total4 + row[u] * cq + (col[u] >> 2))
+                                       : make_float4(0.f, 0.f, 0.f, 0.f);
+                    }
+#pragma unroll
+                for (int u = 0; u < 2; ++u)
+#pragma unroll
+                    for (int q = 0; q < 4; ++q) {
+                        sq[u][q].x += pv[u][q].x; sq[u][q].y += pv[u][q].y; sq[u][q].z += pv[u][q].z; sq[u][q].w += pv[u][q].w;
+                    }
+            }
+#pragma unroll
+            for (int u = 0; u < 2; ++u) {
+                unsigned h0 = 0u, l0 = 0u, h1 = 0u, l1 = 0u;
+                if (row[u] >= 0) {
+                    float4 x = make_float4(sq[u][0].x + sq[u][1].x + sq[u][2].x + sq[u][3].x, sq[u][0].y + sq[u][1].y + sq[u][2].y + sq[u][3].y,
+                                           sq[u][0].z + sq[u][1].z + sq[u][2].z + sq[u][3].z, sq[u][0].w + sq[u][1].w + sq[u][2].w + sq[u][3].w);
+                    if (a.acc_in) {
+                        const float4 q = *reinterpret_cast<const float4*>(a.acc_in + row[u] * a.acc_ld + col[u]);
+                        x.x += q.x; x.y += q.y; x.z += q.z; x.w += q.w;
+                    }
+                    const float4 sc = a.scale ? *reinterpret_cast<const float4*>(a.scale + col[u]) : make_float4(1.f, 1.f, 1.f, 1.f);
+                    const float4 sh = a.shift ? *reinterpret_cast<const float4*>(a.shift + col[u]) : make_float4(0.f, 0.f, 0.f, 0.f);
+                    x.x = x.x * sc.x + sh.x; x.y = x.y * sc.y + sh.y; x.z = x.z * sc.z + sh.z; x.w = x.w * sc.w + sh.w;
+                    if (a.res) {
+                        const float4 q = a.res_hl ? hl_load4(a.res + row[u] * a.res_ld, col[u])
+                                                  : *reinterpret_cast<const float4*>(a.res + row[u] * a.res_ld + col[u]);
+                        x.x += q.x; x.y += q.y; x.z += q.z; x.w += q.w;
+                    }
+                    if (a.relu) { x.x = fmaxf(x.x, 0.f); x.y = fmaxf(x.y, 0.f); x.z = fmaxf(x.z, 0.f); x.w = fmaxf(x.w, 0.f); }
+                    if (a.range_flag && hl_out_of_range(x)) *a.range_flag = 1;
+                    hl_split2(x.x, x.y, h0, l0);
+                    hl_split2(x.z, x.w, h1, l1);
+                }
+                const int piece = (col[u] & 31) >> 3, within = ((col[u] & 31) * 2) & 15, sw = rl[u] & 7;
+                unsigned char* pr = At + rl[u] * 128 + within;
+                *reinterpret_cast<uint2*>(pr + ((piece ^ sw) << 4)) = make_uint2(h0, h1);
+                *reinterpret_cast<uint2*>(pr + (((piece + 4) ^ sw) << 4)) = make_uint2(l0, l1);
+            }
+        }
+        __builtin_amdgcn_fence(__ATOMIC_RELEASE, "wavefront");
+        __builtin_amdgcn_wave_barrier();
+        __builtin_amdgcn_fence(__ATOMIC_ACQUIRE, "wavefront");
+        {
+            const unsigned char* Ar = At + l31 * 128;
+            const unsigned char* Bb = by_s + c * B_CHUNK + l31 * 64;
+            const int sw = l31 & 7;
+#pragma unroll
+            for (int ks = 0; ks < 2; ++ks) {
+                const int pa = 2 * ks + half;
+                const f16x8 a0 = *reinterpret_cast<const f16x8*>(Ar + ((pa ^ sw) << 4));
+                const f16x8 a1 = *reinterpret_cast<const f16x8*>(Ar + (((pa + 4) ^ sw) << 4));
+                const int piece = (pa ^ bswz) << 4;
+#pragma unroll
+                for (int nb = 0; nb < NB; ++nb) {
+                    const f16x8 b0 = *reinterpret_cast<const f16x8*>(Bb + nb * 32 * 64 + piece);
+                    const f16x8 b1 = *reinterpret_cast<const f16x8*>(Bb + (NB * 32 + nb * 32) * 64 + piece);
+                    acc[nb] = __builtin_amdgcn_mfma_f32_32x32x16_f16(a0, b1, acc[nb], 0, 0, 0);
+                    acc[nb] = __builtin_amdgcn_mfma_f32_32x32x16_f16(a1, b0, acc[nb], 0, 0, 0);
+                    acc[nb] = __builtin_amdgcn_mfma_f32_32x32x16_f16(a0, b0, acc[nb], 0, 0, 0);
+                }
+            }
+        }
+        __builtin_amdgcn_fence(__ATOMIC_RELEASE, "wavefront");
+        __builtin_amdgcn_wave_barrier();
+        __builtin_amdgcn_fence(__ATOMIC_ACQUIRE, "wavefront");
+    }
+    if constexpr (SPLIT) {
+        close_split();
+    } else {
+#pragma unroll
+        for (int nb = 0; nb < NB; ++nb)
+#pragma unroll
+            for (int r = 0; r < 16; ++r) acc[nb][r] *= t.acc_scale;
+    }
+    __syncthreads();
+    float (*Y)[YLD] = reinterpret_cast<float (*)[YLD]>(by_s + wave * 32 * YLD * 4);
+#pragma unroll
+    for (int nb = 0; nb < NB; ++nb)
+#pragma unroll
+        for (int r = 0; r < 16; ++r)
+            Y[(r & 3) + 8 * (r >> 2) + 4 * half][nb * 32 + l31] = SPLIT ? xs[SPLIT ? nb : 0][r] : acc[nb][r];
+    __builtin_amdgcn_fence(__ATOMIC_RELEASE, "wavefront");
+    __builtin_amdgcn_wave_barrier();
+    __builtin_amdgcn_fence(__ATOMIC_ACQUIRE, "wavefront");
+    const int cq_o = t.cout >> 2;
+    for (int e = lane; e < 32 * cq_o; e += 64) {
+        const int rl = e / cq_o, col = (e - rl * cq_o) * 4;
+        const long long i = row0 + wave * 32 + rl;
+        float4 v = *reinterpret_cast<const float4*>(&Y[rl][col]);
+        const float4 sc = t.scale ? *reinterpret_cast<const float4*>(t.scale + col) : make_float4(1.f, 1.f, 1.f, 1.f);
+        const float4 sh = t.shift ? *reinterpret_cast<const float4*>(t.shift + col) : make_float4(0.f, 0.f, 0.f, 0.f);
+        v.x = v.x * sc.x + sh.x; v.y = v.y * sc.y + sh.y; v.z = v.z * sc.z + sh.z; v.w = v.w * sc.w + sh.w;
+        if (t.relu) { v.x = fmaxf(v.x, 0.f); v.y = fmaxf(v.y, 0.f); v.z = fmaxf(v.z, 0.f); v.w = fmaxf(v.w, 0.f); }
+        if (i < t.n_out) *reinterpret_cast<float4*>(t.out + i * t.out_ld + col) = v;
+        if constexpr (HEAD != 0) *reinterpret_cast<float4*>(&Y[rl][col]) = v;
+    }
+    if constexpr (HEAD != 0) {
+        __builtin_amdgcn_fence(__ATOMIC_RELEASE, "wavefront");
+        __builtin_amdgcn_wave_barrier();
+        __builtin_amdgcn_fence(__ATOMIC_ACQUIRE, "wavefront");
+        const long long i = row0 + wave * 32 + l31;
+        if (half == 0 && i < t.n_out) {
+            if constexpr (HEAD == 1) head_joint_row(Y[l31], i, t.ncls, t.log_scale, t.xyz, t.hscale, t.prob, t.cls);
+            else head_separate_row(Y[l31], i, t.log_scale, t.xyz, t.hscale, t.prob);
+        }
+    }
+}
+
 }
 namespace cvsc {
 std::atomic<int> g_ablation{0};
+thread_local const TailArgs* t_tail = nullptr;
+thread_local int t_tail_head = 0;
+thread_local bool t_tail_done = false;
+std::atomic<long long> g_tail_launches{0};
+template <int NB, int HEAD>
+static void launch_tail(const ConvArgs& a, const TailArgs& t, hipStream_t st) {
+    const unsigned grid = (unsigned)((t.n_out + TM - 1) / TM);
+    if (t.splits > 1) conv_finish_tail<NB, HEAD, true><<<grid, THREADS, 0, st>>>(a, t);
+    else conv_finish_tail<NB, HEAD, false><<<grid, THREADS, 0, st>>>(a, t);
+}
 int launch_finish(const ConvArgs& a, hipStream_t st) {
     if (g_ablation.load(std::memory_order_relaxed) & 1) return CV_OK;
     const long long total = a.n_out * (long long)a.cout;
+    if (t_tail && a.wide && a.splits <= FINISH_SMALL_MAX && a.out_hl && a.cout % KC == 0 && a.cout <= TAIL_MAX_NCH * KC) {
+        const TailArgs& t = *t_tail;
+        if (t.cout <= 32) {
+            if (t_tail_head == 1) launch_tail<1, 1>(a, t, st);
+            else if (t_tail_head == 2) launch_tail<1, 2>(a, t, st);
+            else launch_tail<1, 0>(a, t, st);
+        } else {
+            if (t_tail_head == 1) launch_tail<2, 1>(a, t, st);
+            else if (t_tail_head == 2) launch_tail<2, 2>(a, t, st);
+            else launch_tail<2, 0>(a, t, st);
+        }
+        CV_LAUNCH_CHECK();
+        t_tail_done = true;
+        g_tail_launches.fetch_add(1, std::memory_order_relaxed);
+        return CV_OK;
+    }
     if (a.wide && a.splits <= FINISH_SMALL_MAX)
         conv_finish_small<<<(unsigned)std::min<long long>((total / 4 + 255) / 256, 16384), 256, 0, st>>>(a);
     else if (a.cout % 4 == 0)
@@ -1969,26 +2219,7 @@
                                                   int* __restrict__ cls) {
     const long long i = blockIdx.x * 256ll + threadIdx.x;
     if (i >= n) return;
-    const float* row = f + i * ld;
-    const float* logit = row + 6 * ncls;
-    float mx = logit[0];
-    int am = 0;
-    for (int k = 1; k <= ncls; ++k)
-        if (logit[k] > mx) { mx = logit[k]; am = k; }
-    float mo = logit[0];
-    int ao = 0;
-    for (int k = 1; k < ncls; ++k)
-        if (logit[k] > mo) { mo = logit[k]; ao = k; }
-    float den = 0.f;
-    for (int k = 0; k <= ncls; ++k) den += expf(logit[k] - mx);
-    const int h = am == ncls ? 0 : am;
-    for (int d = 0; d < 3; ++d) {
-        xyz[i * 3 + d] = row[h * 3 + d];
-        const float s = row[3 * ncls + h * 3 + d];
-        scale[i * 3 + d] = log_scale ? expf(s) : s;
-    }
-    prob[i] = expf(mo - mx) / den;
-    cls[i] = ao;
+    head_joint_row(f + i * ld, i, ncls, log_scale, xyz, scale, prob, cls);
 }
 
 __global__ __launch_bounds__(256) void head_separate(const float* __restrict__ f, long long n, int ld,
@@ -1996,19 +2227,13 @@
                                                      float* __restrict__ scale, float* __restrict__ prob) {
     const long long i = blockIdx.x * 256ll + threadIdx.x;
     if (i >= n) return;
-    const float* row = f + i * ld;
-    for (int d = 0; d < 3; ++d) {
-        xyz[i * 3 + d] = row[d];
-        scale[i * 3 + d] = log_scale ? expf(row[3 + d]) : row[3 + d];
-    }
-    const float mx = fmaxf(row[6], row[7]);
-    const float e0 = expf(row[6] - mx), e1 = expf(row[7] - mx);
-    prob[i] = e1 / (e0 + e1);
+    head_separate_row(f + i * ld, i, log_scale, xyz, scale, prob);
 }
 
 std::atomic<long long> g_opt_zskip{getenv("CV_ZSKIP") ? atoll(getenv("CV_ZSKIP")) : 0};
 std::atomic<long long> g_opt_hd_mask{getenv("CV_HD") ? atoll(getenv("CV_HD")) : 4};
 std::atomic<long long> g_opt_hd_min_rows{getenv("CV_HD_MIN_ROWS") ? atoll(getenv("CV_HD_MIN_ROWS")) : 16384};
+std::atomic<long long> g_opt_tail_fuse{getenv("CV_TAIL_FUSE") ? atoll(getenv("CV_TAIL_FUSE")) : 0};
 std::atomic<long long> g_opt_hd_shape{getenv("CV_HD_SHAPE") ? atoll(getenv("CV_HD_SHAPE")) : 2};
 
 template <int NB>
@@ -2138,8 +2363,9 @@
 int cv_sp_set_option(const char* name, long long value, long long* previous) {
     CV_REQUIRE(name, CV_EINVAL, "null option name");
     std::atomic<long long>* o = !strcmp(name, "hd_mask") ? &g_opt_hd_mask : !strcmp(name, "hd_min_rows") ? &g_opt_hd_min_rows :
-                                !strcmp(name, "hd_shape") ? &g_opt_hd_shape : !strcmp(name, "zskip") ? &g_opt_zskip : nullptr;
-    CV_REQUIRE(o, CV_EINVAL, "unknown option '%s' (hd_mask, hd_min_rows, hd_shape, zskip)", name);
+                                !strcmp(name, "hd_shape") ? &g_opt_hd_shape : !strcmp(name, "zskip") ? &g_opt_zskip :
+                                !strcmp(name, "tail_fuse") ? &g_opt_tail_fuse : nullptr;
+    CV_REQUIRE(o, CV_EINVAL, "unknown option '%s' (hd_mask, hd_min_rows, hd_shape, zskip, tail_fuse)", name);
     const long long before = o->exchange(value, std::memory_order_relaxed);
     if (previous) *previous = before;
     return CV_OK;
@@ -2148,7 +2374,9 @@
 int cv_sp_get_option(const char* name, long long* value) {
     CV_REQUIRE(name && value, CV_EINVAL, "null option name / value");
     const std::atomic<long long>* o = !strcmp(name, "hd_mask") ? &g_opt_hd_mask : !strcmp(name, "hd_min_rows") ? &g_opt_hd_min_rows :
-                                      !strcmp(name, "hd_shape") ? &g_opt_hd_shape : !strcmp(name, "zskip") ? &g_opt_zskip : nullptr;
+                                      !strcmp(name, "hd_shape") ? &g_opt_hd_shape : !strcmp(name, "zskip") ? &g_opt_zskip :
+                                      !strcmp(name, "tail_fuse") ? &g_opt_tail_fuse :
+                                      !strcmp(name, "tail_launches") ? &g_tail_launches : nullptr;
     CV_REQUIRE(o, CV_EINVAL, "unknown option '%s'", name);
     *value = o->load(std::memory_order_relaxed);
     return CV_OK;
@@ -2207,8 +2435,59 @@
     return 256 + std::min<size_t>(64 * one, std::max<size_t>((size_t)48 << 20, 3 * one));
 }
 
+static int conv_f32(const cv_conv_desc* d, void* stream);
+
+static cv_conv_desc tail_consumer_desc(const cv_conv_desc* d) {
+    const cv_conv_tail& t = *d->tail;
+    cv_conv_desc c = {};
+    c.in = d->out; c.n_in = d->n_out; c.in_ld = d->out_ld; c.cin = d->cout; c.in_hl = d->out_hl;
+    c.weight = t.weight; c.weight_x6 = t.weight_x6; c.weight_pieces = t.weight_pieces; c.acc_scale = t.acc_scale;
+    c.K = 1; c.cout = t.cout; c.nbr = t.map; c.n_out = t.n_out;
+    c.scale = t.scale; c.shift = t.shift; c.relu = t.relu;
+    c.out = t.out; c.out_ld = t.out_ld;
+    c.ws = d->ws; c.ws_bytes = d->ws_bytes;
+    c.range_flag = t.range_flag;
+    return c;
+}
+
 int cv_sp_conv_f32(const cv_conv_desc* d, void* stream) {
     CV_REQUIRE(d, CV_EINVAL, "null descriptor");
+    if (!d->tail) return conv_f32(d, stream);
+    const cv_conv_tail& t = *d->tail;
+    CV_REQUIRE(t.weight && t.out && t.cout > 0 && t.n_out > 0 && t.out_ld >= t.cout && (t.map || t.n_out == d->n_out), CV_EINVAL,
+               "bad convolution tail");
+    CV_REQUIRE(t.head_kind >= 0 && t.head_kind <= 2 && (t.head_kind == 0 || (t.d_xyz && t.d_scale && t.d_prob)) &&
+                   (t.head_kind != 1 || (t.d_class && t.nclasses > 0)), CV_EINVAL, "bad head of the convolution tail");
+    TailArgs ta = {static_cast<const unsigned short*>(t.weight_x6), t.map, t.n_out, t.cout, t.relu, t.scale, t.shift,
+                   t.acc_scale != 0.f ? t.acc_scale : 1.f, t.out, t.out_ld, 1, t.nclasses, t.log_scale, t.d_xyz, t.d_scale, t.d_prob,
+                   t.d_class};
+    bool can = g_opt_tail_fuse.load(std::memory_order_relaxed) != 0 && t.weight_pieces == 2 && t.weight_x6 && d->cout % KC == 0 &&
+               t.cout % 4 == 0 && t.cout <= 64 && t.out_ld % 4 == 0 &&
+               ((reinterpret_cast<uintptr_t>(t.out) | reinterpret_cast<uintptr_t>(t.scale) | reinterpret_cast<uintptr_t>(t.shift) |
+                 reinterpret_cast<uintptr_t>(t.weight_x6) | reinterpret_cast<uintptr_t>(d->ws)) & 15) == 0 &&
+               (t.head_kind != 1 || 7 * t.nclasses + 1 <= t.cout) && (t.head_kind != 2 || t.cout >= 8);
+    if (can) {
+        const int sp = pick_splits(t.n_out, t.cout, 1, d->cout, true);
+        const size_t need = sizeof(float) * (size_t)sp * (size_t)t.n_out * (size_t)t.cout;
+        if (sp > 1 && d->ws && d->ws_bytes >= need) ta.splits = sp;
+        else if (sp > 1) can = false;
+        if (ta.splits > 4) can = false;
+    }
+    t_tail = can ? &ta : nullptr;
+    t_tail_head = t.head_kind;
+    t_tail_done = false;
+    int rc = conv_f32(d, stream);
+    t_tail = nullptr;
+    if (rc != CV_OK || t_tail_done) return rc;
+    const cv_conv_desc c = tail_consumer_desc(d);
+    rc = conv_f32(&c, stream);
+    if (rc != CV_OK || t.head_kind == 0) return rc;
+    if (t.head_kind == 1)
+        return cv_head_joint_f32(t.out, t.n_out, t.out_ld, t.nclasses, t.log_scale, t.d_xyz, t.d_scale, t.d_prob, t.d_class, stream);
+    return cv_head_separate_f32(t.out, t.n_out, t.out_ld, t.log_scale, t.d_xyz, t.d_scale, t.d_prob, stream);
+}
+
+static int conv_f32(const cv_conv_desc* d, void* stream) {
     CV_REQUIRE(d->in && d->weight && d->out, CV_EINVAL, "null pointer argument");
     CV_REQUIRE(d->n_in > 0 && d->n_out > 0 && d->cin > 0 && d->cout > 0 && d->K > 0, CV_EINVAL, "bad conv sizes");
     CV_REQUIRE(d->nbr || (d->K == 1 && d->n_in == d->n_out), CV_EINVAL, "a kernel map is required unless K == 1");
diff --git a/canonicalvoting_amd/csrc/sparse_conv_common.h b/canonicalvoting_amd/csrc/sparse_conv_common.h
--- a/canonicalvoting_amd/csrc/sparse_conv_common.h
+++ b/canonicalvoting_amd/csrc/sparse_conv_common.h
@@ -49,6 +49,20 @@
     const unsigned char* gvalid;
 };
 
+struct TailArgs {
+    const unsigned short* wp;
+    const int* map;
+    long long n_out;
+    int cout;
+    int relu;
+    const float* scale; const float* shift;
+    float acc_scale;
+    float* out; int out_ld;
+    int splits;
+    int ncls, log_scale;
+    float* xyz; float* hscale; float* prob; int* cls;
+};
+
 __device__ __forceinline__ void hl_split2(float x0, float x1, unsigned& h, unsigned& l);
 __device__ __forceinline__ float4 hl_load4(const float* row, int col) {
     const unsigned char* p = reinterpret_cast<const unsigned char*>(row) + (col >> 5) * 128 + (col & 31) * 2;
diff --git a/canonicalvoting_amd/me/__init__.py b/canonicalvoting_amd/me/__init__.py
--- a/canonicalvoting_amd/me/__init__.py
+++ b/canonicalvoting_amd/me/__init__.py
@@ -390,7 +390,7 @@
 def conv_forward(x_feats, weight, nbr, n_out, scale=None, shift=None, residual=None, relu=False,
                  out=None, flavour=0, row_perm=None, j_begin=0, j_end=0, acc_in=None, perm_groups=0,
                  cache_weights=True, pieces=None, in_hl=False, out_hl=False, res_hl=False, stem_mfma=False,
-                 split_tickets=None, weight_t=False, acc_scale_dev=None):
+                 split_tickets=None, weight_t=False, acc_scale_dev=None, tail=None):
     if pieces is None:
         pieces = 1 if COMPUTE_DTYPE == "bf16" else 3
     L = _lib.lib()
@@ -482,6 +482,8 @@
                       1 if (perm_groups > 1 and getattr(row_perm, "_cv_has_map", False)) else 0,
                       2 if flag is not None else (1 if (pieces == 1 and wp6 is not None) else 0), acc_scale, p(flag),
                       1 if in_hl else 0, 1 if out_hl else 0, 1 if res_hl else 0, p(split_tickets), p(acc_scale_dev))
+    if tail is not None:
+        d.tail = ctypes.pointer(tail)
     with _on(dev):
         _lib.check(L.cv_sp_conv_f32(ctypes.byref(d), _stream(dev)), "cv_sp_conv_f32")
     return out
diff --git a/include/cv_hip.h b/include/cv_hip.h
--- a/include/cv_hip.h
+++ b/include/cv_hip.h
@@ -14,7 +14,7 @@
 #define CV_EHIP (-5)
 #define CV_ERANGE (-34)
 
-#define CV_ABI_VERSION 4
+#define CV_ABI_VERSION 5
 int cv_abi_version(void);
 const char* cv_last_error(void);
 
@@ -112,6 +112,28 @@
 
 int cv_sp_up_map(const int32_t* d_nbr_down, long long n_coarse, long long n_fine, int32_t* d_up,
                  void* stream);
+
+typedef struct cv_conv_tail {
+    const float* weight;
+    const void* weight_x6;
+    int weight_pieces;
+    float acc_scale;
+    int cout;
+    int relu;
+    const float* scale;
+    const float* shift;
+    const int32_t* map;
+    long long n_out;
+    float* out;
+    int out_ld;
+    int32_t* range_flag;
+    int head_kind;
+    int nclasses, log_scale;
+    float* d_xyz;
+    float* d_scale;
+    float* d_prob;
+    int32_t* d_class;
+} cv_conv_tail;
 
 typedef struct cv_conv_desc {
     const float* in;
@@ -150,6 +172,7 @@
     int in_hl, out_hl, res_hl;
     int32_t* split_tickets;
     const float* acc_scale_dev;
+    const cv_conv_tail* tail;
 } cv_conv_desc;
 #define CV_SPLIT_TICKETS 4096
 
@@ -239,6 +262,17 @@
                    int n_levels, void* d_arena, size_t arena_bytes, const void* const* ext_ptr, const int* ext_ld,
                    const int32_t* const* maps, int n_maps, const int32_t* const* perms, int n_perms,
                    void* d_ws, size_t ws_bytes, int32_t* range_flag, void* stream);
+typedef struct cv_net_head {
+    int kind, nclasses, log_scale;
+    float* d_xyz;
+    float* d_scale;
+    float* d_prob;
+    int32_t* d_class;
+} cv_net_head;
+int cv_net_run_head_f32(const cv_net_op* ops, int n_ops, const cv_net_buf* bufs, int n_bufs, const long long* level_rows,
+                        int n_levels, void* d_arena, size_t arena_bytes, const void* const* ext_ptr, const int* ext_ld,
+                        const int32_t* const* maps, int n_maps, const int32_t* const* perms, int n_perms,
+                        void* d_ws, size_t ws_bytes, int32_t* range_flag, const cv_net_head* head, void* stream);
 
 int cv_sp_mask_keys(const int32_t* d_nbr, long long n, int K, int j_begin, int j_end, long long* d_keys,
                     void* stream);
```

Result: no change. 625.2 (-0.2%).
